# batra-mlp-lab/visdial

Hardware: AMD Instinct MI355X
Metric: QA-rounds/sec training mn-att-ques-im-hist+disc (batch 20x10x100) (higher is better)
Workload: dtype f32 operands and results; the option recurrence multiplies the EXACT 3-way bf16 split of both operands (9 bf16 MFMA products per fp32 product, f32 accumulate: fp32-grade, errors at the f32 MFMA's own level) -- its two step kernels and its weight-gradient contraction; f32 MFMA (v_mfma_f32_32x32x2_f32

## Files before the change

### visdial_amd/csrc/common.h

```cpp
#pragma once
#include <hip/hip_runtime.h>
#include <stdint.h>
#include <stdio.h>
#include <string.h>

#define VD_OK 0
#define VD_ERR_ARG -1
#define VD_ERR_HIP -2
#define VD_ERR_STATE -3
#define VD_FLAG_BF16 1
#define VD_FLAG_SPLIT9 2
#define VD_FLAG_SPLIT6 4
#define VD_FLAG_SPLIT3 8
#define VD_FLAG_SPLIT (VD_FLAG_SPLIT9 | VD_FLAG_SPLIT6 | VD_FLAG_SPLIT3)
#define VD_FLAG_LIVE_PREFIX 16
#define VD_FLAG_STATE_ONLY 32
#define VD_FLAG_TREE 64
#define VD_LIVE_PREFIX_ROWS 128

void vd_set_error(const char* fmt, ...);

#define VD_CHECK_ARG(cond, ...)                                   \
  do {                                                            \
    if (!(cond)) {                                                \
      vd_set_error(__VA_ARGS__);                                  \
      return VD_ERR_ARG;                                          \
    }                                                             \
  } while (0)

#define VD_HIP(expr)                                                          \
  do {                                                                        \
    hipError_t e__ = (expr);                                                  \
    if (e__ != hipSuccess) {                                                  \
      vd_set_error("%s:%d: %s -> %s", __FILE__, __LINE__, #expr,              \
                   hipGetErrorString(e__));                                   \
      return VD_ERR_HIP;                                                      \
    }                                                                         \
  } while (0)

#define VD_LAUNCH_CHECK() VD_HIP(hipGetLastError())

static inline int vd_cdiv(long a, long b) { return (int)((a + b - 1) / b); }
static inline unsigned grid_for(long n) { return (unsigned)std::max<long>(1, std::min<long>((n + 255) / 256, 4096)); }

void vd_range_push(const char* name);
void vd_range_pop();
struct VdRange {
  explicit VdRange(const char* name) { vd_range_push(name); }
  ~VdRange() { vd_range_pop(); }
  VdRange(const VdRange&) = delete;
  VdRange& operator=(const VdRange&) = delete;
};

struct VdStreamScratch {
  float* wht = nullptr;
  size_t wht_bytes = 0;
  unsigned* sync = nullptr;
  size_t sync_bytes = 0;
};
int vd_stream_scratch(hipStream_t stream, size_t wht_bytes, size_t sync_bytes, VdStreamScratch* out);
int vd_num_cus();

struct VdZeroSet {
  float* buf[6];
  int ncols[6];
  int n;
  long quads_per_row;
};
int vd_zero_inactive_multi(const VdZeroSet& z, const int32_t* nact_dev, int T, int N, hipStream_t stream);

typedef unsigned short vd_bf16_bits;
int vd_lstm_forward_c16(const vd_bf16_bits* table16, int64_t tab_ld, const int32_t* tok_gather, const float* Wh, vd_bf16_bits* gates16,
                        vd_bf16_bits* h16, float* h_last, float* c, int T, int N, int H, hipStream_t stream);
int vd_lstm_backward_c16(const float* Wh, vd_bf16_bits* gates16, const float* c, const float* dh_last, float* dc_work, int T, int N, int H,
                         hipStream_t stream);
int vd_f32_to_bf16(const float* src, vd_bf16_bits* dst, int64_t n, hipStream_t stream);
int vd_gemm_tn_acc_bf16(const vd_bf16_bits* A16, const vd_bf16_bits* B16, float* C, int64_t ldc, int M, int N, int K, hipStream_t stream);
int vd_segment_rowsum_acc_bf16(const vd_bf16_bits* X16, int64_t ldx, const int32_t* tok, const int32_t* perm, int64_t n, int ncol,
                               float* out, int64_t ldo, hipStream_t stream);

int vd_bf16_shadow_get(int slot, const float* base, size_t floats, vd_bf16_bits** out);
const vd_bf16_bits* vd_bf16_shadow_find(const float* p, size_t floats);
void vd_bf16_shadow_invalidate(const float* p, size_t floats);

typedef float f32x16 __attribute__((ext_vector_type(16)));

__device__ __forceinline__ float vd_rcp(float x) { return __builtin_amdgcn_rcpf(x); }
__device__ __forceinline__ float vd_sigmoid(float x) { return vd_rcp(1.0f + __expf(-x)); }
__device__ __forceinline__ float vd_tanh(float x) {
  const float e = __expf(-2.0f * fabsf(x));
  const float t = (1.0f - e) * vd_rcp(1.0f + e);
  return copysignf(t, x);
}

typedef unsigned vd_u32x4 __attribute__((ext_vector_type(4)));
typedef unsigned vd_u32x2 __attribute__((ext_vector_type(2)));
__device__ __forceinline__ __amdgpu_buffer_rsrc_t vd_rsrc(const void* p) {
  return __builtin_amdgcn_make_buffer_rsrc(const_cast<void*>(p), 0, -1, 0x00020000);
}
__device__ __forceinline__ float4 vd_buf_ld4(__amdgpu_buffer_rsrc_t r, unsigned voff, unsigned soff) {
  const vd_u32x4 v = __builtin_amdgcn_raw_buffer_load_b128(r, voff, soff, 0);
  return make_float4(__uint_as_float(v.x), __uint_as_float(v.y), __uint_as_float(v.z), __uint_as_float(v.w));
}
__device__ __forceinline__ void vd_buf_st4(__amdgpu_buffer_rsrc_t r, unsigned voff, unsigned soff, const float4& v) {
  const vd_u32x4 t = {__float_as_uint(v.x), __float_as_uint(v.y), __float_as_uint(v.z), __float_as_uint(v.w)};
  __builtin_amdgcn_raw_buffer_store_b128(t, r, voff, soff, 0);
}
__device__ __forceinline__ void vd_buf_st4_bf16(__amdgpu_buffer_rsrc_t r, unsigned voff, unsigned soff, const float4& v) {
  typedef __bf16 bf4 __attribute__((ext_vector_type(4)));
  const bf4 t = {(__bf16)v.x, (__bf16)v.y, (__bf16)v.z, (__bf16)v.w};
  __builtin_amdgcn_raw_buffer_store_b64(__builtin_bit_cast(vd_u32x2, t), r, voff, soff, 0);
}

__device__ __forceinline__ float4 vd_bf16x4_unpack(const vd_u32x2 v) {
  return make_float4(__uint_as_float(v.x << 16), __uint_as_float(v.x & 0xffff0000u), __uint_as_float(v.y << 16),
                     __uint_as_float(v.y & 0xffff0000u));
}
__device__ __forceinline__ float4 vd_buf_ld4_bf16(__amdgpu_buffer_rsrc_t r, unsigned voff, unsigned soff) {
  return vd_bf16x4_unpack(__builtin_amdgcn_raw_buffer_load_b64(r, voff, soff, 0));
}

__device__ __forceinline__ void vd_st4_bf16(vd_bf16_bits* p, const float4& v) {
  typedef __bf16 bf4 __attribute__((ext_vector_type(4)));
  bf4 t = {(__bf16)v.x, (__bf16)v.y, (__bf16)v.z, (__bf16)v.w};
  *reinterpret_cast<bf4*>(p) = t;
}

__device__ __forceinline__ float wave_sum(float v) {
#pragma unroll
  for (int o = 32; o > 0; o >>= 1) v += __shfl_xor(v, o, 64);
  return v;
}
__device__ __forceinline__ float wave_max(float v) {
#pragma unroll
  for (int o = 32; o > 0; o >>= 1) v = fmaxf(v, __shfl_xor(v, o, 64));
  return v;
}

__device__ __forceinline__ float block_row_lse(const float* row, int V, float* red) {
  const int tid = threadIdx.x, lane = tid & 63, wave = tid >> 6;
  float mx = -INFINITY;
  for (int c = tid; c < V; c += 256) mx = fmaxf(mx, row[c]);
  mx = wave_max(mx);
  if (lane == 0) red[wave] = mx;
  __syncthreads();
  mx = fmaxf(fmaxf(red[0], red[1]), fmaxf(red[2], red[3]));
  float sum = 0.f;
  for (int c = tid; c < V; c += 256) sum += expf(row[c] - mx);
  sum = wave_sum(sum);
  if (lane == 0) red[4 + wave] = sum;
  __syncthreads();
  return mx + logf(red[4] + red[5] + red[6] + red[7]);
}
```

### visdial_amd/csrc/elementwise.hip

```cpp
#include <stdlib.h>

#include "common.h"

__device__ __forceinline__ uint32_t mix32(uint64_t x) {
  x ^= x >> 33;
  x *= 0xff51afd7ed558ccdULL;
  x ^= x >> 33;
  x *= 0xc4ceb9fe1a85ec53ULL;
  x ^= x >> 33;
  return (uint32_t)x;
}

__global__ void dropout_mask_kernel(uint8_t* __restrict__ mask, long n, uint64_t seed, float p) {
  const long i4 = ((long)blockIdx.x * blockDim.x + threadIdx.x) * 4;
  if (i4 >= n) return;
  const uint32_t thr = (uint32_t)(p * 16777216.0f);
  uint8_t m[4];
#pragma unroll
  for (int k = 0; k < 4; ++k) {
    const uint32_t h = mix32(seed * 0x9E3779B97F4A7C15ULL + (uint64_t)(i4 + k));
    m[k] = ((h >> 8) >= thr) ? 1 : 0;
  }
  if (i4 + 3 < n) {
    *reinterpret_cast<uint32_t*>(mask + i4) = m[0] | (m[1] << 8) | (m[2] << 16) | ((uint32_t)m[3] << 24);
  } else {
    for (int k = 0; k < 4 && i4 + k < n; ++k) mask[i4 + k] = m[k];
  }
}

__global__ void dropout_apply_kernel(const float* __restrict__ x, const uint8_t* __restrict__ mask,
                                     float* __restrict__ y, long n, float scale) {
  const long i = (long)blockIdx.x * blockDim.x + threadIdx.x;
  if (i < n) y[i] = mask[i] ? x[i] * scale : 0.f;
}

__global__ void tanh_bwd_kernel(const float* __restrict__ dy, const float* __restrict__ y,
                                float* __restrict__ dx, long n) {
  const long i = (long)blockIdx.x * blockDim.x + threadIdx.x;
  if (i < n) {
    const float t = y[i];
    dx[i] = dy[i] * (1.f - t * t);
  }
}

__global__ void axpby_kernel(const float* __restrict__ a, const float* __restrict__ b, float* __restrict__ c,
                             long n, float alpha, float beta) {
  const long i = (long)blockIdx.x * blockDim.x + threadIdx.x;
  if (i < n) c[i] = alpha * a[i] + (b ? beta * b[i] : 0.f);
}

__global__ void embed_gather_kernel(const float* __restrict__ emb, const int* __restrict__ tok,
                                    const uint8_t* __restrict__ mask, float* __restrict__ out, long rows, int E,
                                    float scale) {
  const int e4 = E >> 2;
  const long idx = (long)blockIdx.x * blockDim.x + threadIdx.x;
  if (idx >= rows * e4) return;
  const long r = idx / e4;
  const int q = (int)(idx - r * e4);
  float4 v = *reinterpret_cast<const float4*>(emb + (long)tok[r] * E + q * 4);
  if (mask) {
    const uint32_t m = *reinterpret_cast<const uint32_t*>(mask + r * E + q * 4);
    v.x = (m & 0xff) ? v.x * scale : 0.f;
    v.y = (m & 0xff00) ? v.y * scale : 0.f;
    v.z = (m & 0xff0000) ? v.z * scale : 0.f;
    v.w = (m & 0xff000000u) ? v.w * scale : 0.f;
  }
  *reinterpret_cast<float4*>(out + r * E + q * 4) = v;
}

__global__ void embed_scatter_kernel(float* __restrict__ demb, const int* __restrict__ tok,
                                     const uint8_t* __restrict__ mask, const float* __restrict__ dx, long rows,
                                     int E, float scale) {
  const long idx = (long)blockIdx.x * blockDim.x + threadIdx.x;
  if (idx >= rows * E) return;
  const long r = idx / E;
  const int e = (int)(idx - r * E);
  float v = dx[idx];
  if (mask) v = mask[idx] ? v * scale : 0.f;
  if (v != 0.f) unsafeAtomicAdd(demb + (long)tok[r] * E + e, v);
}

__global__ void mask_time_fwd_kernel(const float* __restrict__ feat, const int* __restrict__ tok,
                                     float* __restrict__ out, int T, int N, int D) {
  const long idx = (long)blockIdx.x * blockDim.x + threadIdx.x;
  const long total = (long)T * N * D;
  if (idx >= total) return;
  const long tn = idx / D;
  const int d = (int)(idx - tn * D);
  const int n = (int)(tn % N);
  out[idx] = tok[tn] != 0 ? feat[(long)n * D + d] : 0.f;
}
__global__ void mask_time_bwd_kernel(const float* __restrict__ dout, const int* __restrict__ tok,
                                     float* __restrict__ dfeat, int T, int N, int D) {
  const long idx = (long)blockIdx.x * blockDim.x + threadIdx.x;
  if (idx >= (long)N * D) return;
  const int n = (int)(idx / D);
  const int d = (int)(idx - (long)n * D);
  float s = 0.f;
  for (int t = 0; t < T; ++t)
    if (tok[(long)t * N + n] != 0) s += dout[((long)t * N + n) * D + d];
  dfeat[idx] = s;
}

__global__ void zero_inactive_rows_kernel(float* __restrict__ buf, long tstride, long ld, int ncols,
                                          const int* __restrict__ nact, int N) {
  const int t = blockIdx.y;
  const int first = nact[t];
  const long total = (long)(N - first) * (ncols >> 2);
  for (long idx = (long)blockIdx.x * blockDim.x + threadIdx.x; idx < total; idx += (long)gridDim.x * blockDim.x) {
    const long r = idx / (ncols >> 2);
    const int q = (int)(idx - r * (ncols >> 2));
    *reinterpret_cast<float4*>(buf + t * tstride + (first + r) * ld + q * 4) = make_float4(0.f, 0.f, 0.f, 0.f);
  }
}

__global__ void zero_inactive_multi_kernel(VdZeroSet z, const int* __restrict__ nact, int N) {
  const int t = blockIdx.y;
  const int first = nact[t];
  const long per_row = z.quads_per_row;
  const long total = (long)(N - first) * per_row;
  for (long idx = (long)blockIdx.x * blockDim.x + threadIdx.x; idx < total; idx += (long)gridDim.x * blockDim.x) {
    const long r = idx / per_row;
    int q = (int)(idx - r * per_row);
    int b = 0;
#pragma unroll
    for (int i = 0; i < 5; ++i)
      if (b == i && i + 1 < z.n && q >= (z.ncols[i] >> 2)) { q -= z.ncols[i] >> 2; b = i + 1; }
    *reinterpret_cast<float4*>(z.buf[b] + ((long)t * N + first + r) * z.ncols[b] + q * 4) = make_float4(0.f, 0.f, 0.f, 0.f);
  }
}

__device__ __forceinline__ int wave_agg_atomic_inc(int* base, int tok, bool active) {
  int result = 0;
  unsigned long long todo = __ballot(active);
  const int lane = threadIdx.x & 63;
  while (todo) {
    const int leader = __ffsll((long long)todo) - 1;
    const int ltok = __shfl(tok, leader, 64);
    const unsigned long long same = __ballot(active && tok == ltok) & todo;
    int basev = 0;
    if (lane == leader) basev = atomicAdd(base + ltok, __popcll(same));
    basev = __shfl(basev, leader, 64);
    if ((same >> lane) & 1ULL) result = basev + __popcll(same & ((1ULL << lane) - 1ULL));
    todo &= ~same;
  }
  return result;
}

__global__ void tok_count_kernel(const int* __restrict__ tok, long n, int* __restrict__ count) {
  const long i = (long)blockIdx.x * blockDim.x + threadIdx.x;
  const bool active = i < n;
  wave_agg_atomic_inc(count, active ? tok[i] : 0, active);
}

__global__ void tok_scan_kernel(const int* __restrict__ count, int V, int* __restrict__ offset,
                                int* __restrict__ cursor) {
  __shared__ int part[1024];
  const int tid = threadIdx.x, nt = blockDim.x;
  const int per = (V + nt - 1) / nt;
  const int b = tid * per, e = min(V, b + per);
  int s = 0;
  for (int i = b; i < e; ++i) s += count[i];
  part[tid] = s;
  __syncthreads();
  if (tid == 0) {
    int run = 0;
    for (int i = 0; i < nt; ++i) {
      const int t = part[i];
      part[i] = run;
      run += t;
    }
    offset[V] = run;
  }
  __syncthreads();
  int run = part[tid];
  for (int i = b; i < e; ++i) {
    offset[i] = run;
    cursor[i] = run;
    run += count[i];
  }
}

__global__ void tok_fill_kernel(const int* __restrict__ tok, long n, int* __restrict__ cursor,
                                int* __restrict__ perm) {
  const long i = (long)blockIdx.x * blockDim.x + threadIdx.x;
  const bool active = i < n;
  const int p = wave_agg_atomic_inc(cursor, active ? tok[i] : 0, active);
  if (active) perm[p] = (int)i;
}

template <int CHUNK, bool X16 = false>
__global__ void __launch_bounds__(256)
segment_rowsum_kernel(const float* __restrict__ X, long ldx, const int* __restrict__ tok,
                      const int* __restrict__ perm, long n, int ncol, float* __restrict__ out, long ldo) {
  __shared__ int srow[CHUNK], stok[CHUNK];
  const long p0 = (long)blockIdx.x * CHUNK;
  if (p0 >= n) return;
  const int cnt = (int)min((long)CHUNK, n - p0);
  if ((int)threadIdx.x < cnt) {
    const int r = perm[p0 + threadIdx.x];
    srow[threadIdx.x] = r;
    stok[threadIdx.x] = tok[r];
  }
  __syncthreads();
  if constexpr (X16) {
    const vd_bf16_bits* X16p = reinterpret_cast<const vd_bf16_bits*>(X);
    for (int c = threadIdx.x * 4; c < ncol; c += blockDim.x * 8) {
      const int c2 = c + blockDim.x * 4;
      const bool two = c2 < ncol;
      float4 acc0 = make_float4(0.f, 0.f, 0.f, 0.f), acc1 = acc0;
      auto flush = [&](int token) {
        float* o = out + (long)token * ldo + c;
        unsafeAtomicAdd(o, acc0.x); unsafeAtomicAdd(o + 1, acc0.y); unsafeAtomicAdd(o + 2, acc0.z); unsafeAtomicAdd(o + 3, acc0.w);
        if (two) {
          float* o2 = out + (long)token * ldo + c2;
          unsafeAtomicAdd(o2, acc1.x); unsafeAtomicAdd(o2 + 1, acc1.y); unsafeAtomicAdd(o2 + 2, acc1.z); unsafeAtomicAdd(o2 + 3, acc1.w);
        }
        acc0 = acc1 = make_float4(0.f, 0.f, 0.f, 0.f);
      };
      int cur = stok[0];
      int j = 0;
      while (j < cnt) {
        uint2 w0[4], w1[4];
        int t[4];
#pragma unroll
        for (int u = 0; u < 4; ++u) {
          const int jj = min(j + u, cnt - 1);
          t[u] = stok[jj];
          const vd_bf16_bits* row = X16p + (long)srow[jj] * ldx;
          w0[u] = *reinterpret_cast<const uint2*>(row + c);
          w1[u] = two ? *reinterpret_cast<const uint2*>(row + c2) : make_uint2(0u, 0u);
        }
#pragma unroll
        for (int u = 0; u < 4; ++u) {
          if (j + u >= cnt) break;
          if (t[u] != cur) {
            flush(cur);
            cur = t[u];
          }
          acc0.x += __uint_as_float(w0[u].x << 16); acc0.y += __uint_as_float(w0[u].x & 0xffff0000u);
          acc0.z += __uint_as_float(w0[u].y << 16); acc0.w += __uint_as_float(w0[u].y & 0xffff0000u);
          acc1.x += __uint_as_float(w1[u].x << 16); acc1.y += __uint_as_float(w1[u].x & 0xffff0000u);
          acc1.z += __uint_as_float(w1[u].y << 16); acc1.w += __uint_as_float(w1[u].y & 0xffff0000u);
        }
        j += 4;
      }
      flush(cur);
    }
    return;
  }
  for (int c = threadIdx.x * 4; c < ncol; c += blockDim.x * 4) {
    float4 acc = make_float4(0.f, 0.f, 0.f, 0.f);
    int cur = stok[0];
    int j = 0;
    while (j < cnt) {
      float4 v[4];
      int t[4];
#pragma unroll
      for (int u = 0; u < 4; ++u) {
        const int jj = min(j + u, cnt - 1);
        t[u] = stok[jj];
        v[u] = *reinterpret_cast<const float4*>(X + (long)srow[jj] * ldx + c);
      }
#pragma unroll
      for (int u = 0; u < 4; ++u) {
        if (j + u >= cnt) break;
        if (t[u] != cur) {
          float* o = out + (long)cur * ldo + c;
          unsafeAtomicAdd(o, acc.x);
          unsafeAtomicAdd(o + 1, acc.y);
          unsafeAtomicAdd(o + 2, acc.z);
          unsafeAtomicAdd(o + 3, acc.w);
          acc = make_float4(0.f, 0.f, 0.f, 0.f);
          cur = t[u];
        }
        acc.x += v[u].x;
        acc.y += v[u].y;
        acc.z += v[u].z;
        acc.w += v[u].w;
      }
      j += 4;
    }
    float* o = out + (long)cur * ldo + c;
    unsafeAtomicAdd(o, acc.x);
    unsafeAtomicAdd(o + 1, acc.y);
    unsafeAtomicAdd(o + 2, acc.z);
    unsafeAtomicAdd(o + 3, acc.w);
  }
}

__global__ void clamp_adam_kernel(float* __restrict__ w, float* __restrict__ g, float* __restrict__ m,
                                  float* __restrict__ v, long n, float gscale, float clip, float b1, float b2,
                                  float eps, float step) {
  const long i4 = ((long)blockIdx.x * blockDim.x + threadIdx.x) * 4;
  if (i4 + 3 < n) {
    float4 W = *reinterpret_cast<float4*>(w + i4), G = *reinterpret_cast<float4*>(g + i4);
    float4 Mv = *reinterpret_cast<float4*>(m + i4), Vv = *reinterpret_cast<float4*>(v + i4);
    float* Wp = &W.x;
    float* Gp = &G.x;
    float* Mp = &Mv.x;
    float* Vp = &Vv.x;
#pragma unroll
    for (int k = 0; k < 4; ++k) {
      float gg = Gp[k] * gscale;
      gg = fminf(fmaxf(gg, -clip), clip);
      Gp[k] = gg;
      Mp[k] = b1 * Mp[k] + (1.f - b1) * gg;
      Vp[k] = b2 * Vp[k] + (1.f - b2) * gg * gg;
      Wp[k] -= step * Mp[k] / (sqrtf(Vp[k]) + eps);
    }
    *reinterpret_cast<float4*>(w + i4) = W;
    *reinterpret_cast<float4*>(g + i4) = G;
    *reinterpret_cast<float4*>(m + i4) = Mv;
    *reinterpret_cast<float4*>(v + i4) = Vv;
  } else {
    for (long i = i4; i < n; ++i) {
      float gg = g[i] * gscale;
      gg = fminf(fmaxf(gg, -clip), clip);
      g[i] = gg;
      m[i] = b1 * m[i] + (1.f - b1) * gg;
      v[i] = b2 * v[i] + (1.f - b2) * gg * gg;
      w[i] -= step * m[i] / (sqrtf(v[i]) + eps);
    }
  }
}

static inline dim3 grid1d(long n, int block) { return dim3((unsigned)((n + block - 1) / block)); }

extern "C" {

int vd_dropout_mask(uint8_t* mask, int64_t n, uint64_t seed, float p, void* stream) {
  VD_CHECK_ARG(mask && n >= 0 && p >= 0.f && p < 1.f && ((uintptr_t)mask & 3) == 0, "vd_dropout_mask: bad args");
  if (n == 0) return VD_OK;
  hipLaunchKernelGGL(dropout_mask_kernel, grid1d((n + 3) / 4, 256), dim3(256), 0, (hipStream_t)stream, mask,
                     (long)n, seed, p);
  VD_LAUNCH_CHECK();
  return VD_OK;
}

int vd_dropout_apply(const float* x, const uint8_t* mask, float* y, int64_t n, float scale, void* stream) {
  VD_CHECK_ARG(x && mask && y && n >= 0, "vd_dropout_apply: bad args");
  if (n == 0) return VD_OK;
  hipLaunchKernelGGL(dropout_apply_kernel, grid1d(n, 256), dim3(256), 0, (hipStream_t)stream, x, mask, y,
                     (long)n, scale);
  VD_LAUNCH_CHECK();
  return VD_OK;
}

int vd_tanh_backward(const float* dy, const float* y, float* dx, int64_t n, void* stream) {
  VD_CHECK_ARG(dy && y && dx && n >= 0, "vd_tanh_backward: bad args");
  if (n == 0) return VD_OK;
  hipLaunchKernelGGL(tanh_bwd_kernel, grid1d(n, 256), dim3(256), 0, (hipStream_t)stream, dy, y, dx, (long)n);
  VD_LAUNCH_CHECK();
  return VD_OK;
}

int vd_axpby(const float* a, const float* b, float* c, int64_t n, float alpha, float beta, void* stream) {
  VD_CHECK_ARG(a && c && n >= 0, "vd_axpby: bad args");
  if (n == 0) return VD_OK;
  hipLaunchKernelGGL(axpby_kernel, grid1d(n, 256), dim3(256), 0, (hipStream_t)stream, a, b, c, (long)n, alpha,
                     beta);
  VD_LAUNCH_CHECK();
  return VD_OK;
}

int vd_mask_time_forward(const float* feat, const int32_t* tok, float* out, int T, int N, int D, void* stream) {
  VD_CHECK_ARG(feat && tok && out && T >= 0 && N >= 0 && D > 0, "vd_mask_time_forward: bad args");
  const long total = (long)T * N * D;
  if (total == 0) return VD_OK;
  hipLaunchKernelGGL(mask_time_fwd_kernel, grid1d(total, 256), dim3(256), 0, (hipStream_t)stream, feat, tok, out,
                     T, N, D);
  VD_LAUNCH_CHECK();
  return VD_OK;
}

int vd_mask_time_backward(const float* dout, const int32_t* tok, float* dfeat, int T, int N, int D,
                          void* stream) {
  VD_CHECK_ARG(dout && tok && dfeat && T >= 0 && N >= 0 && D > 0, "vd_mask_time_backward: bad args");
  if ((long)N * D == 0) return VD_OK;
  hipLaunchKernelGGL(mask_time_bwd_kernel, grid1d((long)N * D, 256), dim3(256), 0, (hipStream_t)stream, dout,
                     tok, dfeat, T, N, D);
  VD_LAUNCH_CHECK();
  return VD_OK;
}

int vd_zero_inactive_rows(float* buf, int64_t tstride, int64_t ld, int ncols, const int32_t* nact_dev, int T,
                          int N, void* stream) {
  VD_CHECK_ARG(buf && nact_dev && T >= 0 && N >= 0 && ncols % 4 == 0 && ld % 4 == 0, "vd_zero_inactive_rows: bad args");
  if (T == 0 || N == 0) return VD_OK;
  hipLaunchKernelGGL(zero_inactive_rows_kernel, dim3(64, T), dim3(256), 0, (hipStream_t)stream, buf, (long)tstride,
                     (long)ld, ncols, nact_dev, N);
  VD_LAUNCH_CHECK();
  return VD_OK;
}

int vd_embed_gather(const float* emb, const int32_t* tok, const uint8_t* mask, float* out, int64_t rows, int E,
                    float scale, void* stream);
}
int vd_zero_inactive_multi(const VdZeroSet& z, const int32_t* nact_dev, int T, int N, hipStream_t stream) {
  VD_CHECK_ARG(z.n >= 1 && z.n <= 6 && nact_dev && T >= 0 && N >= 0, "vd_zero_inactive_multi: bad args");
  if (T == 0 || N == 0) return VD_OK;
  VdZeroSet zz = z;
  zz.quads_per_row = 0;
  for (int i = 0; i < z.n; ++i) {
    VD_CHECK_ARG(z.buf[i] && z.ncols[i] % 4 == 0, "vd_zero_inactive_multi: buffer %d", i);
    zz.quads_per_row += z.ncols[i] >> 2;
  }
  hipLaunchKernelGGL(zero_inactive_multi_kernel, dim3(128, T), dim3(256), 0, stream, zz, nact_dev, N);
  VD_LAUNCH_CHECK();
  return VD_OK;
}
extern "C" {
int vd_embed_gather(const float* emb, const int32_t* tok, const uint8_t* mask, float* out, int64_t rows, int E,
                    float scale, void* stream) {
  VD_CHECK_ARG(emb && tok && out && rows >= 0 && E > 0 && E % 4 == 0, "vd_embed_gather: bad args (E=%d)", E);
  if (rows == 0) return VD_OK;
  hipLaunchKernelGGL(embed_gather_kernel, grid1d(rows * (E / 4), 256), dim3(256), 0, (hipStream_t)stream, emb,
                     tok, mask, out, (long)rows, E, scale);
  VD_LAUNCH_CHECK();
  return VD_OK;
}

int vd_embed_scatter_acc(float* demb, const int32_t* tok, const uint8_t* mask, const float* dx, int64_t rows,
                         int E, float scale, void* stream) {
  VD_CHECK_ARG(demb && tok && dx && rows >= 0 && E > 0, "vd_embed_scatter_acc: bad args");
  if (rows == 0) return VD_OK;
  hipLaunchKernelGGL(embed_scatter_kernel, grid1d(rows * E, 256), dim3(256), 0, (hipStream_t)stream, demb, tok,
                     mask, dx, (long)rows, E, scale);
  VD_LAUNCH_CHECK();
  return VD_OK;
}

int vd_token_sort(const int32_t* tok, int64_t n, int V, int32_t* offset, int32_t* work, int32_t* perm,
                  void* stream) {
  VD_CHECK_ARG(tok && offset && work && perm && n >= 0 && V > 0, "vd_token_sort: bad args");
  hipStream_t s = (hipStream_t)stream;
  int* count = work;
  int* cursor = work + V;
  VD_HIP(hipMemsetAsync(count, 0, sizeof(int) * V, s));
  if (n > 0) {
    hipLaunchKernelGGL(tok_count_kernel, grid1d(n, 256), dim3(256), 0, s, tok, (long)n, count);
    VD_LAUNCH_CHECK();
  }
  hipLaunchKernelGGL(tok_scan_kernel, dim3(1), dim3(1024), 0, s, count, V, offset, cursor);
  VD_LAUNCH_CHECK();
  if (n > 0) {
    hipLaunchKernelGGL(tok_fill_kernel, grid1d(n, 256), dim3(256), 0, s, tok, (long)n, cursor, perm);
    VD_LAUNCH_CHECK();
  }
  return VD_OK;
}

int vd_segment_rowsum_acc(const float* X, int64_t ldx, const int32_t* tok, const int32_t* perm, int64_t n,
                          int ncol, float* out, int64_t ldo, void* stream) {
  VD_CHECK_ARG(X && tok && perm && out && n >= 0 && ncol > 0 && ncol % 4 == 0 && ldx % 4 == 0 && ldo % 4 == 0,
               "vd_segment_rowsum_acc: bad args");
  if (n == 0) return VD_OK;
  hipLaunchKernelGGL(segment_rowsum_kernel<256>, grid1d(n, 256), dim3(256), 0, (hipStream_t)stream, X, (long)ldx, tok, perm, (long)n, ncol,
                     out, (long)ldo);
  VD_LAUNCH_CHECK();
  return VD_OK;
}

int vd_clamp_adam(float* w, float* g, float* m, float* v, int64_t n, float gscale, float clip, float beta1,
                  float beta2, float eps, float step, void* stream) {
  VD_CHECK_ARG(w && g && m && v && n >= 0, "vd_clamp_adam: bad args");
  VD_CHECK_ARG((((uintptr_t)w | (uintptr_t)g | (uintptr_t)m | (uintptr_t)v) & 15) == 0,
               "vd_clamp_adam: buffers must be 16-byte aligned");
  if (n == 0) return VD_OK;
  hipLaunchKernelGGL(clamp_adam_kernel, grid1d((n + 3) / 4, 256), dim3(256), 0, (hipStream_t)stream, w, g, m, v,
                     (long)n, gscale, clip, beta1, beta2, eps, step);
  VD_LAUNCH_CHECK();
  return VD_OK;
}

}

int vd_segment_rowsum_acc_bf16(const vd_bf16_bits* X16, int64_t ldx, const int32_t* tok, const int32_t* perm, int64_t n, int ncol,
                               float* out, int64_t ldo, hipStream_t stream) {
  VD_CHECK_ARG(X16 && tok && perm && out && n >= 0 && ncol % 4 == 0 && ldx % 4 == 0, "vd_segment_rowsum_acc_bf16: bad args");
  if (n == 0) return VD_OK;
  hipLaunchKernelGGL((segment_rowsum_kernel<256, true>), grid1d(n, 256), dim3(256), 0, stream, reinterpret_cast<const float*>(X16), (long)ldx,
                     tok, perm, (long)n, ncol, out, (long)ldo);
  VD_LAUNCH_CHECK();
  return VD_OK;
}
```

### visdial_amd/csrc/gemm_ops.hip

```cpp
#include "gemm_core.h"
#include "split_core.h"

using CfgBigDB = GemmCfg<4, 1, 4, 32>;
using CfgBig = GemmCfg<4, 1, 4, 16, 0, 3>;
using CfgSmall = GemmCfg<1, 4, 1, 32, 0, 3>;

static inline bool use_small(int M, int N) {
  return (long)vd_cdiv(M, CfgBig::BM) * vd_cdiv(N, CfgBig::BN) < 48;
}

static int check_align(const void* p, long ld, const char* what) {
  if (((uintptr_t)p & 15) != 0 || (ld & 3) != 0) {
    vd_set_error("%s: pointer must be 16-byte aligned and leading dimension a multiple of 4 (ld=%ld)", what, ld);
    return VD_ERR_ARG;
  }
  return VD_OK;
}

__global__ void colsum_kernel(const float* __restrict__ X, long ld, int M, int N, int rows_per_block,
                              float* __restrict__ out) {
  const int col = blockIdx.x * blockDim.x + threadIdx.x;
  if (col >= N) return;
  const int r0 = blockIdx.y * rows_per_block;
  const int r1 = min(M, r0 + rows_per_block);
// ... 82 lines not shown
#pragma unroll
    for (int r = 0; r < 16; ++r) acc[j][r] = 0.f;

  const int key = (lane & 7) >> 1, col = (lane >> 3) * 16 + (lane & 1) * 8;
  unsigned voffa[2], voffb[2];
#pragma unroll
  for (int i = 0; i < 2; ++i) {
    const int krow = (i * 4 + wm) * 4 + key;
    voffa[i] = (unsigned)(((long)krow * M + m0 + col) * 2);
    voffb[i] = (unsigned)(((long)krow * N + n0 + col) * 2);
  }
  const unsigned lds0 = (unsigned)(uintptr_t)lds;
  auto issue = [&](int kt, int buf) {
    const float* ak = reinterpret_cast<const float*>(A + (long)(ks + kt * 32) * M);
    const float* bk = reinterpret_cast<const float*>(B + (long)(ks + kt * 32) * N);
#pragma unroll
    for (int i = 0; i < 2; ++i) glds16(voffb[i], bk, lds0 + buf * 2 * TILE + TILE + (i * 4 + wm) * 1024);
#pragma unroll
    for (int i = 0; i < 2; ++i) glds16(voffa[i], ak, lds0 + buf * 2 * TILE + (i * 4 + wm) * 1024);
  };
  const int g = lane >> 4, li = lane & 15;
  const int frag = ((g >> 1) * 2) * 1024 + (g & 1) * 128 + li * 8;

  if (nk > 0) {
    issue(0, 0);
    if (nk > 1) issue(1, 1);
    int buf = 0;
    for (int kt = 0; kt < nk; ++kt) {
      if (kt + 1 < nk) asm volatile("s_waitcnt vmcnt(4)" ::: "memory");
      else asm volatile("s_waitcnt vmcnt(0)" ::: "memory");
      asm volatile("s_barrier" ::: "memory");
      if (kt + 2 < nk) issue(kt + 2, buf == 0 ? 2 : buf - 1);
      const char* ta = lds + buf * 2 * TILE;
      const char* tb = ta + TILE;
#pragma unroll
      for (int st = 0; st < 2; ++st) {
        const vd_bf16x8 a8 = tr_read8(ta, frag + st * 4096 + wm * 256);
        vd_bf16x8 b8[4];
#pragma unroll
        for (int j = 0; j < 4; ++j) b8[j] = tr_read8(tb, frag + st * 4096 + j * 256);
#pragma unroll
        for (int j = 0; j < 4; ++j) acc[j] = __builtin_amdgcn_mfma_f32_32x32x16_bf16(a8, b8[j], acc[j], 0, 0, 0);
      }
      buf = buf == 2 ? 0 : buf + 1;
    }
  }
#pragma unroll
  for (int j = 0; j < 4; ++j) {
    const int c = n0 + j * 32 + (lane & 31);
#pragma unroll
    for (int r = 0; r < 16; ++r) {
      const int row = m0 + wm * 32 + mfma_row(r, lane);
      unsafeAtomicAdd(C + (long)row * ldc + c, acc[j][r]);
    }
  }
}

template <int NBUF>
__global__ void __launch_bounds__(512)
gemm_bf16_tn_tr256_kernel(const vd_bf16_bits* __restrict__ A, const vd_bf16_bits* __restrict__ B, float* __restrict__ C, long ldc,
                          int M, int N, int K, int kchunk, int tiles_m, int tiles_n) {
  extern __shared__ __attribute__((aligned(16))) float smem[];
  constexpr int TILE = 16384;
  char* const lds = reinterpret_cast<char*>(smem);
  const int wg = xcd_remap(blockIdx.x, gridDim.x);
  const int tile_n = wg % tiles_n, tile_m = (wg / tiles_n) % tiles_m, split = wg / (tiles_n * tiles_m);
  const int ks = split * kchunk, ke = min(K, ks + kchunk);
  const int nk = ke > ks ? (ke - ks) / 32 : 0;
  const int lane = threadIdx.x & 63;
  const int w = __builtin_amdgcn_readfirstlane((int)threadIdx.x >> 6);
  const int wm = w & 3, wn = w >> 2;
  const int m0 = tile_m * 256, n0 = tile_n * 256;

  f32x16 acc[2][4];
#pragma unroll
  for (int i = 0; i < 2; ++i)
#pragma unroll
    for (int j = 0; j < 4; ++j)
#pragma unroll
      for (int r = 0; r < 16; ++r) acc[i][j][r] = 0.f;

  unsigned voffa[2], voffb[2];
#pragma unroll
  for (int i = 0; i < 2; ++i) {
    const int krow = (i * 8 + w) * 2 + (lane >> 5);
    const int cb = ((lane & 31) * 16) ^ ((krow & 3) << 6);
    voffa[i] = (unsigned)(((long)krow * M + m0) * 2 + cb);
    voffb[i] = (unsigned)(((long)krow * N + n0) * 2 + cb);
  }
  const unsigned lds0 = (unsigned)(uintptr_t)lds;
  auto issue = [&](int kt, int buf) {
    const float* ak = reinterpret_cast<const float*>(A + (long)(ks + kt * 32) * M);
    const float* bk = reinterpret_cast<const float*>(B + (long)(ks + kt * 32) * N);
#pragma unroll
    for (int i = 0; i < 2; ++i) glds16(voffb[i], bk, lds0 + buf * 2 * TILE + TILE + (i * 8 + w) * 1024);
#pragma unroll
    for (int i = 0; i < 2; ++i) glds16(voffa[i], ak, lds0 + buf * 2 * TILE + (i * 8 + w) * 1024);
  };
  const int g = lane >> 4, li = lane & 15;
  const int frag = (g >> 1) * 4096 + (li >> 2) * 512 + (g & 1) * 32 + (li & 3) * 8;
  int xa[2], xb[4];
#pragma unroll
  for (int i = 0; i < 2; ++i) xa[i] = frag + (((wm * 2 + i) ^ (li >> 2)) << 6);
#pragma unroll
  for (int j = 0; j < 4; ++j) xb[j] = frag + (((wn * 4 + j) ^ (li >> 2)) << 6);
  auto rd8 = [&](const char* base, int off) {
    typedef __attribute__((address_space(3))) vd_s16x4* lds_p;
    union {
      vd_s16x4 h[2];
      vd_bf16x8 v;
    } u;
    u.h[0] = __builtin_amdgcn_ds_read_tr16_b64_v4i16((lds_p)(base + off));
    u.h[1] = __builtin_amdgcn_ds_read_tr16_b64_v4i16((lds_p)(base + off + 2048));
    return u.v;
  };

  struct Frags {
    vd_bf16x8 a[2], b[4];
  };
  auto read_step = [&](Frags& f, int buf, int st) {
    const char* ta = lds + buf * 2 * TILE;
    const char* tb = ta + TILE;
#pragma unroll
    for (int i = 0; i < 2; ++i) f.a[i] = rd8(ta, xa[i] + st * 8192);
#pragma unroll
    for (int j = 0; j < 4; ++j) f.b[j] = rd8(tb, xb[j] + st * 8192);
  };
  auto mfma_step = [&](const Frags& f) {
#pragma unroll
    for (int i = 0; i < 2; ++i)
#pragma unroll
      for (int j = 0; j < 4; ++j) acc[i][j] = __builtin_amdgcn_mfma_f32_32x32x16_bf16(f.a[i], f.b[j], acc[i][j], 0, 0, 0);
  };
  auto wait_tiles_in_flight = [&](int later) {
    if (later >= 3) asm volatile("s_waitcnt vmcnt(12)" ::: "memory");
    else if (later == 2) asm volatile("s_waitcnt vmcnt(8)" ::: "memory");
    else if (later == 1) asm volatile("s_waitcnt vmcnt(4)" ::: "memory");
    else asm volatile("s_waitcnt vmcnt(0)" ::: "memory");
  };
  if (nk > 0) {
#pragma unroll
    for (int i = 0; i < NBUF - 1; ++i)
      if (i < nk) issue(i, i);
    wait_tiles_in_flight(min(NBUF - 2, nk - 1));
    asm volatile("s_barrier" ::: "memory");
    Frags f0, f1;
    read_step(f0, 0, 0);
    int buf = 0;
    for (int kt = 0; kt < nk; ++kt) {
      const int nbuf = buf == NBUF - 1 ? 0 : buf + 1;
      read_step(f1, buf, 1);
      mfma_step(f0);
      if (kt + 1 < nk) {
        wait_tiles_in_flight(min(NBUF - 3, nk - 2 - kt));
        asm volatile("s_barrier" ::: "memory");
        if (kt + NBUF - 1 < nk) issue(kt + NBUF - 1, buf == 0 ? NBUF - 1 : buf - 1);
        read_step(f0, nbuf, 0);
      }
      mfma_step(f1);
      buf = nbuf;
    }
  }
#pragma unroll
  for (int i = 0; i < 2; ++i)
#pragma unroll
    for (int j = 0; j < 4; ++j) {
      const int c = n0 + wn * 128 + j * 32 + (lane & 31);
#pragma unroll
      for (int r = 0; r < 16; ++r) {
        const int row = m0 + wm * 64 + i * 32 + mfma_row(r, lane);
        unsafeAtomicAdd(C + (long)row * ldc + c, acc[i][j][r]);
      }
    }
}

static int launch_gemm_bf16_tn_tr256(const vd_bf16_bits* A, const vd_bf16_bits* B, float* C, long ldc, int M, int N, int K,
                                     hipStream_t stream) {
  const int tiles_m = M / 256, tiles_n = N / 256;
  long splits = vd_cdiv(256, (long)tiles_m * tiles_n);
  int kchunk = vd_cdiv(vd_cdiv(K, splits), 32) * 32;
  if (kchunk < 32) kchunk = 32;
  splits = vd_cdiv(K, kchunk);
  static bool attr_set = false;
#ifndef VD_TR256_NBUF
#define VD_TR256_NBUF 3
#endif
  constexpr int NBUF = VD_TR256_NBUF;
  const int lds = NBUF * 2 * 16384;
  if (!attr_set) {
    VD_HIP(hipFuncSetAttribute(reinterpret_cast<const void*>(gemm_bf16_tn_tr256_kernel<NBUF>),
                               hipFuncAttributeMaxDynamicSharedMemorySize, lds));
    attr_set = true;
  }
  hipLaunchKernelGGL(gemm_bf16_tn_tr256_kernel<NBUF>, dim3((unsigned)(tiles_m * tiles_n * splits)), dim3(512), lds, stream, A, B, C,
                     ldc, M, N, K, kchunk, tiles_m, tiles_n);
  VD_LAUNCH_CHECK();
  return VD_OK;
}

static int launch_gemm_bf16_tn_tr(const vd_bf16_bits* A, const vd_bf16_bits* B, float* C, long ldc, int M, int N, int K,
                                  hipStream_t stream) {
  const int tiles_m = M / 128, tiles_n = N / 128;
  long splits = vd_cdiv(768, (long)tiles_m * tiles_n);
  int kchunk = vd_cdiv(vd_cdiv(K, splits), 32) * 32;
  if (kchunk < 32) kchunk = 32;
  splits = vd_cdiv(K, kchunk);
  static bool attr_set = false;
  const int lds = 3 * 2 * 8192;
  if (!attr_set) {
    VD_HIP(hipFuncSetAttribute(reinterpret_cast<const void*>(gemm_bf16_tn_tr_kernel),
                               hipFuncAttributeMaxDynamicSharedMemorySize, lds));
    attr_set = true;
  }
  hipLaunchKernelGGL(gemm_bf16_tn_tr_kernel, dim3((unsigned)(tiles_m * tiles_n * splits)), dim3(256), lds, stream, A, B, C,
                     ldc, M, N, K, kchunk, tiles_m, tiles_n);
  VD_LAUNCH_CHECK();
  return VD_OK;
}

extern "C" {

int vd_gemm_nt(const float* A, int64_t lda, const float* W, int64_t ldw, const float* bias, float* C,
               int64_t ldc, int M, int N, int K, int act, int accumulate, void* stream) {
  VD_CHECK_ARG(A && W && C && M >= 0 && N >= 0 && K >= 0 && K % 4 == 0, "vd_gemm_nt: bad args M=%d N=%d K=%d", M,
               N, K);
  if (int rc = check_align(A, lda, "vd_gemm_nt A")) return rc;
  if (int rc = check_align(W, ldw, "vd_gemm_nt W")) return rc;
  SrcRow a{A, lda}, b{W, ldw};
  hipStream_t s = (hipStream_t)stream;
  if (use_small(M, N)) {
    EpiStore<1> e{C, ldc, bias, act, accumulate};
    return launch_gemm<CfgSmall>(M, N, K, 1, a, b, e, s);
  }
  EpiStore<4> e{C, ldc, bias, act, accumulate};
  if (M >= 1024 && K >= 64 && K % 16 == 0 && (long)M * lda * 4 < (1L << 32) && (long)N * ldw * 4 < (1L << 32)) {
    int splits = 1;
    const long tiles = (long)vd_cdiv(M, 128) * vd_cdiv(N, 128);
    if (accumulate == 2 && !bias && act == VD_ACT_NONE && tiles < 512 && K >= 1024) {
      splits = (int)vd_cdiv(768, tiles);
      if (splits > K / 512) splits = K / 512;
    }
    return launch_gemm_glds<GemmCfg<4, 1, 4, 16, 0, 4, 41984>, false>(M, N, K, splits, A, lda, W, ldw, e, s, -1, splits > 1);
  }
  return launch_gemm<CfgBig>(M, N, K, 1, a, b, e, s);
}

int vd_gemm_nn(const float* A, int64_t lda, const float* B, int64_t ldb, const float* bias, float* C,
               int64_t ldc, int M, int N, int K, int accumulate, void* stream) {
  VD_CHECK_ARG(A && B && C && M >= 0 && N >= 0 && K >= 0 && (K % 4 == 0 || lda >= (K + 3) / 4 * 4) && N % 4 == 0,
               "vd_gemm_nn: bad args M=%d N=%d K=%d", M, N, K);
  if (int rc = check_align(A, lda, "vd_gemm_nn A")) return rc;
  if (int rc = check_align(B, ldb, "vd_gemm_nn B")) return rc;
  SrcRow a{A, lda};
  SrcK b{B, ldb};
  hipStream_t s = (hipStream_t)stream;
  if (use_small(M, N)) {
    EpiStore<1> e{C, ldc, bias, VD_ACT_NONE, accumulate};
    return launch_gemm<CfgSmall>(M, N, K, 1, a, b, e, s);
  }
  EpiStore<4> e{C, ldc, bias, VD_ACT_NONE, accumulate};
  return launch_gemm<CfgBig>(M, N, K, 1, a, b, e, s);
}

}

template <int NT>
struct EpiStoreLive : EpiStore<NT> {
  const int* tok_mask;
  static constexpr bool HAS_DEAD = true;
  __device__ __forceinline__ bool dead(int row_base, int ) const { return tok_mask[row_base] == 0; }
};
static_assert(CfgSmall::BM == VD_LSTM_FWD_TILE_SMALL && CfgBig::BM == VD_LSTM_FWD_TILE_BIG, "the projection's row tiles are the step kernels'");

int vd_gemm_nn_live_p(const float* A, int64_t lda, const float* B, int64_t ldb, const float* bias, float* C, int64_t ldc, int M, int N, int K,
                      const int32_t* tok_mask, int row_tile, hipStream_t s) {
  VD_CHECK_ARG(A && B && C && tok_mask && M >= 0 && N >= 0 && K >= 0 && (K % 4 == 0 || lda >= (K + 3) / 4 * 4) && N % 4 == 0 &&
                   (row_tile == CfgSmall::BM || row_tile == CfgBig::BM),
               "vd_gemm_nn (live rows): bad args M=%d N=%d K=%d row tile %d", M, N, K, row_tile);
  if (int rc = check_align(A, lda, "vd_gemm_nn (live rows) A")) return rc;
  if (int rc = check_align(B, ldb, "vd_gemm_nn (live rows) B")) return rc;
  SrcRow a{A, lda};
  SrcK b{B, ldb};
  if (row_tile == CfgSmall::BM) {
    EpiStoreLive<1> e{{C, ldc, bias, VD_ACT_NONE, 0}, tok_mask};
    return launch_gemm<CfgSmall>(M, N, K, 1, a, b, e, s);
  }
  EpiStoreLive<4> e{{C, ldc, bias, VD_ACT_NONE, 0}, tok_mask};
  return launch_gemm<CfgBig>(M, N, K, 1, a, b, e, s);
}

extern "C" {

int vd_gemm_tn_acc(const float* A, int64_t lda, const float* B, int64_t ldb, float* C, int64_t ldc, int M,
                   int N, int K, int flags, void* stream) {
  VD_CHECK_ARG(A && B && C && M >= 0 && N >= 0 && K >= 0 && (M % 4 == 0 || lda >= (M + 3) / 4 * 4) &&
                   (N % 4 == 0 || ldb >= (N + 3) / 4 * 4),
               "vd_gemm_tn_acc: bad args M=%d N=%d K=%d", M, N, K);
  if (int rc = check_align(A, lda, "vd_gemm_tn_acc A")) return rc;
  if (int rc = check_align(B, ldb, "vd_gemm_tn_acc B")) return rc;
  if (K == 0) return VD_OK;
  SrcK a{A, lda}, b{B, ldb};
  EpiAtomic<4> e{C, ldc};
  const long tiles = (long)vd_cdiv(M, CfgBig::BM) * vd_cdiv(N, CfgBig::BN);
  if ((flags & VD_FLAG_SPLIT9) && !(flags & VD_FLAG_BF16) && vd_tn_split_tiles(M, N) && K >= 8192 &&
      16L * lda * 4 < (1L << 31) && 16L * ldb * 4 < (1L << 31)) {
    const int K1 = K & ~15;
    if (int rc = launch_gemm_split_tn<9>(M, N, K1, A, lda, B, ldb, C, ldc, (hipStream_t)stream)) return rc;
    if (K1 == K) return VD_OK;
    SrcK a2{A + (long)K1 * lda, lda}, b2{B + (long)K1 * ldb, ldb};
    return launch_gemm<GemmCfg<4, 1, 4, 16, 0, 4, 41984>>(M, N, K - K1, 1, a2, b2, e, (hipStream_t)stream);
  }
  const bool kmaj = !(flags & VD_FLAG_BF16) && vd_tn_kmajor_fits(M, N, K);
  if (kmaj && K % 16 != 0) {
    const int K1 = K & ~15;
    if (int rc = vd_gemm_tn_acc(A, lda, B, ldb, C, ldc, M, N, K1, flags, stream)) return rc;
    SrcK a2{A + (long)K1 * lda, lda}, b2{B + (long)K1 * ldb, ldb};
    return launch_gemm<GemmCfg<4, 1, 4, 16, 0, 4, 41984>>(M, N, K - K1, 1, a2, b2, e, (hipStream_t)stream);
  }
  long splits = vd_cdiv(768, tiles);
  const long max_splits = vd_cdiv(K, 1024);
  if (splits > max_splits) splits = max_splits;
  if (splits < 1) splits = 1;
  if (flags & VD_FLAG_BF16) {
    if (M % 128 == 0 && N % 128 == 0 && K >= 32 && lda == M && ldb == N && (long)32 * N * 2 + 256 < (1L << 31)) {
      const vd_bf16_bits* a16 = vd_bf16_shadow_find(A, (size_t)K * M);
      const vd_bf16_bits* b16 = vd_bf16_shadow_find(B, (size_t)K * N);
      if (a16 && b16) {
        const int K1 = K & ~31;
        if (int rc = launch_gemm_bf16_tn_tr(a16, b16, C, ldc, M, N, K1, (hipStream_t)stream)) return rc;
        if (K1 == K) return VD_OK;
        SrcK a2{A + (long)K1 * lda, lda}, b2{B + (long)K1 * ldb, ldb};
        return launch_gemm<GemmCfg<4, 1, 4, 32, 0, 3, 0, 1>>(M, N, K - K1, 1, a2, b2, e, (hipStream_t)stream);
      }
    }
    if (vd_tn_split_tiles(M, N) && K >= 1024 && lda % 4 == 0 && ldb % 4 == 0 && 16L * lda * 4 < (1L << 31) &&
        16L * ldb * 4 < (1L << 31)) {
      const int K1 = K & ~15;
      if (int rc = launch_gemm_split_tn<1>(M, N, K1, A, lda, B, ldb, C, ldc, (hipStream_t)stream)) return rc;
      if (K1 == K) return VD_OK;
      SrcK a2{A + (long)K1 * lda, lda}, b2{B + (long)K1 * ldb, ldb};
      return launch_gemm<GemmCfg<4, 1, 4, 32, 0, 3, 0, 1>>(M, N, K - K1, 1, a2, b2, e, (hipStream_t)stream);
    }
    return launch_gemm<GemmCfg<4, 1, 4, 32, 0, 3, 0, 1>>(M, N, K, (int)splits, a, b, e, (hipStream_t)stream);
  }
  if (kmaj)
    return launch_gemm_glds<GemmCfg<4, 1, 4, 16, 0, 4, 41984>, true>(M, N, K, (int)splits, A, lda, B, ldb, e, (hipStream_t)stream, 0);
  return launch_gemm<GemmCfg<4, 1, 4, 16, 0, 4, 41984>>(M, N, K, (int)splits, a, b, e, (hipStream_t)stream);
}

int vd_gemm_tn_rows_acc(const float* A, int64_t lda, const int32_t* a_rows, const float* B, int64_t ldb,
                        const int32_t* b_rows, float* C, int64_t ldc, int M, int N, int K, void* stream) {
  VD_CHECK_ARG(A && B && C && a_rows && b_rows && M >= 0 && N >= 0 && K >= 0 && (M % 4 == 0 || lda >= (M + 3) / 4 * 4) &&
                   (N % 4 == 0 || ldb >= (N + 3) / 4 * 4),
               "vd_gemm_tn_rows_acc: bad args M=%d N=%d K=%d", M, N, K);
  if (int rc = check_align(A, lda, "vd_gemm_tn_rows_acc A")) return rc;
  if (int rc = check_align(B, ldb, "vd_gemm_tn_rows_acc B")) return rc;
  if (K == 0) return VD_OK;
  SrcKRows a{A, lda, a_rows}, b{B, ldb, b_rows};
  EpiAtomic<4> e{C, ldc};
  using Cfg = GemmCfg<4, 1, 4, 16, 0, 4, 41984>;
  const long tiles = (long)vd_cdiv(M, Cfg::BM) * vd_cdiv(N, Cfg::BN);
  long splits = vd_cdiv(768, tiles);
  const long max_splits = vd_cdiv(K, 1024);
  if (splits > max_splits) splits = max_splits;
  if (splits < 1) splits = 1;
  return launch_gemm<Cfg>(M, N, K, (int)splits, a, b, e, (hipStream_t)stream);
}

int vd_colsum_acc(const float* X, int64_t ld, int M, int N, float* out, void* stream) {
  VD_CHECK_ARG(X && out && M >= 0 && N >= 0, "vd_colsum_acc: bad args");
  if (M == 0 || N == 0) return VD_OK;
  if (N % 4 == 0 && ld % 4 == 0 && ((uintptr_t)X & 15) == 0 && M >= 64) {
    const int cb4 = vd_cdiv(N, 256);
    int rb4 = vd_cdiv(2048, cb4);
    int rpb = vd_cdiv(vd_cdiv(M, rb4), 4) * 4;
    if (rpb < 32) rpb = 32;
    rb4 = vd_cdiv(M, rpb);
    hipLaunchKernelGGL(colsum4_kernel, dim3(cb4, rb4), dim3(256), 0, (hipStream_t)stream, X, ld, M, N, rpb, out);
    VD_LAUNCH_CHECK();
    return VD_OK;
  }
  const int cb = vd_cdiv(N, 256);
  int rb = vd_cdiv(1024, cb);
  int rows_per_block = vd_cdiv(M, rb);
  if (rows_per_block < 16) rows_per_block = 16;
  rb = vd_cdiv(M, rows_per_block);
  hipLaunchKernelGGL(colsum_kernel, dim3(cb, rb), dim3(256), 0, (hipStream_t)stream, X, ld, M, N,
                     rows_per_block, out);
  VD_LAUNCH_CHECK();
  return VD_OK;
}

}

__global__ void __launch_bounds__(256) bf16_tn_tail_kernel(const vd_bf16_bits* __restrict__ A, const vd_bf16_bits* __restrict__ B, float* __restrict__ C,
                                                           long ldc, int M, int N, int K) {
  const long i = (long)blockIdx.x * 256 + threadIdx.x;
  if (i >= (long)M * N) return;
  const int m = (int)(i / N), n = (int)(i % N);
  float acc = 0.f;
  for (int k = 0; k < K; ++k)
    acc += __uint_as_float((unsigned)A[(long)k * M + m] << 16) * __uint_as_float((unsigned)B[(long)k * N + n] << 16);
  unsafeAtomicAdd(C + (long)m * ldc + n, acc);
}
int vd_gemm_tn_acc_bf16(const vd_bf16_bits* A16, const vd_bf16_bits* B16, float* C, int64_t ldc, int M, int N, int K, hipStream_t stream) {
  VD_CHECK_ARG(A16 && B16 && C && M % 128 == 0 && N % 128 == 0 && K >= 0, "vd_gemm_tn_acc_bf16: M, N must be multiples of 128");
  const int K1 = K & ~31;
  if (K1 > 0) {
    const bool big = M % 256 == 0 && N % 256 == 0 && K1 >= 8192;
    if (int rc = big ? launch_gemm_bf16_tn_tr256(A16, B16, C, ldc, M, N, K1, stream) : launch_gemm_bf16_tn_tr(A16, B16, C, ldc, M, N, K1, stream)) return rc;
  }
  if (K1 < K) {
    hipLaunchKernelGGL(bf16_tn_tail_kernel, dim3((unsigned)(((long)M * N + 255) / 256)), dim3(256), 0, stream, A16 + (long)K1 * M, B16 + (long)K1 * N,
                       C, (long)ldc, M, N, K - K1);
    VD_LAUNCH_CHECK();
  }
  return VD_OK;
}
```

### visdial_amd/csrc/paths.h

```cpp
#pragma once
#include "common.h"

static inline int vd_precision_flags(int lstmBf16) {
  switch (lstmBf16) {
    case 0: return 0;
    case 1: return VD_FLAG_BF16;
    case 3: return VD_FLAG_SPLIT3;
    case 6: return VD_FLAG_SPLIT6;
    case 9: return VD_FLAG_SPLIT9;
    default: return -1;
  }
}
static inline int vd_split_nprod(int flags) {
  return (flags & VD_FLAG_SPLIT9) ? 9 : (flags & VD_FLAG_SPLIT6) ? 6 : (flags & VD_FLAG_SPLIT3) ? 3 : 0;
}

constexpr long VD_THROUGHPUT_ROWS = 2048;
constexpr int VD_LSTM_FWD_TILE_BIG = 128, VD_LSTM_FWD_TILE_SMALL = 32;
static inline int vd_lstm_fwd_row_tile(long N) { return N >= VD_THROUGHPUT_ROWS ? VD_LSTM_FWD_TILE_BIG : VD_LSTM_FWD_TILE_SMALL; }
static inline bool vd_lstm_glds_fwd_fits(long N, int H) { return N >= VD_THROUGHPUT_ROWS && H % 32 == 0 && N * H * 4 < (1L << 32); }
static inline bool vd_lstm_glds_bwd_fits(long N, int H) { return N >= VD_THROUGHPUT_ROWS && H % 32 == 0 && N * 4 * H * 4 < (1L << 32); }
static inline bool vd_lstm_bf16_fits(long N, int H) { return N >= VD_THROUGHPUT_ROWS && H % 32 == 0; }
static inline bool vd_lstm_c16_fits(long N, int H) { return N >= VD_THROUGHPUT_ROWS && H % 128 == 0; }

static inline bool vd_tn_kmajor_fits(long M, long N, long K) { return M % 128 == 0 && N % 128 == 0 && K >= 1024; }
constexpr int VD_SPLIT_TN_BM = 256, VD_SPLIT_TN_BN = 128;
static inline bool vd_tn_split_tiles(long M, long N) { return M % VD_SPLIT_TN_BM == 0 && N % VD_SPLIT_TN_BN == 0; }

static inline bool vd_img_split_ok(long rows, int H, int Kc) {
  return rows >= 128 && H % 16 == 0 && Kc % 16 == 0 && rows * (H > Kc ? H : Kc) * 4 < (1L << 32);
}

static inline bool vd_lhood_fused_fits(long rows, long ldh, long V, long ldw, int H) {
  return H >= 64 && H % 16 == 0 && V >= 128 && ldh % 4 == 0 && ldw % 4 == 0 && rows * ldh * 4 < (1L << 32) && V * ldw * 4 < (1L << 32);
}
static inline bool vd_lhood_prefix_fits(int T, long rows) { return T >= 1 && T < 256 && rows >= 1; }
```

### visdial_amd/csrc/rt_core.h

```cpp
#pragma once
#include <math.h>
#include <stdarg.h>
#include <stdlib.h>
#include <string.h>

#include <algorithm>
#include <map>
#include <memory>
#include <numeric>
#include <random>
#include <string>
#include <vector>

#include "../../include/visdial_hip.h"
#include "common.h"
#include "paths.h"

int vd_lstm2_forward_p(const vd_lstm2_fwd_t* st, int nstacks, int H, int flags, hipStream_t stream);
int vd_lstm2_backward_p(const vd_lstm2_bwd_t* st, int nstacks, int H, int flags, hipStream_t stream);

int vd_img_drop_gather(const float* pre, const uint8_t* mask1, float* xdrop, int N, int R, int S2, int H, float scale, hipStream_t stream);
int vd_img_common_forward_p(const float* pre, const uint8_t* mask1, const float* xdrop, const float* Wc, const float* bc, const float* qc,
                            const uint8_t* mask2, float* iqc, int N, int R, int S2, int H, int Kc, float scale, int flags, hipStream_t stream);
int vd_img_tr_backward_p(const float* dz, const float* Wc, const float* p, const float* datt, const uint8_t* mask1, float* dpre, int N, int R,
                         int S2, int H, int Kc, float scale, int flags, hipStream_t stream);
int vd_img_common_wgrad_p(const float* dz, const float* pre, const uint8_t* mask1, const float* xdrop, float* dWc, int N, int R, int S2, int H,
                          int Kc, float scale, int flags, hipStream_t stream);

int vd_gemm_nn_live_p(const float* A, int64_t lda, const float* B, int64_t ldb, const float* bias, float* C, int64_t ldc, int M, int N, int K,
                      const int32_t* tok_mask, int row_tile, hipStream_t stream);
int vd_lhood_order_p(const int32_t* tok_in, const int32_t* target, int T, int64_t rows, int C, int32_t* perm, int32_t* rep, int32_t* tok_in_s,
                     int32_t* target_s, int32_t* work, int32_t* info, hipStream_t stream);
int64_t vd_lhood_order_work_ints(int T, int64_t rows);
int vd_lhood_sum_p(const float* nll, const int32_t* act, int64_t n_act, int T, int64_t rows, int C, const int32_t* perm, float* out, int64_t ldo,
                   hipStream_t stream);

int vd_lhood_lse_p(const float* h, int64_t ldh, int64_t rows, const int32_t* act, int64_t n_act, const float* W, int64_t ldw, const float* bias,
                   int V, int H, float* lse, hipStream_t stream);
int vd_lhood_edge_sum_p(const float* h, int64_t ldh, const int32_t* node_row, const float* lse, const int32_t* enode, const int32_t* etgt, int T,
                        int64_t rows, int C, const float* W, int64_t ldw, const float* bias, int H, float* out, int64_t ldo, hipStream_t stream);

#define VD_TRY(expr)                  \
  do {                                \
    const int rc__ = (expr);          \
    if (rc__ != VD_OK) return rc__;   \
  } while (0)

namespace vdrt {

struct Tensor {
  std::string name;
  long off, rows, cols;
  int kind;
  long numel() const { return rows * cols; }
};

struct DevBuf {
  void* p = nullptr;
  size_t bytes = 0;
};

struct SeqTok {
  int T = 0, N = 0;
  bool present = false, sorted = false;
  int32_t* tok = nullptr;
  std::vector<int32_t> nact;
  int32_t *tok_sorted = nullptr, *fwd_idx = nullptr, *inv_idx = nullptr, *perm = nullptr, *inv = nullptr, *nact_dev = nullptr;
  int32_t *act = nullptr, *act1 = nullptr, *prev1 = nullptr;
  int n_act = 0, n_act1 = 0;
};

struct TreeChunk {
  int o0 = 0, C = 0, Tl = 0, Nw = 0;
  long n_nodes = 0;
  std::vector<int32_t> widths;
  int32_t* mask2 = nullptr;
  int32_t* node_row = nullptr;
  int32_t *enode = nullptr, *etgt = nullptr;
};

struct BatchSlot {
  int B = 0;
  bool tree_ok = false;
  std::vector<TreeChunk> tree;
  SeqTok q, h, opt, ain, aout, oin, oout;
  float* img = nullptr;
  int32_t* gt = nullptr;
  std::vector<int32_t> gt_host;
  bool has_gt = false;
  int32_t* opt_uid = nullptr;
  int opt_total = 0;
  int32_t *opt_sort_off = nullptr, *opt_sort_perm = nullptr;
  bool cached = false;
  uint64_t cache_stamp = 0;
  std::vector<int32_t> miss_keys, opt_host;
  hipEvent_t ready = nullptr;
  hipEvent_t done = nullptr;
  bool used = false;
  bool uploaded = false;
  std::map<std::string, DevBuf> bufs, pinned;
};

struct RowIndex {
  int T = 0;
  std::vector<int32_t> keys;
  std::vector<int32_t> table;
  int32_t size() const { return T ? (int32_t)(keys.size() / (size_t)T) : 0; }
  void reset(int T_) {
    T = T_;
    keys.clear();
    table.assign(1024, -1);
  }
  size_t home(const int32_t* row) const {
    uint64_t h = 1469598103934665603ull;
    for (int t = 0; t < T; ++t) h = (h ^ (uint32_t)row[t]) * 1099511628211ull;
    return (size_t)(h ^ (h >> 29)) & (table.size() - 1);
  }
  int32_t find(const int32_t* row) const {
    for (size_t pos = home(row);; pos = (pos + 1) & (table.size() - 1)) {
      const int32_t u = table[pos];
      if (u < 0) return -1;
      if (memcmp(keys.data() + (size_t)u * T, row, (size_t)T * sizeof(int32_t)) == 0) return u;
    }
  }
  int32_t add(const int32_t* row) {
    if ((size_t)(size() + 1) * 2 > table.size()) {
      table.assign(table.size() * 2, -1);
      for (int32_t u = 0; u < size(); ++u) place(keys.data() + (size_t)u * T, u);
    }
    const int32_t id = size();
    keys.insert(keys.end(), row, row + T);
    place(keys.data() + (size_t)id * T, id);
    return id;
  }
  void place(const int32_t* row, int32_t id) {
    size_t pos = home(row);
    while (table[pos] >= 0) pos = (pos + 1) & (table.size() - 1);
    table[pos] = id;
  }
};

struct OptionCache {
  long capacity = 0;
  RowIndex index;
  float* table = nullptr;
  long table_rows = 0;
  uint64_t stamp = 1;
  void flush() {
    index.reset(index.T);
    ++stamp;
  }
};
static constexpr long VD_OPTION_CACHE_DEFAULT_ROWS = 262144;
static constexpr long VD_OPTION_CACHE_FIRST_ROWS = 16384;

struct Encoder;
struct Decoder;

}

struct vd_model {
  vd_model_params p;
  int flags = 0;
  std::string enc_name, dec_name;
  std::vector<vdrt::Tensor> spec;
  std::map<std::string, int> index;
  long numel = 0;
  float *W = nullptr, *G = nullptr, *M = nullptr, *V = nullptr;
  std::map<std::string, vdrt::DevBuf> ws;
  std::map<std::string, vdrt::DevBuf> ext_masks;
  hipStream_t s_main = nullptr, s_enc = nullptr, s_img = nullptr, s_hist = nullptr, s_tab = nullptr, s_copy = nullptr;
  hipStream_t s_wg = nullptr;
  bool wg_active = false, wg_used = false;
  std::vector<hipEvent_t> ev_pool;
  size_t ev_next = 0;
  hipEvent_t ev_enc_grads = nullptr;
  hipEvent_t ev_updated = nullptr;
  bool updated_recorded = false;
  bool enc_grads_recorded = false;
  hipEvent_t ev_loss = nullptr, ev_prof[6] = {nullptr, nullptr, nullptr, nullptr, nullptr, nullptr};
  bool training = true, streams = true, prof_valid = false;
  long step = 0;
  int adam_t = 0;
  double lr = 1e-3;
  vdrt::BatchSlot slot[2];
  int cur = -1, uploaded = -1;
  float* loss_host = nullptr;
  long loss_cap = 0, loss_n = 0;
  bool loss_is_sum = false;
  std::unique_ptr<vdrt::Encoder> enc;
  std::unique_ptr<vdrt::Decoder> dec;
  float* scores = nullptr;
  float* gen_enc_out = nullptr;
  int gen_seq_len = 0;
  int N = 0, O = 0;
  long lhood_exec = -1, lhood_total = 0;
  bool use_im = false, use_hist = false, is_att = false, is_graph = false;
  vdrt::OptionCache ocache;
  bool lhood_tree = false;
  bool prof_hist = false;
  ~vd_model();
};

namespace vdrt {

inline int dev_get(std::map<std::string, DevBuf>& m, const std::string& key, size_t bytes, void** out) {
  DevBuf& b = m[key];
  if (b.bytes < bytes) {
    if (b.p) VD_HIP(hipFree(b.p));
    b.p = nullptr;
    b.bytes = 0;
    VD_HIP(hipMalloc(&b.p, bytes ? bytes : 16));
    b.bytes = bytes ? bytes : 16;
  }
  *out = b.p;
  return VD_OK;
}
inline int pin_get(std::map<std::string, DevBuf>& m, const std::string& key, size_t bytes, void** out) {
  DevBuf& b = m[key];
  if (b.bytes < bytes) {
    if (b.p) VD_HIP(hipHostFree(b.p));
    b.p = nullptr;
    b.bytes = 0;
    VD_HIP(hipHostMalloc(&b.p, bytes ? bytes : 16, hipHostMallocDefault));
    b.bytes = bytes ? bytes : 16;
  }
  *out = b.p;
  return VD_OK;
}

template <class T>
int ws_get(vd_model* m, const std::string& key, size_t count, T** out) {
  void* p = nullptr;
  VD_TRY(dev_get(m->ws, key, count * sizeof(T), &p));
  *out = static_cast<T*>(p);
  return VD_OK;
}

inline void add_lstm(vd_model* m, const std::string& name, long D, long H) {
  m->spec.push_back(Tensor{name + ".W", 0, D + H, 4 * H, 1});
  m->spec.push_back(Tensor{name + ".b", 0, 1, 4 * H, 2});
}
inline void add_linear(vd_model* m, const std::string& name, long in, long out) {
  m->spec.push_back(Tensor{name + ".W", 0, out, in, 3});
  m->spec.push_back(Tensor{name + ".b", 0, 1, out, 4});
}
inline std::string hop_sfx(int i) { return i == 0 ? std::string() : std::to_string(i + 1); }

inline float* Wp(vd_model* m, const std::string& n) { return m->W + m->spec[m->index.at(n)].off; }
inline float* Gp(vd_model* m, const std::string& n) { return m->G + m->spec[m->index.at(n)].off; }

inline int fork_stream(vd_model* m, hipStream_t from, hipStream_t side) {
  if (side == from) return VD_OK;
  hipEvent_t e = m->ev_pool[m->ev_next++ % m->ev_pool.size()];
  VD_HIP(hipEventRecord(e, from));
  VD_HIP(hipStreamWaitEvent(side, e, 0));
  return VD_OK;
}
inline int join_stream(vd_model* m, hipStream_t side, hipStream_t to) { return fork_stream(m, side, to); }
inline hipStream_t side_stream(vd_model* m, hipStream_t wanted, hipStream_t cur) { return m->streams ? wanted : cur; }
inline int wg_fork(vd_model* m, hipStream_t cur, hipStream_t* out) {
  *out = cur;
  if (!m->wg_active || !m->s_wg) return VD_OK;
  VD_TRY(fork_stream(m, cur, m->s_wg));
  m->wg_used = true;
  *out = m->s_wg;
  return VD_OK;
}

inline int drop_mask(vd_model* m, const std::string& site, size_t numel, float p, hipStream_t s, uint8_t** out) {
  *out = nullptr;
  if (!m->training || p <= 0.f) return VD_OK;
  auto it = m->ext_masks.find(site);
  if (it != m->ext_masks.end()) {
    VD_CHECK_ARG(it->second.bytes >= numel, "dropout mask '%s' holds %zu bytes, the batch needs %zu", site.c_str(),
                 it->second.bytes, numel);
    *out = static_cast<uint8_t*>(it->second.p);
    return VD_OK;
  }
  if (!m->ext_masks.empty()) {
    vd_set_error("external dropout masks are set but none for site '%s'", site.c_str());
    return VD_ERR_STATE;
  }
  uint8_t* buf = nullptr;
  VD_TRY(ws_get(m, "dropmask." + site, numel + 4, &buf));
  uint32_t h = 2166136261u;
  for (const char c : site) h = (h ^ (uint8_t)c) * 16777619u;
  const uint64_t seed = ((uint64_t)((m->p.seed * 1000003ull + (uint64_t)m->step) & 0xffffffffull) << 32) | h;
  VD_TRY(vd_dropout_mask(buf, (int64_t)numel, seed, p, s));
  *out = buf;
  return VD_OK;
}
inline int dropout_fwd(vd_model* m, const std::string& key, const float* x, const uint8_t* mask, float scale, long n, hipStream_t s,
                       const float** y) {
  *y = x;
  if (!mask) return VD_OK;
  float* buf;
  VD_TRY(ws_get(m, key, (size_t)n, &buf));
  VD_TRY(vd_dropout_apply(x, mask, buf, n, scale, s));
  *y = buf;
  return VD_OK;
}

inline int index_array(vd_model* m, const std::string& key, const std::vector<int32_t>& host, int32_t** out) {
  DevBuf& b = m->ws[key];
  if (b.bytes != host.size() * sizeof(int32_t) || !b.p) {
    if (b.p) VD_HIP(hipFree(b.p));
    b.p = nullptr;
    VD_HIP(hipMalloc(&b.p, host.size() * sizeof(int32_t) + 16));
    b.bytes = host.size() * sizeof(int32_t);
    VD_HIP(hipMemcpy(b.p, host.data(), b.bytes, hipMemcpyHostToDevice));
  }
  *out = static_cast<int32_t*>(b.p);
  return VD_OK;
}
inline int round_index(vd_model* m, int N, int R, int32_t** out) {
  std::vector<int32_t> h(N);
  for (int n = 0; n < N; ++n) h[n] = n / R;
  return index_array(m, "idx.rep." + std::to_string(N) + "." + std::to_string(R), h, out);
}

struct Linear {
  std::string name;
  long in = 0, out = 0;
  const float* x = nullptr;
  float* y = nullptr;
  long M = 0;
  bool tanh_ = false;
  void init(const std::string& n, long i, long o) { name = n; in = i; out = o; }
  int forward(vd_model* m, hipStream_t s, const float* x_, long M_, bool tanh, float** y_out) {
    x = x_; M = M_; tanh_ = tanh;
    VD_TRY(ws_get(m, name + ".y", (size_t)M * out, &y));
    VD_TRY(vd_gemm_nt(x, in, Wp(m, name + ".W"), in, Wp(m, name + ".b"), y, out, (int)M, (int)out, (int)in,
                      tanh ? VD_ACT_TANH : VD_ACT_NONE, 0, s));
    if (y_out) *y_out = y;
    return VD_OK;
  }
  int backward(vd_model* m, hipStream_t s, const float* dy, bool need_dx, float** dx_out) {
    const float* d = dy;
    if (tanh_) {
      float* dpre;
      VD_TRY(ws_get(m, name + ".dpre", (size_t)M * out, &dpre));
      VD_TRY(vd_tanh_backward(dy, y, dpre, M * out, s));
      d = dpre;
    }
    VD_TRY(vd_gemm_tn_acc(d, out, x, in, Gp(m, name + ".W"), in, (int)out, (int)in, (int)M, 0, s));
    VD_TRY(vd_colsum_acc(d, out, (int)M, (int)out, Gp(m, name + ".b"), s));
    if (dx_out) *dx_out = nullptr;
    if (need_dx) {
      float* dx;
      VD_TRY(ws_get(m, name + ".dx", (size_t)M * in, &dx));
      VD_TRY(vd_gemm_nn(d, out, Wp(m, name + ".W"), in, nullptr, dx, in, (int)M, (int)in, (int)out, 0, s));
      if (dx_out) *dx_out = dx;
    }
    return VD_OK;
  }
};

struct CatLinear {
  std::string name;
  std::vector<long> dims;
  long D = 0, H = 0, N = 0;
  Linear lin;
  const uint8_t* mask = nullptr;
  float scale = 1.f;
  void init(const std::string& n, const std::vector<long>& d, long H_) {
    name = n; dims = d; H = H_; D = 0;
    for (long v : d) D += v;
    lin.init(n, D, H_);
  }
  int forward(vd_model* m, hipStream_t s, const std::vector<const float*>& parts, long N_, const uint8_t* mask_, float scale_,
              float** y) {
    N = N_; mask = mask_; scale = scale_;
    float* cat;
    VD_TRY(ws_get(m, name + ".cat", (size_t)N * D, &cat));
    long off = 0;
    for (size_t i = 0; i < dims.size(); ++i) {
      VD_TRY(vd_copy_2d(cat + off, D, parts[i], dims[i], N, dims[i], s));
      off += dims[i];
    }
    const float* catd;
    VD_TRY(dropout_fwd(m, name + ".in", cat, mask, scale, N * D, s, &catd));
    return lin.forward(m, s, catd, N, true, y);
  }
  int backward(vd_model* m, hipStream_t s, const float* dy, const std::vector<bool>& need, std::vector<float*>* out) {
    float* dcatd;
    VD_TRY(lin.backward(m, s, dy, true, &dcatd));
    const float* dcat;
    VD_TRY(dropout_fwd(m, name + ".din", dcatd, mask, scale, N * D, s, &dcat));
    out->assign(dims.size(), nullptr);
    long off = 0;
    for (size_t i = 0; i < dims.size(); ++i) {
      if (need.empty() || need[i]) {
        float* g;
        VD_TRY(ws_get(m, name + ".dpart" + std::to_string(i), (size_t)N * dims[i], &g));
// ... 188 lines not shown
```

### visdial_amd/csrc/rt_decoders.h

```cpp
#pragma once
#include "rt_encoders.h"

namespace vdrt {

int option_cache_resolve(vd_model* m, BatchSlot& sl, const int32_t* options, long NO, int To, hipStream_t s);

struct Decoder {
  virtual ~Decoder() {}
  virtual void declare(vd_model* m) = 0;
  virtual int forward_backward(vd_model* m, BatchSlot& b, bool only_forward) = 0;
  virtual int retrieve(vd_model* m, BatchSlot& b) = 0;
  virtual int retrieve_lhood(vd_model*, BatchSlot&) {
    vd_set_error("vd_model_retrieve_lhood: the live-row log-likelihood head scores candidates of decoder 'gen'; this model's decoder is 'disc'");
    return VD_ERR_ARG;
  }
  virtual int gen_begin(vd_model*, const int32_t*, int) { return no_gen(); }
  virtual int gen_step(vd_model*, const int32_t*, float*) { return no_gen(); }
  virtual int gen_select(vd_model*, const int32_t*, int) { return no_gen(); }
  virtual int gen_beam_search(vd_model*, int, int, int, int, int32_t*, double*) { return no_gen(); }
  virtual int gen_sample(vd_model*, int, int, int, double, const double*, int32_t*, double*) { return no_gen(); }
  static int no_gen() {
    vd_set_error("sampling / beam search only for the generative decoder (model.lua:436-438)");
    return VD_ERR_STATE;
  }
};

inline int stage_loss(vd_model* m, const float* loss_rows, long n, bool is_sum, hipStream_t s) {
  if (m->loss_cap < n) {
    if (m->loss_host) VD_HIP(hipHostFree(m->loss_host));
    m->loss_host = nullptr;
    VD_HIP(hipHostMalloc((void**)&m->loss_host, (size_t)n * sizeof(float), hipHostMallocDefault));
    m->loss_cap = n;
  }
  m->loss_n = n;
  m->loss_is_sum = is_sum;
  VD_HIP(hipMemcpyAsync(m->loss_host, loss_rows, (size_t)n * sizeof(float), hipMemcpyDeviceToHost, s));
  VD_HIP(hipEventRecord(m->ev_loss, s));
  return VD_OK;
}

#ifdef VD_PROBE_PHASES
inline hipEvent_t* probe_events() {
  static hipEvent_t e[6];
  static bool made = false;
  if (!made) { for (auto& x : e) (void)hipEventCreate(&x); made = true; }
  return e;
}
#define VD_PROBE_REC(i, stream) (void)hipEventRecord(probe_events()[i], stream)
#else
#define VD_PROBE_REC(i, stream)
#endif
struct Disc : Decoder {
  void declare(vd_model* m) override { add_lstm(m, "opt", m->p.embedSize, m->p.rnnHiddenSize); }
  int forward_backward(vd_model* m, BatchSlot& b, bool only_forward) override {
    VD_CHECK_ARG(b.opt.present, "decoder 'disc' needs batch.options");
    VD_CHECK_ARG(only_forward || b.has_gt, "training decoder 'disc' needs batch.answer_ind");
    if (b.cached) return forward_cached(m, b, only_forward);
    const int N = b.q.N, O = m->p.numOptions, NOfull = N * O, NO = b.opt.N, To = b.opt.T;
    const bool dedup = b.opt_uid != nullptr;
    VD_CHECK_ARG(dedup ? NO <= NOfull : NO == NOfull, "decoder 'disc': %d option rows for %d x %d candidates", NO, N, O);
    const long H = m->p.rnnHiddenSize, E = m->p.embedSize, V = m->p.vocabSize;
    hipStream_t s = m->s_main;
    hipStream_t se = side_stream(m, m->s_enc, s);
    hipStream_t st = side_stream(m, m->s_tab, s);
    float *table, *gates, *h, *c, *scores, *loss_rows;
    VD_TRY(ws_get(m, "opt.table", (size_t)(V + 1) * 4 * H, &table));
    VD_TRY(ws_get(m, "opt.gates", (size_t)To * NO * 4 * H, &gates));
    VD_TRY(ws_get(m, "opt.h", (size_t)To * NO * H, &h));
    VD_TRY(ws_get(m, "opt.c", (size_t)To * NO * H, &c));
    VD_TRY(ws_get(m, "opt.scores", (size_t)N * O, &scores));
    VD_TRY(ws_get(m, "crit.loss_rows", (size_t)N, &loss_rows));
    float* Wopt = Wp(m, "opt.W");
    const int flags = m->flags;
    VD_TRY(fork_stream(m, s, se));
    float* enc_out = nullptr;
    VD_TRY(vd_gemm_nn(Wp(m, "embed"), E, Wopt, 4 * H, Wp(m, "opt.b"), table, 4 * H, (int)V + 1, (int)(4 * H), (int)E, 0, s));
    const bool c16 = (flags & VD_FLAG_BF16) && vd_lstm_c16_fits(NO, (int)H);
    vd_bf16_bits *gates16 = reinterpret_cast<vd_bf16_bits*>(gates), *h16 = reinterpret_cast<vd_bf16_bits*>(h), *table16 = nullptr;
    float* h_last = nullptr;
    if (c16) {
      float* t16;
      VD_TRY(ws_get(m, "opt.table16", (size_t)(V + 1) * 2 * H, &t16));
      VD_TRY(ws_get(m, "opt.h_last", (size_t)NO * H, &h_last));
      table16 = reinterpret_cast<vd_bf16_bits*>(t16);
      VD_TRY(vd_f32_to_bf16(table, table16, (V + 1) * 4 * H, s));
    }
    VD_HIP(hipEventRecord(m->ev_prof[0], s));
    {
      VdRange r("disc: option LSTM forward");
      if (c16) VD_TRY(vd_lstm_forward_c16(table16, 4 * H, b.opt.tok, Wopt + E * 4 * H, gates16, h16, h_last, c, To, NO, (int)H, s));
      else VD_TRY(vd_lstm_forward(table, 0, 4 * H, b.opt.tok, nullptr, Wopt + E * 4 * H, nullptr, nullptr, gates, h, c, To, NO, (int)H, flags, s));
    }
    VD_HIP(hipEventRecord(m->ev_prof[1], s));
    {
      VdRange r("encoder forward");
      VD_TRY(m->enc->forward(m, se, b, &enc_out));
      VD_PROBE_REC(0, se);
    }
    VD_TRY(join_stream(m, se, s));
    const float* optH = c16 ? h_last : h + (long)(To - 1) * NO * H;
    float *d_optH = nullptr, *d_enc = nullptr, *d_optH_full = nullptr;
    if (dedup) {
      float* full;
      VD_TRY(ws_get(m, "opt.h_full", (size_t)NOfull * H, &full));
      VD_TRY(vd_embed_gather(optH, b.opt_uid, nullptr, full, NOfull, (int)H, 1.f, s));
      optH = full;
    }
    if (!only_forward) {
      VD_TRY(ws_get(m, "crit.d_optH", (size_t)NO * H, &d_optH));
      VD_TRY(ws_get(m, "crit.d_enc", (size_t)N * H, &d_enc));
      if (dedup) VD_TRY(ws_get(m, "crit.d_optH_full", (size_t)NOfull * H, &d_optH_full));
    }
    VD_TRY(vd_score_ce(optH, enc_out, b.gt, scores, loss_rows, dedup ? d_optH_full : d_optH, d_enc, N, O, (int)H, 1.0f / N, s));
    if (dedup && !only_forward) {
      VD_TRY(vd_memset(d_optH, 0, (long)NO * H * 4, s));
      VD_TRY(vd_embed_scatter_acc(d_optH, b.opt_uid, nullptr, d_optH_full, NOfull, (int)H, 1.f, s));
    }
    VD_TRY(stage_loss(m, loss_rows, N, false, s));
    m->scores = scores;
    m->prof_valid = !only_forward;
    if (only_forward) return VD_OK;
    VD_TRY(fork_stream(m, s, se));
    float *dc, *dtab;
    int32_t* perm = b.opt_sort_perm;
    VD_TRY(ws_get(m, "opt.dc", (size_t)NO * H, &dc));
    VD_TRY(ws_get(m, "opt.dtable", (size_t)(V + 1) * 4 * H, &dtab));
    VD_CHECK_ARG(perm, "decoder 'disc': the batch slot carries no option-token sort");
    VD_TRY(fork_stream(m, s, st));
    VD_TRY(vd_memset(dtab, 0, (V + 1) * 4 * H * 4, st));
    VD_HIP(hipEventRecord(m->ev_prof[2], s));
    m->wg_active = m->streams && m->s_wg && (flags & VD_FLAG_BF16) != 0;
    m->wg_used = false;
    auto enc_bwd = [&]() -> int {
      VdRange r("encoder backward");
      VD_TRY(m->enc->backward(m, se, b, d_enc));
      VD_PROBE_REC(1, se);
      if (m->wg_used) VD_PROBE_REC(2, m->s_wg);
      if (m->wg_used) {
        VD_TRY(fork_stream(m, se, m->s_wg));
        VD_HIP(hipEventRecord(m->ev_enc_grads, m->s_wg));
      } else {
        VD_HIP(hipEventRecord(m->ev_enc_grads, se));
      }
      m->enc_grads_recorded = true;
      return VD_OK;
    };
    {
      VdRange r("disc: option LSTM backward");
      if (c16) VD_TRY(vd_lstm_backward_c16(Wopt + E * 4 * H, gates16, c, d_optH, dc, To, NO, (int)H, s));
      else VD_TRY(vd_lstm_backward(Wopt + E * 4 * H, gates, c, nullptr, nullptr, d_optH, nullptr, dc, nullptr, nullptr, nullptr, To, NO, (int)H, flags, s));
    }
    VD_HIP(hipEventRecord(m->ev_prof[3], s));
    VD_TRY(enc_bwd());
    VdRange rwg("disc: table gradient + dWh");
    VD_TRY(fork_stream(m, s, st));
    if (c16) VD_TRY(vd_segment_rowsum_acc_bf16(gates16, 4 * H, b.opt.tok, perm, (long)To * NO, (int)(4 * H), dtab, 4 * H, st));
    else VD_TRY(vd_segment_rowsum_acc(gates, 4 * H, b.opt.tok, perm, (long)To * NO, (int)(4 * H), dtab, 4 * H, st));
    VD_TRY(vd_colsum_acc(dtab, 4 * H, (int)V + 1, (int)(4 * H), Gp(m, "opt.b"), st));
    VD_TRY(vd_gemm_tn_acc(Wp(m, "embed"), E, dtab, 4 * H, Gp(m, "opt.W"), 4 * H, (int)E, (int)(4 * H), (int)V + 1, 0, st));
    VD_HIP(hipEventRecord(m->ev_prof[4], s));
    if (To > 1 && c16)
      VD_TRY(vd_gemm_tn_acc_bf16(h16, gates16 + (long)NO * 4 * H, Gp(m, "opt.W") + E * 4 * H, 4 * H, (int)H, (int)(4 * H), (To - 1) * NO, s));
    else if (To > 1)
      VD_TRY(vd_gemm_tn_acc(h, H, gates + (long)NO * 4 * H, 4 * H, Gp(m, "opt.W") + E * 4 * H, 4 * H, (int)H, (int)(4 * H), (To - 1) * NO,
                            flags & (VD_FLAG_BF16 | VD_FLAG_SPLIT9), s));
    VD_HIP(hipEventRecord(m->ev_prof[5], s));
    VD_TRY(vd_gemm_nt(dtab, 4 * H, Wopt, 4 * H, nullptr, Gp(m, "embed"), E, (int)V + 1, (int)E, (int)(4 * H), VD_ACT_NONE, 2, st));
    VD_PROBE_REC(3, st);
    VD_TRY(join_stream(m, se, s));
    if (m->wg_used) VD_TRY(join_stream(m, m->s_wg, s));
    m->wg_active = m->wg_used = false;
    VD_TRY(join_stream(m, st, s));
    VD_PROBE_REC(4, s);
    return VD_OK;
  }
  int retrieve(vd_model* m, BatchSlot& b) override { return forward_backward(m, b, true); }

  int forward_cached(vd_model* m, BatchSlot& b, bool only_forward) {
    if (!only_forward || m->training) {
      vd_set_error("decoder 'disc': this batch was uploaded for cached evaluation (VD_OPTION_CACHE with training off) and carries only the "
                   "candidate rows the cache did not hold; upload it again after vd_model_set_training(1) for a training step");
      return VD_ERR_STATE;
    }
    OptionCache& oc = m->ocache;
    const int N = b.q.N, O = m->p.numOptions, NOfull = N * O, To = b.opt.T;
    const long H = m->p.rnnHiddenSize, E = m->p.embedSize, V = m->p.vocabSize;
    hipStream_t s = m->s_main;
    hipStream_t se = side_stream(m, m->s_enc, s);
    if (b.cache_stamp != oc.stamp) {
      VD_HIP(hipEventSynchronize(b.ready));
      VD_TRY(option_cache_resolve(m, b, b.opt_host.data(), NOfull, To, s));
      VD_HIP(hipStreamSynchronize(s));
    }
    const int U = b.opt.N;
    const long count = oc.index.size();
    VD_CHECK_ARG(b.opt_total == NOfull && (long)b.miss_keys.size() == (long)U * To && count <= oc.capacity,
                 "decoder 'disc': inconsistent cached batch (%d candidates, %d misses)", b.opt_total, U);
    if (oc.table_rows < count + U) {
      const long want = std::min(std::max(2 * oc.table_rows, VD_OPTION_CACHE_FIRST_ROWS), oc.capacity);
      const long rows = std::max(want, count + U);
      float* nt = nullptr;
      VD_HIP(hipMalloc((void**)&nt, (size_t)rows * H * sizeof(float)));
      if (oc.table) {
        if (count > 0) VD_HIP(hipMemcpyAsync(nt, oc.table, (size_t)count * H * sizeof(float), hipMemcpyDeviceToDevice, s));
        VD_HIP(hipStreamSynchronize(s));
        VD_HIP(hipFree(oc.table));
      }
      oc.table = nt;
      oc.table_rows = rows;
    }
    float *scores, *loss_rows, *full;
    VD_TRY(ws_get(m, "opt.scores", (size_t)N * O, &scores));
    VD_TRY(ws_get(m, "crit.loss_rows", (size_t)N, &loss_rows));
    VD_TRY(ws_get(m, "opt.h_full", (size_t)NOfull * H, &full));
    VD_TRY(fork_stream(m, s, se));
    if (U > 0) {
      VdRange r("disc: option LSTM forward (state only, cache misses)");
      float *table, *h, *c;
      VD_TRY(ws_get(m, "opt.table", (size_t)(V + 1) * 4 * H, &table));
      VD_TRY(ws_get(m, "opt.h2", (size_t)2 * U * H, &h));
      VD_TRY(ws_get(m, "opt.c2", (size_t)2 * U * H, &c));
      float* Wopt = Wp(m, "opt.W");
      VD_TRY(vd_gemm_nn(Wp(m, "embed"), E, Wopt, 4 * H, Wp(m, "opt.b"), table, 4 * H, (int)V + 1, (int)(4 * H), (int)E, 0, s));
      VD_TRY(vd_lstm_forward(table, 0, 4 * H, b.opt.tok, nullptr, Wopt + E * 4 * H, nullptr, nullptr, nullptr, h, c, To, U, (int)H,
                             m->flags | VD_FLAG_STATE_ONLY, s));
      VD_HIP(hipMemcpyAsync(oc.table + count * H, h + (long)((To - 1) & 1) * U * H, (size_t)U * H * sizeof(float), hipMemcpyDeviceToDevice, s));
      const long fit = std::min<long>(U, oc.capacity - count);
      for (long i = 0; i < fit; ++i) oc.index.add(b.miss_keys.data() + (size_t)i * To);
    }
    ++oc.stamp;
    float* enc_out = nullptr;
    {
      VdRange r("encoder forward");
      VD_TRY(m->enc->forward(m, se, b, &enc_out));
    }
    VD_TRY(join_stream(m, se, s));
    VD_TRY(vd_embed_gather(oc.table, b.opt_uid, nullptr, full, NOfull, (int)H, 1.f, s));
    VD_TRY(vd_score_ce(full, enc_out, b.gt, scores, loss_rows, nullptr, nullptr, N, O, (int)H, 1.0f / N, s));
    VD_TRY(stage_loss(m, loss_rows, N, false, s));
    m->scores = scores;
    m->prof_valid = false;
    return VD_OK;
  }
};

struct Gen;
int Gen_begin(Gen* g, vd_model* m, const int32_t* rounds, int n);
int Gen_step(Gen* g, vd_model* m, const int32_t* tokens, float* host_logp);
int Gen_select(Gen* g, vd_model* m, const int32_t* src, int n_keep);
int Gen_beam_search(Gen* g, vd_model* m, int k, int L, int start, int end, int32_t* host_tokens, double* host_scores);
int Gen_sample(Gen* g, vd_model* m, int L, int start, int end, double T, const double* host_u, int32_t* host_tokens,
               double* host_loglik);

struct Gen : Decoder {
  int gen_begin(vd_model* m, const int32_t* r, int n) override { return Gen_begin(this, m, r, n); }
  int gen_step(vd_model* m, const int32_t* t, float* lp) override { return Gen_step(this, m, t, lp); }
  int gen_select(vd_model* m, const int32_t* src, int k) override { return Gen_select(this, m, src, k); }
  int gen_beam_search(vd_model* m, int k, int L, int st, int en, int32_t* t, double* sc) override {
    return Gen_beam_search(this, m, k, L, st, en, t, sc);
  }
  int gen_sample(vd_model* m, int L, int st, int en, double T, const double* u, int32_t* t, double* ll) override {
    return Gen_sample(this, m, L, st, en, T, u, t, ll);
  }
  std::vector<SeqLSTM> rnn;
  long E = 0, H = 0, V = 0, Vp = 0;
  int gen_n = 0;
  void declare(vd_model* m) override {
    E = m->p.embedSize; H = m->p.rnnHiddenSize; V = m->p.vocabSize; Vp = (V + 3) / 4 * 4;
    rnn.resize(m->p.numLayers);
    for (int l = 0; l < m->p.numLayers; ++l) {
      add_lstm(m, "dec" + std::to_string(l + 1), l == 0 ? E : H, H);
      rnn[l].init("dec" + std::to_string(l + 1), l == 0 ? E : H, H);
    }
    add_linear(m, "vocab", H, V);
  }
  int forwardConnect(vd_model* m, hipStream_t s, const float* encOut, int seqLen, const int32_t* rep, long rows) {
    auto put = [&](const float* x, const std::string& key, const float** dst) -> int {
      if (!rep) {
        *dst = x;
        return VD_OK;
      }
      float* r;
      VD_TRY(ws_get(m, key, (size_t)rows * H, &r));
      VD_TRY(vd_embed_gather(x, rep, nullptr, r, rows, (int)H, 1.f, s));
      *dst = r;
      return VD_OK;
    };
    std::vector<SeqLSTM>* layers = m->enc->rnnLayers();
    if (layers) {
      for (size_t i = 0; i < layers->size(); ++i) {
        VD_TRY(put((*layers)[i].out_at(seqLen - 1), "ret.h0_" + std::to_string(i), &rnn[i].userPrevOutput));
        VD_TRY(put((*layers)[i].cell_at(seqLen - 1), "ret.c0_" + std::to_string(i), &rnn[i].userPrevCell));
      }
      return put(encOut, "ret.enc", &rnn[layers->size() - 1].userPrevOutput);
    }
    return put(encOut, "ret.enc", &rnn.back().userPrevOutput);
  }
  const float* backwardConnect(vd_model* m) {
    std::vector<SeqLSTM>* layers = m->enc->rnnLayers();
    if (layers) {
      const size_t n = rnn.size();
      for (size_t i = 0; i < n; ++i) {
        (*layers)[i].userNextGradCell = rnn[i].userGradPrevCell;
        if (i != n - 1) (*layers)[i].gradPrevOutput = rnn[i].userGradPrevOutput;
      }
      return rnn[layers->size() - 1].userGradPrevOutput;
    }
    return rnn.back().userGradPrevOutput;
  }
  int forward_backward(vd_model* m, BatchSlot& b, bool only_forward) override {
    VD_CHECK_ARG(b.ain.present && b.aout.present, "decoder 'gen' needs batch.answer_in / answer_out");
    hipStream_t s = m->s_main;
    const int N = b.q.N, Ta = b.ain.T;
    const long rows = (long)Ta * N;
    float* encOut;
    {
      VdRange r("encoder forward");
      VD_TRY(m->enc->forward(m, s, b, &encOut));
    }
    VdRange rdec("gen: decoder forward + criterion + backward");
    VD_TRY(forwardConnect(m, s, encOut, m->enc->seqLen(b), nullptr, N));
    float *x, *h, *logits, *loss_rows;
    VD_TRY(ws_get(m, "dec.x", (size_t)rows * E, &x));
    VD_TRY(ws_get(m, "dec.logits", (size_t)rows * Vp, &logits));
    VD_TRY(ws_get(m, "dec.loss_rows", (size_t)rows, &loss_rows));
    VD_TRY(vd_embed_gather(Wp(m, "embed"), b.ain.tok, nullptr, x, rows, (int)E, 1.f, s));
    VD_TRY(lstm_stack_forward(m, s, rnn, {x}, Ta, N, b.ain.tok, &h));
    m->prof_valid = false;
    m->prof_hist = false;
    VD_HIP(hipEventRecord(m->ev_prof[4], s));
    VD_TRY(vd_gemm_nt(h, H, Wp(m, "vocab.W"), H, Wp(m, "vocab.b"), logits, Vp, (int)rows, (int)V, (int)H, VD_ACT_NONE, 0, s));
    VD_TRY(vd_logsoftmax_nll(logits, Vp, rows, (int)V, b.ain.tok, b.aout.tok, loss_rows, only_forward ? 0 : 1, s));
    VD_TRY(stage_loss(m, loss_rows, rows, true, s));
    if (only_forward) return VD_OK;
    float* dh;
    VD_TRY(ws_get(m, "dec.dh", (size_t)rows * H, &dh));
    VD_TRY(vd_gemm_tn_acc(logits, Vp, h, H, Gp(m, "vocab.W"), H, (int)V, (int)H, (int)rows, 0, s));
    VD_TRY(vd_colsum_acc(logits, Vp, (int)rows, (int)V, Gp(m, "vocab.b"), s));
    VD_TRY(vd_gemm_nn(logits, Vp, Wp(m, "vocab.W"), H, nullptr, dh, H, (int)rows, (int)H, (int)V, 0, s));
    VD_HIP(hipEventRecord(m->ev_prof[5], s));
    std::vector<float*> dx;
    VD_TRY(lstm_stack_backward(m, s, rnn, nullptr, dh, &dx));
    VD_TRY(vd_embed_scatter_acc(Gp(m, "embed"), b.ain.tok, nullptr, dx[0], rows, (int)E, 1.f, s));
    const float* gradDecOut = backwardConnect(m);
    VD_CHECK_ARG(gradDecOut, "backwardConnect produced no gradient");
    {
      VdRange r("encoder backward");
      VD_TRY(m->enc->backward(m, s, b, gradDecOut));
    }
    VD_HIP(hipEventRecord(m->ev_enc_grads, s));
    m->enc_grads_recorded = true;
    m->prof_valid = m->prof_hist;
    return VD_OK;
  }
  int retrieve(vd_model* m, BatchSlot& b) override { return retrieve_head(m, b, false); }
  int retrieve_lhood(vd_model* m, BatchSlot& b) override {
    if (m->lhood_tree && b.tree_ok) return retrieve_tree(m, b);
    return retrieve_head(m, b, true);
  }
  int retrieve_tree(vd_model* m, BatchSlot& b) {
    VD_CHECK_ARG(b.oin.present && b.oout.present, "retrieval with decoder 'gen' needs batch.option_in / option_out");
    hipStream_t s = m->s_main;
    const int N = b.q.N, O = m->p.numOptions, T = b.oin.T;
    float* encOut;
    VD_TRY(m->enc->forward(m, s, b, &encOut));
    const int seqLen = m->enc->seqLen(b);
    float *lhood, *table;
    VD_TRY(ws_get(m, "ret.lhood", (size_t)N * O, &lhood));
    VD_TRY(ws_get(m, "ret.table", (size_t)(V + 1) * 4 * H, &table));
    VD_TRY(vd_gemm_nn(Wp(m, "embed"), E, rnn[0].Wx(m), 4 * H, Wp(m, rnn[0].name + ".b"), table, 4 * H, (int)V + 1, (int)(4 * H), (int)E, 0, s));
    m->lhood_exec = 0;
    m->lhood_total = (long)T * N * O;
    for (const TreeChunk& tc : b.tree) {
      const long rows = (long)N * tc.C;
      const long tile = vd_lstm_fwd_row_tile(tc.Nw);
      for (int t = 0; t < tc.Tl; ++t) m->lhood_exec += std::min<long>(tc.Nw, (tc.widths[t] + tile - 1) / tile * tile);
      float *h = nullptr, *lse;
      VD_TRY(ws_get(m, "ret.lse", (size_t)std::max<long>(1, tc.n_nodes), &lse));
      if (tc.Tl > 0) {
        VD_TRY(forwardConnect(m, s, encOut, seqLen, nullptr, N));
        VD_TRY(rnn[0].forward_tree(m, s, table, nullptr, tc.Tl, tc.Nw, N, tc.mask2, &h));
        for (size_t l = 1; l < rnn.size(); ++l) VD_TRY(rnn[l].forward_tree(m, s, nullptr, h, tc.Tl, tc.Nw, N, tc.mask2, &h));
        VD_TRY(vd_lhood_lse_p(h, H, (long)tc.Tl * tc.Nw, tc.node_row, tc.n_nodes, Wp(m, "vocab.W"), H, Wp(m, "vocab.b"), (int)V, (int)H, lse, s));
      }
      VD_TRY(vd_lhood_edge_sum_p(h, H, tc.node_row, lse, tc.enode, tc.etgt, tc.Tl, rows, tc.C, Wp(m, "vocab.W"), H, Wp(m, "vocab.b"), (int)H,
                                 lhood + tc.o0, O, s));
    }
    m->scores = lhood;
    m->prof_valid = false;
    return VD_OK;
  }
  int retrieve_head(vd_model* m, BatchSlot& b, bool live) {
    VD_CHECK_ARG(b.oin.present && b.oout.present, "retrieval with decoder 'gen' needs batch.option_in / option_out");
    hipStream_t s = m->s_main;
    const int N = b.q.N, O = m->p.numOptions, T = b.oin.T;
    float* encOut;
    VD_TRY(m->enc->forward(m, s, b, &encOut));
    const int seqLen = m->enc->seqLen(b);
    float* lhood;
    VD_TRY(ws_get(m, "ret.lhood", (size_t)N * O, &lhood));
    const long per_opt = (long)T * N * (live ? E + 6 * H * (long)rnn.size() : Vp);
    const int oc = (int)std::max<long>(1, std::min<long>(O, (1L << 30) / std::max<long>(1, per_opt)));
    const bool ordered = live && vd_lhood_prefix_fits(T, (long)N * std::min(O, oc));
    float* table = nullptr;
    if (ordered) {
      VD_TRY(ws_get(m, "ret.table", (size_t)(V + 1) * 4 * H, &table));
      VD_TRY(vd_gemm_nn(Wp(m, "embed"), E, rnn[0].Wx(m), 4 * H, Wp(m, rnn[0].name + ".b"), table, 4 * H, (int)V + 1, (int)(4 * H), (int)E, 0, s));
    }
    if (live) {
      m->lhood_exec = 0;
      m->lhood_total = (long)T * N * O;
    }
    for (int o0 = 0; o0 < O; o0 += oc) {
      const int C = std::min(O, o0 + oc) - o0;
      const long rows = (long)N * C;
      int32_t *cin, *cout, *idx;
      VD_TRY(ws_get(m, "ret.cin", (size_t)T * rows, &cin));
      VD_TRY(ws_get(m, "ret.cout", (size_t)T * rows, &cout));
      VD_TRY(vd_copy_2d((float*)cin, C, (const float*)(b.oin.tok + o0), O, (long)T * N, C, s));
      VD_TRY(vd_copy_2d((float*)cout, C, (const float*)(b.oout.tok + o0), O, (long)T * N, C, s));
      float *x, *h, *logits, *nll, *acc;
      VD_TRY(ws_get(m, "ret.nll", (size_t)T * rows, &nll));
      if (ordered) {
        int32_t *perm, *cin_s, *cout_s, *owork, *info, *act, *work, n_act = 0;
        void* info_host;
        VD_TRY(ws_get(m, "ret.perm", (size_t)rows, &perm));
        VD_TRY(ws_get(m, "ret.rep", (size_t)rows, &idx));
        VD_TRY(ws_get(m, "ret.cin_s", (size_t)T * rows, &cin_s));
        VD_TRY(ws_get(m, "ret.cout_s", (size_t)T * rows, &cout_s));
        VD_TRY(ws_get(m, "ret.order_work", (size_t)vd_lhood_order_work_ints(T, rows), &owork));
        VD_TRY(ws_get(m, "ret.order_info", (size_t)T + 1, &info));
        VD_TRY(pin_get(b.pinned, "ret.order_info", ((size_t)T + 1) * sizeof(int32_t), &info_host));
        VD_TRY(ws_get(m, "ret.act", (size_t)T * rows, &act));
        VD_TRY(ws_get(m, "ret.act_work", (size_t)(T * rows + 1023) / 1024 + 1, &work));
        VD_TRY(vd_lhood_order_p(cin, cout, T, rows, C, perm, idx, cin_s, cout_s, owork, info, s));
        VD_HIP(hipMemcpyAsync(info_host, info, ((size_t)T + 1) * sizeof(int32_t), hipMemcpyDeviceToHost, s));
        VD_TRY(vd_lhood_live_rows(cin_s, cout_s, T * rows, act, work, &n_act, s));
        const int32_t* hinfo = static_cast<const int32_t*>(info_host);
        const int flags = hinfo[0] ? 0 : VD_FLAG_LIVE_PREFIX;
        int Tl = T;
        long ran = (long)T * rows;
        if (flags) {
          const long tile = vd_lstm_fwd_row_tile(rows);
          Tl = 1;
          ran = 0;
          for (int t = 0; t < T; ++t) {
            if (hinfo[1 + t] > 0) Tl = t + 1;
            ran += std::min<long>(rows, (hinfo[1 + t] + tile - 1) / tile * tile);
          }
        }
        m->lhood_exec += ran;
        VD_TRY(forwardConnect(m, s, encOut, seqLen, idx, rows));
        VD_TRY(rnn[0].forward_ordered(m, s, table, nullptr, Tl, (int)rows, cin_s, flags, &h));
        for (size_t l = 1; l < rnn.size(); ++l) VD_TRY(rnn[l].forward_ordered(m, s, nullptr, h, Tl, (int)rows, cin_s, flags, &h));
        VD_TRY(vd_lhood_nll(h, H, Tl * rows, act, n_act, cout_s,
                             Wp(m, "vocab.W"), H, Wp(m, "vocab.b"), (int)V, (int)H, nll, s));
        VD_TRY(vd_lhood_sum_p(nll, act, n_act, T, rows, C, perm, lhood + o0, O, s));
        continue;
      }
      std::vector<int32_t> hidx(rows);
      for (long r = 0; r < rows; ++r) hidx[r] = (int32_t)(r / C);
      VD_TRY(index_array(m, "idx.ret." + std::to_string(rows) + "." + std::to_string(C), hidx, &idx));
      VD_TRY(forwardConnect(m, s, encOut, seqLen, idx, rows));
      VD_TRY(ws_get(m, "ret.x", (size_t)T * rows * E, &x));
      VD_TRY(vd_embed_gather(Wp(m, "embed"), cin, nullptr, x, T * rows, (int)E, 1.f, s));
      VD_TRY(lstm_stack_forward(m, s, rnn, {x}, T, (int)rows, cin, &h));
// ... 246 lines not shown
```

### visdial_amd/csrc/runtime.hip

```cpp
#include "rt_decoders.h"

using namespace vdrt;

vd_model::~vd_model() {}

namespace {

int upload_tokens(BatchSlot& sl, SeqTok& ss, const std::string& tag, const int32_t* rows_major, int N, int T, bool sorted, hipStream_t s) {
  ss.T = T;
  ss.N = N;
  ss.present = true;
  ss.sorted = sorted;
  const size_t TN = (size_t)T * N;
  const size_t total = sorted ? 7 * TN + 2 * (size_t)N + T : TN;
  int32_t* stage = nullptr;
  VD_TRY(pin_get(sl.pinned, tag + ".stage", total * sizeof(int32_t), (void**)&stage));
  int32_t* tok = stage;
  std::vector<int> len(sorted ? N : 0);
  for (int n = 0; n < N; ++n) {
    int first = T;
    for (int t = 0; t < T; ++t) {
      const int32_t v = rows_major[(size_t)n * T + t];
      tok[(size_t)t * N + n] = v;
      if (v != 0 && first == T) first = t;
    }
    if (sorted) len[n] = T - first;
  }
  if (sorted) {
    int32_t* tok_sorted = stage + TN;
    int32_t* fwd_idx = stage + 2 * TN;
    int32_t* inv_idx = stage + 3 * TN;
    int32_t* perm = stage + 4 * TN;
    int32_t* inv = perm + N;
    int32_t* nact = inv + N;
    std::vector<int> order(N);
    std::iota(order.begin(), order.end(), 0);
    std::stable_sort(order.begin(), order.end(), [&](int a, int b) { return len[a] > len[b]; });
    for (int i = 0; i < N; ++i) {
      perm[i] = order[i];
      inv[order[i]] = i;
    }
    ss.nact.assign(T, 0);
    for (int t = 0; t < T; ++t) {
      int c = 0;
      for (int n = 0; n < N; ++n) c += len[n] >= T - t;
      ss.nact[t] = c;
      nact[t] = c;
      for (int i = 0; i < N; ++i) {
        tok_sorted[(size_t)t * N + i] = tok[(size_t)t * N + perm[i]];
        fwd_idx[(size_t)t * N + i] = t * N + perm[i];
        inv_idx[(size_t)t * N + i] = t * N + inv[i];
      }
    }
    int32_t* act = nact + T;
    int na = 0;
    for (int t = 0; t < T; ++t)
      for (int i = 0; i < ss.nact[t]; ++i) act[na++] = t * N + i;
    const int n0 = T > 0 ? ss.nact[0] : 0;
    int32_t* prev1 = act + TN;
    for (int k = n0; k < na; ++k) prev1[k - n0] = act[k] - N;
    ss.n_act = na;
    ss.n_act1 = na - n0;
  }
  int32_t* dev = nullptr;
  VD_TRY(dev_get(sl.bufs, tag + ".dev", total * sizeof(int32_t), (void**)&dev));
  VD_HIP(hipMemcpyAsync(dev, stage, total * sizeof(int32_t), hipMemcpyHostToDevice, s));
  ss.tok = dev;
  if (sorted) {
    ss.tok_sorted = dev + TN;
    ss.fwd_idx = dev + 2 * TN;
    ss.inv_idx = dev + 3 * TN;
    ss.perm = dev + 4 * TN;
    ss.inv = ss.perm + N;
    ss.nact_dev = ss.inv + N;
    ss.act = ss.nact_dev + T;
    ss.act1 = ss.act + (T > 0 ? ss.nact[0] : 0);
    ss.prev1 = ss.act + TN;
  }
  return VD_OK;
}

bool has(const std::string& s, const char* sub) { return s.find(sub) != std::string::npos; }

}

int vdrt::option_cache_resolve(vd_model* m, BatchSlot& sl, const int32_t* options, long NO, int To, hipStream_t s) {
  OptionCache& oc = m->ocache;
  if (oc.index.T != To) {
    oc.index.reset(To);
    ++oc.stamp;
  }
  const int32_t count = oc.index.size();
  RowIndex miss;
  miss.reset(To);
  int32_t* up = nullptr;
  VD_TRY(pin_get(sl.pinned, "opt.uid.stage", (size_t)NO * sizeof(int32_t), (void**)&up));
  for (long r = 0; r < NO; ++r) {
    const int32_t* row = options + (size_t)r * To;
    int32_t u = oc.index.find(row);
    if (u < 0) {
      int32_t l = miss.find(row);
      if (l < 0) l = miss.add(row);
      u = count + l;
    }
    up[r] = u;
  }
  const int U = miss.size();
  sl.miss_keys.swap(miss.keys);
  sl.cached = true;
  sl.cache_stamp = oc.stamp;
  sl.opt_total = (int)NO;
  if (U > 0) {
    VD_TRY(upload_tokens(sl, sl.opt, "opt", sl.miss_keys.data(), U, To, false, s));
  } else {
    sl.opt.T = To;
    sl.opt.N = 0;
    sl.opt.present = true;
    sl.opt.sorted = false;
    sl.opt.tok = nullptr;
  }
  VD_TRY(dev_get(sl.bufs, "opt.uid", (size_t)NO * sizeof(int32_t), (void**)&sl.opt_uid));
  VD_HIP(hipMemcpyAsync(sl.opt_uid, up, (size_t)NO * sizeof(int32_t), hipMemcpyHostToDevice, s));
  sl.opt_sort_off = sl.opt_sort_perm = nullptr;
  return VD_OK;
}

struct TreeHost {
  int Tl = 0, Nw = 0;
  long n_nodes = 0;
  std::vector<int32_t> widths, enode, etgt;
  std::vector<std::vector<int32_t>> tok, par;
};

static void tree_build_range(const int32_t* oin, const int32_t* oout, int N, int O, int T, int o0, int C, TreeHost& th) {
  const long rows = (long)N * C;
  std::vector<int32_t> cur((size_t)rows);
  std::vector<uint8_t> alive((size_t)rows, 1);
  for (long r = 0; r < rows; ++r) cur[r] = (int32_t)(r / C);
  th = TreeHost();
  th.enode.assign((size_t)T * rows, 0);
  th.etgt.assign((size_t)T * rows, 0);
  std::vector<uint64_t> keys;
  std::vector<int32_t> vals;
  for (int t = 0; t < T; ++t) {
    long cnt = 0;
    for (long r = 0; r < rows; ++r) {
      if (alive[r] && oin[((size_t)(r / C) * O + o0 + r % C) * T + t] == 0) alive[r] = 0;
      cnt += alive[r];
    }
    if (cnt == 0) break;
    size_t cap = 16;
    while (cap < 2 * (size_t)cnt) cap <<= 1;
    keys.assign(cap, ~0ull);
    vals.assign(cap, -1);
    std::vector<int32_t> ltok, lpar;
    for (long r = 0; r < rows; ++r) {
      if (!alive[r]) continue;
      const size_t src = ((size_t)(r / C) * O + o0 + r % C) * T + t;
      const uint64_t key = ((uint64_t)(uint32_t)cur[r] << 32) | (uint32_t)oin[src];
      size_t pos = (size_t)((key * 0x9E3779B97F4A7C15ull) >> 20) & (cap - 1);
      while (keys[pos] != ~0ull && keys[pos] != key) pos = (pos + 1) & (cap - 1);
      if (keys[pos] == ~0ull) {
        keys[pos] = key;
        vals[pos] = (int32_t)ltok.size();
        ltok.push_back(oin[src]);
        lpar.push_back(cur[r]);
      }
      cur[r] = vals[pos];
      if (oout[src] != 0) {
        th.enode[(size_t)t * rows + r] = (int32_t)(th.n_nodes + cur[r]);
        th.etgt[(size_t)t * rows + r] = oout[src];
      }
    }
    th.widths.push_back((int32_t)ltok.size());
    th.n_nodes += (long)ltok.size();
    th.Nw = std::max<int>(th.Nw, (int)ltok.size());
    th.tok.push_back(std::move(ltok));
    th.par.push_back(std::move(lpar));
    th.Tl = t + 1;
  }
}

static bool tree_chunk_fits(const TreeHost& th, long H, long layers) {
  const long slots = (long)th.Tl * th.Nw;
  return slots * (2 * H * layers + 4 * H * (layers - 1)) <= (1L << 30) && slots * H * 4 < (1L << 32) && (long)th.Nw * 4 * H * 4 < (1L << 32) &&
         slots < (1L << 31);
}

static int tree_chunks(vd_model* m, BatchSlot& sl, const int32_t* oin, const int32_t* oout, int N, int O, int T, int o0, int C, hipStream_t s) {
  TreeHost th;
  tree_build_range(oin, oout, N, O, T, o0, C, th);
  if (!tree_chunk_fits(th, m->p.rnnHiddenSize, m->p.numLayers) && C > 1) {
    VD_TRY(tree_chunks(m, sl, oin, oout, N, O, T, o0, C / 2, s));
    return tree_chunks(m, sl, oin, oout, N, O, T, o0 + C / 2, C - C / 2, s);
  }
  TreeChunk tc;
  tc.o0 = o0; tc.C = C; tc.Tl = th.Tl; tc.Nw = th.Nw; tc.n_nodes = th.n_nodes; tc.widths = th.widths;
  const size_t slots = (size_t)th.Tl * th.Nw, edges = (size_t)T * N * C;
  const size_t total = 2 * slots + (size_t)th.n_nodes + 2 * edges;
  const std::string tag = "tree." + std::to_string(sl.tree.size());
  int32_t *stage = nullptr, *dev = nullptr;
  VD_TRY(pin_get(sl.pinned, tag + ".stage", total * sizeof(int32_t), (void**)&stage));
  VD_TRY(dev_get(sl.bufs, tag, total * sizeof(int32_t), (void**)&dev));
  memset(stage, 0, 2 * slots * sizeof(int32_t));
  int32_t* nr = stage + 2 * slots;
  for (int t = 0; t < th.Tl; ++t) {
    const size_t w = th.tok[t].size();
    memcpy(stage + (size_t)t * th.Nw, th.tok[t].data(), w * sizeof(int32_t));
    memcpy(stage + slots + (size_t)t * th.Nw, th.par[t].data(), w * sizeof(int32_t));
    for (size_t n = 0; n < w; ++n) *nr++ = (int32_t)((size_t)t * th.Nw + n);
  }
  memcpy(nr, th.enode.data(), edges * sizeof(int32_t));
  memcpy(nr + edges, th.etgt.data(), edges * sizeof(int32_t));
  if (total) VD_HIP(hipMemcpyAsync(dev, stage, total * sizeof(int32_t), hipMemcpyHostToDevice, s));
  tc.mask2 = dev;
  tc.node_row = dev + 2 * slots;
  tc.enode = tc.node_row + th.n_nodes;
  tc.etgt = tc.enode + edges;
  sl.tree.push_back(std::move(tc));
  return VD_OK;
}

static int build_lhood_tree(vd_model* m, BatchSlot& sl, const int32_t* oin, const int32_t* oout, int N, int O, int T, hipStream_t s) {
  sl.tree.clear();
  sl.tree_ok = false;
  const long V = m->p.vocabSize;
  for (size_t r = 0; r < (size_t)N * O; ++r) {
    bool run = true;
    for (int t = 0; t < T; ++t) {
      const int32_t a = oin[r * T + t], b = oout[r * T + t];
      if (a < 0 || a > V || b < 0 || b > V || (a != 0 && !run)) return VD_OK;
      run = run && a != 0;
    }
  }
  VD_TRY(tree_chunks(m, sl, oin, oout, N, O, T, 0, O, s));
  sl.tree_ok = true;
  return VD_OK;
}

extern "C" {

int vd_model_create(const vd_model_params* p, const char* encoder, const char* decoder, vd_model** out) {
  VD_CHECK_ARG(p && encoder && decoder && out, "vd_model_create: null argument");
  std::unique_ptr<Encoder> enc = make_encoder(encoder);
  std::unique_ptr<Decoder> dec = make_decoder(decoder);
  if (!enc || !dec) {
    vd_set_error("vd_model_create: unknown plug-in pair '%s' + '%s' (encoders: lf-ques, lf-ques-im, lf-ques-hist, lf-ques-im-hist, "
                 "lf-att-ques-im-hist, hre-ques-hist, hre-ques-im-hist, hrea-ques-im-hist, mn-ques-hist, mn-ques-im-hist, "
                 "mn-att-ques-im-hist; decoders: disc, gen)", encoder, decoder);
    return VD_ERR_ARG;
  }
  const std::string en(encoder);
  const bool use_im = has(en, "im"), is_att = has(en, "att") && !has(en, "hrea");
  VD_CHECK_ARG(p->rnnHiddenSize > 0 && p->rnnHiddenSize % 32 == 0 && p->embedSize > 0 && p->embedSize % 4 == 0 && p->vocabSize > 0 &&
                   p->maxQuesCount > 0 && p->numOptions > 0,
               "vd_model_create: rnnHiddenSize must be a positive multiple of 32, embedSize of 4; vocabSize, maxQuesCount, numOptions > 0");
  VD_CHECK_ARG(((long)p->vocabSize + 1) * 4 * p->rnnHiddenSize * 4 < (1L << 32),
               "vd_model_create: (vocabSize + 1) x 4 x rnnHiddenSize floats exceed 4 GB");
  VD_CHECK_ARG(!use_im || (p->imgFeatureSize > 0 && p->imgFeatureSize % 4 == 0), "vd_model_create: imgFeatureSize must be a positive multiple of 4");
  VD_CHECK_ARG(!is_att || (p->commonEmbeddingSize > 0 && p->commonEmbeddingSize % 4 == 0 && p->imgSpatialSize > 0),
               "vd_model_create: commonEmbeddingSize must be a positive multiple of 4 and imgSpatialSize > 0 for attention encoders");
  VD_CHECK_ARG(!(has(en, "hre") && use_im) || (p->imgEmbedSize > 0 && p->imgEmbedSize % 4 == 0),
               "vd_model_create: imgEmbedSize must be a positive multiple of 4 for hre*-ques-im-hist");
  VD_CHECK_ARG(p->dropout >= 0.f && p->dropout < 1.f, "vd_model_create: dropout must lie in [0, 1)");
  const int flags = vd_precision_flags(p->lstmBf16);
  VD_CHECK_ARG(flags >= 0, "vd_model_create: lstmBf16 must be 0, 1, 3, 6 or 9 (got %d)", p->lstmBf16);
  long cache_rows = 0;
  if (const char* e = getenv("VD_OPTION_CACHE")) {
    const long v = atol(e);
    cache_rows = v <= 0 ? 0 : v == 1 ? VD_OPTION_CACHE_DEFAULT_ROWS : v;
  }
  VD_CHECK_ARG(!cache_rows || std::string(decoder) == "disc",
               "vd_model_create: VD_OPTION_CACHE caches the candidate encodings of decoder 'disc'; this model's decoder is '%s'", decoder);
  VD_CHECK_ARG(!cache_rows || p->lstmBf16 != 1,
               "vd_model_create: VD_OPTION_CACHE needs the state-only option recurrence, which the compact bf16 recurrence (lstmBf16 = 1) "
               "does not have");
  VD_CHECK_ARG(cache_rows < (1L << 30), "vd_model_create: VD_OPTION_CACHE = %ld rows is out of range", cache_rows);
  bool lhood_tree = false;
  if (const char* e = getenv("VD_LHOOD_TREE")) lhood_tree = atol(e) > 0;
  VD_CHECK_ARG(!lhood_tree || std::string(decoder) == "gen",
               "vd_model_create: VD_LHOOD_TREE scores the candidates of decoder 'gen' over a prefix tree; this model's decoder is '%s'", decoder);
  VD_CHECK_ARG(!lhood_tree || p->lstmBf16 != 1,
               "vd_model_create: VD_LHOOD_TREE runs the exact fp32 tree recurrence (VD_FLAG_TREE), which the compact bf16 recurrence "
               "(lstmBf16 = 1) does not have");
  vd_model* m = new vd_model();
  m->p = *p;
  m->flags = flags;
  m->ocache.capacity = cache_rows;
  m->lhood_tree = lhood_tree;
  if (m->p.numAttentionLayers < 1 || has(en, "lf-att")) m->p.numAttentionLayers = 1;
  if (m->p.numLayers < 1) m->p.numLayers = 2;
  m->enc_name = encoder;
  m->dec_name = decoder;
  m->use_im = use_im;
  m->use_hist = has(en, "hist");
  m->is_att = is_att;
  m->is_graph = en.rfind("mn", 0) == 0 || en.rfind("lf-att", 0) == 0;
  m->lr = p->learningRate;
  m->streams = p->useStreams != 0;
  m->enc = std::move(enc);
  m->dec = std::move(dec);
  m->spec.push_back(Tensor{"embed", 0, p->vocabSize + 1, p->embedSize, 0});
  m->enc->declare(m);
  m->dec->declare(m);
  long off = 0;
  for (size_t i = 0; i < m->spec.size(); ++i) {
    m->spec[i].off = off;
    m->index[m->spec[i].name] = (int)i;
    off += (m->spec[i].numel() + 3) / 4 * 4;
  }
  m->numel = off;
  auto fail = [&](int rc) {
    vd_model_destroy(m);
    return rc;
  };
  for (float** v : {&m->W, &m->G, &m->M, &m->V}) {
    if (hipMalloc((void**)v, off * sizeof(float)) != hipSuccess) {
      vd_set_error("vd_model_create: hipMalloc of %ld floats failed", off);
      return fail(VD_ERR_HIP);
    }
    (void)hipMemset(*v, 0, off * sizeof(float));
  }
  int least = 0, greatest = 0;
  (void)hipDeviceGetStreamPriorityRange(&least, &greatest);
  if (hipStreamCreateWithPriority(&m->s_main, hipStreamNonBlocking, least) != hipSuccess) return fail(VD_ERR_HIP);
  for (hipStream_t* s : {&m->s_enc, &m->s_img, &m->s_copy})
    if (hipStreamCreateWithPriority(s, hipStreamNonBlocking, greatest) != hipSuccess) return fail(VD_ERR_HIP);
  const int tab_prio = greatest;
  if (hipStreamCreateWithPriority(&m->s_tab, hipStreamNonBlocking, tab_prio) != hipSuccess) return fail(VD_ERR_HIP);
  if (least - greatest >= 2 &&
      hipStreamCreateWithPriority(&m->s_wg, hipStreamNonBlocking, (least + greatest) / 2) != hipSuccess)
    return fail(VD_ERR_HIP);
  m->s_hist = m->s_img;
  m->ev_pool.resize(64);
  for (auto& e : m->ev_pool)
    if (hipEventCreateWithFlags(&e, hipEventDisableTiming) != hipSuccess) return fail(VD_ERR_HIP);
  if (hipEventCreateWithFlags(&m->ev_loss, hipEventDisableTiming) != hipSuccess) return fail(VD_ERR_HIP);
  if (hipEventCreateWithFlags(&m->ev_enc_grads, hipEventDisableTiming) != hipSuccess) return fail(VD_ERR_HIP);
  if (hipEventCreateWithFlags(&m->ev_updated, hipEventDisableTiming) != hipSuccess) return fail(VD_ERR_HIP);
  for (auto& e : m->ev_prof)
    if (hipEventCreate(&e) != hipSuccess) return fail(VD_ERR_HIP);
  for (auto& sl : m->slot)
    if (hipEventCreateWithFlags(&sl.ready, hipEventDisableTiming) != hipSuccess ||
        hipEventCreateWithFlags(&sl.done, hipEventDisableTiming) != hipSuccess)
      return fail(VD_ERR_HIP);
  *out = m;
  return VD_OK;
}

void vd_model_destroy(vd_model* m) {
  if (!m) return;
  (void)hipDeviceSynchronize();
  for (float* v : {m->W, m->G, m->M, m->V})
    if (v) (void)hipFree(v);
  for (auto& kv : m->ws)
    if (kv.second.p) (void)hipFree(kv.second.p);
  for (auto& kv : m->ext_masks)
    if (kv.second.p) (void)hipFree(kv.second.p);
  if (m->ocache.table) (void)hipFree(m->ocache.table);
  for (auto& sl : m->slot) {
    for (auto& kv : sl.bufs)
      if (kv.second.p) (void)hipFree(kv.second.p);
    for (auto& kv : sl.pinned)
      if (kv.second.p) (void)hipHostFree(kv.second.p);
    if (sl.ready) (void)hipEventDestroy(sl.ready);
    if (sl.done) (void)hipEventDestroy(sl.done);
  }
  if (m->loss_host) (void)hipHostFree(m->loss_host);
  for (auto& e : m->ev_pool)
    if (e) (void)hipEventDestroy(e);
  if (m->ev_loss) (void)hipEventDestroy(m->ev_loss);
  if (m->ev_enc_grads) (void)hipEventDestroy(m->ev_enc_grads);
  if (m->ev_updated) (void)hipEventDestroy(m->ev_updated);
  for (auto& e : m->ev_prof)
    if (e) (void)hipEventDestroy(e);
  for (hipStream_t s : {m->s_main, m->s_enc, m->s_img, m->s_tab, m->s_copy, m->s_wg})
    if (s) {
      (void)hipStreamDestroy(s);
    }
  delete m;
}

int64_t vd_model_num_tensors(const vd_model* m) { return m ? (int64_t)m->spec.size() : 0; }
int64_t vd_model_flat_size(const vd_model* m) { return m ? m->numel : 0; }

int vd_model_tensor_info(const vd_model* m, int64_t i, char* name64, int64_t* offset, int64_t* rows, int64_t* cols) {
  VD_CHECK_ARG(m && i >= 0 && i < (int64_t)m->spec.size(), "vd_model_tensor_info: bad index");
  const Tensor& t = m->spec[i];
  if (name64) {
    strncpy(name64, t.name.c_str(), 63);
    name64[63] = 0;
  }
  if (offset) *offset = t.off;
  if (rows) *rows = t.rows;
  if (cols) *cols = t.cols;
  return VD_OK;
}

int vd_model_flat_pointers(vd_model* m, float** W, float** dW, float** adam_m, float** adam_v) {
  VD_CHECK_ARG(m, "vd_model_flat_pointers: null model");
  m->ocache.flush();
  if (W) *W = m->W;
  if (dW) *dW = m->G;
  if (adam_m) *adam_m = m->M;
  if (adam_v) *adam_v = m->V;
  return VD_OK;
}

void* vd_model_stream(vd_model* m) { return m ? (void*)m->s_main : nullptr; }

int vd_model_encoder_range(const vd_model* m, int64_t* lo, int64_t* hi) {
  VD_CHECK_ARG(m && lo && hi, "vd_model_encoder_range: null");
  const char* first_dec = m->dec_name == "disc" ? "opt.W" : "dec1.W";
  *lo = m->spec[1].off;
  *hi = m->spec[m->index.at(first_dec)].off;
  return VD_OK;
}
int vd_model_wait_encoder_grads(vd_model* m, void* stream) {
  VD_CHECK_ARG(m && m->enc_grads_recorded, "vd_model_wait_encoder_grads: no backward pass has been enqueued");
  VD_HIP(hipStreamWaitEvent((hipStream_t)stream, m->ev_enc_grads, 0));
  return VD_OK;
}

int vd_model_init_params(vd_model* m, uint64_t seed) {
  VD_CHECK_ARG(m, "vd_model_init_params: null model");
  std::mt19937_64 rng(seed);
  std::vector<float> host((size_t)m->numel, 0.f);
  const long H = m->p.rnnHiddenSize;
  for (const Tensor& t : m->spec) {
    float* w = host.data() + t.off;
    const long n = t.numel();
    if (t.kind == 0) {
      std::normal_distribution<float> nd(0.f, 1.f);
      for (long i = t.cols; i < n; ++i) w[i] = nd(rng);
    } else if (t.kind == 1) {
      std::normal_distribution<float> nd(0.f, 1.f / sqrtf((float)t.rows));
      for (long i = 0; i < n; ++i) w[i] = nd(rng);
    } else if (t.kind == 2) {
      for (long i = H; i < 2 * H; ++i) w[i] = 1.f;
    } else {
      const long in = t.kind == 3 ? t.cols : m->spec[m->index.at(t.name.substr(0, t.name.size() - 2) + ".W")].cols;
      const float s = 1.f / sqrtf((float)in);
      std::uniform_real_distribution<float> ud(-s, s);
      for (long i = 0; i < n; ++i) w[i] = ud(rng);
    }
  }
  VD_HIP(hipMemcpy(m->W, host.data(), host.size() * sizeof(float), hipMemcpyHostToDevice));
  m->ocache.flush();
  return VD_OK;
}

int vd_model_set_tensor(vd_model* m, const char* name, const float* host, int64_t n) {
  VD_CHECK_ARG(m && name && host && m->index.count(name), "vd_model_set_tensor: unknown tensor '%s'", name ? name : "(null)");
  const Tensor& t = m->spec[m->index.at(name)];
  VD_CHECK_ARG(n == t.numel(), "vd_model_set_tensor: '%s' holds %ld values, got %ld", name, t.numel(), (long)n);
  VD_HIP(hipStreamSynchronize(m->s_main));
  VD_HIP(hipMemcpy(m->W + t.off, host, n * sizeof(float), hipMemcpyHostToDevice));
  m->ocache.flush();
  return VD_OK;
}

int vd_model_get_tensor(vd_model* m, const char* name, int which, float* host, int64_t n) {
  VD_CHECK_ARG(m && name && host && m->index.count(name), "vd_model_get_tensor: unknown tensor '%s'", name ? name : "(null)");
  const Tensor& t = m->spec[m->index.at(name)];
  VD_CHECK_ARG(n == t.numel() && which >= 0 && which <= 3, "vd_model_get_tensor: bad size / selector");
  VD_HIP(hipStreamSynchronize(m->s_main));
  float* base[4] = {m->W, m->G, m->M, m->V};
  VD_HIP(hipMemcpy(host, base[which] + t.off, n * sizeof(float), hipMemcpyDeviceToHost));
  return VD_OK;
}

int vd_model_set_training(vd_model* m, int on) {
  VD_CHECK_ARG(m, "vd_model_set_training: null model");
  m->training = on != 0;
  if (on) m->ocache.flush();
  return VD_OK;
}

int vd_model_set_dropout_mask(vd_model* m, const char* site, const uint8_t* host, int64_t n) {
  VD_CHECK_ARG(m, "vd_model_set_dropout_mask: null model");
  VD_HIP(hipStreamSynchronize(m->s_main));
  if (!host) {
    for (auto& kv : m->ext_masks)
      if (kv.second.p) VD_HIP(hipFree(kv.second.p));
    m->ext_masks.clear();
    return VD_OK;
  }
  VD_CHECK_ARG(site && n > 0, "vd_model_set_dropout_mask: bad arguments");
  void* p = nullptr;
  VD_TRY(dev_get(m->ext_masks, site, (size_t)n, &p));
  VD_HIP(hipMemcpy(p, host, (size_t)n, hipMemcpyHostToDevice));
  return VD_OK;
}

int vd_model_upload_batch(vd_model* m, const vd_batch* hb) {
  VD_CHECK_ARG(m && hb && hb->ques_fwd && hb->B > 0 && hb->Tq > 0, "vd_model_upload_batch: missing ques_fwd / B / Tq");
  VD_CHECK_ARG(!m->use_hist || (hb->hist && hb->Th > 0), "vd_model_upload_batch: encoder '%s' needs hist", m->enc_name.c_str());
  VD_CHECK_ARG(!m->use_im || hb->img_feat, "vd_model_upload_batch: encoder '%s' needs img_feat", m->enc_name.c_str());
  const bool disc = m->dec_name == "disc";
  VD_CHECK_ARG(!disc || (hb->options && hb->To > 0), "vd_model_upload_batch: decoder 'disc' needs options");
  VdRange r("vd_model_upload_batch");
  BatchSlot& sl = m->slot[m->cur < 0 ? 0 : (m->cur ^ 1)];
  hipStream_t s = m->s_copy;
  if (sl.used) VD_HIP(hipStreamWaitEvent(s, sl.done, 0));
  if (sl.uploaded) VD_HIP(hipEventSynchronize(sl.ready));
  sl.uploaded = true;
  sl.B = hb->B;
  const int R = m->p.maxQuesCount, N = hb->B * R, O = m->p.numOptions;
  const long NO = (long)N * O;
  for (SeqTok* t : {&sl.q, &sl.h, &sl.opt, &sl.ain, &sl.aout, &sl.oin, &sl.oout}) t->present = false;
  VD_TRY(upload_tokens(sl, sl.q, "q", hb->ques_fwd, N, hb->Tq, m->is_graph, s));
  const bool hist_wave = !m->is_graph && m->p.numLayers == 2;
  if (m->use_hist) VD_TRY(upload_tokens(sl, sl.h, "h", hb->hist, N, hb->Th, m->is_graph || hist_wave, s));
  if (m->use_im) {
    const size_t img_n = (size_t)hb->B * (m->is_att ? (size_t)m->p.imgSpatialSize * m->p.imgSpatialSize : 1) * m->p.imgFeatureSize;
    float* ip = nullptr;
    VD_TRY(pin_get(sl.pinned, "img.stage", img_n * sizeof(float), (void**)&ip));
    memcpy(ip, hb->img_feat, img_n * sizeof(float));
    VD_TRY(dev_get(sl.bufs, "img", img_n * sizeof(float), (void**)&sl.img));
    VD_HIP(hipMemcpyAsync(sl.img, ip, img_n * sizeof(float), hipMemcpyHostToDevice, s));
  }
  if (disc) {
    sl.opt_uid = nullptr;
    sl.opt_total = (int)NO;
    sl.cached = false;
    const int To = hb->To;
    bool dedup = false;
    if (m->ocache.capacity > 0 && !m->training) {
      sl.opt_host.assign(hb->options, hb->options + (size_t)NO * To);
      VD_TRY(option_cache_resolve(m, sl, sl.opt_host.data(), NO, To, s));
    } else if (NO > 1) {
      std::vector<int32_t> uid((size_t)NO), uniq;
      uniq.reserve((size_t)NO * To);
      const size_t cap = (size_t)1 << (64 - __builtin_clzll((unsigned long long)(2 * NO)));
      std::vector<int32_t> table(cap, -1);
      int U = 0;
      for (long r = 0; r < NO; ++r) {
        const int32_t* row = hb->options + (size_t)r * To;
        uint64_t h = 1469598103934665603ull;
        for (int t = 0; t < To; ++t) h = (h ^ (uint32_t)row[t]) * 1099511628211ull;
        size_t pos = (size_t)(h ^ (h >> 29)) & (cap - 1);
        for (;;) {
          const int32_t u = table[pos];
          if (u < 0) {
            table[pos] = U;
            uid[r] = U++;
            uniq.insert(uniq.end(), row, row + To);
            break;
          }
          if (memcmp(uniq.data() + (size_t)u * To, row, (size_t)To * sizeof(int32_t)) == 0) {
            uid[r] = u;
            break;
          }
          pos = (pos + 1) & (cap - 1);
        }
      }
      if ((double)U <= 0.95 * (double)NO) {
        dedup = true;
        VD_TRY(upload_tokens(sl, sl.opt, "opt", uniq.data(), U, To, false, s));
        int32_t* up = nullptr;
        VD_TRY(pin_get(sl.pinned, "opt.uid.stage", (size_t)NO * sizeof(int32_t), (void**)&up));
        memcpy(up, uid.data(), (size_t)NO * sizeof(int32_t));
        VD_TRY(dev_get(sl.bufs, "opt.uid", (size_t)NO * sizeof(int32_t), (void**)&sl.opt_uid));
        VD_HIP(hipMemcpyAsync(sl.opt_uid, up, (size_t)NO * sizeof(int32_t), hipMemcpyHostToDevice, s));
      }
    }
    if (!dedup && !sl.cached) VD_TRY(upload_tokens(sl, sl.opt, "opt", hb->options, (int)NO, hb->To, false, s));
    sl.opt_sort_off = sl.opt_sort_perm = nullptr;
    if (!sl.cached) {
      const long V1 = (long)m->p.vocabSize + 1, n = (long)sl.opt.T * sl.opt.N;
      int32_t* work;
      VD_TRY(dev_get(sl.bufs, "opt.sort_off", (size_t)(V1 + 1) * sizeof(int32_t), (void**)&sl.opt_sort_off));
      VD_TRY(dev_get(sl.bufs, "opt.sort_work", (size_t)2 * V1 * sizeof(int32_t), (void**)&work));
      VD_TRY(dev_get(sl.bufs, "opt.sort_perm", (size_t)n * sizeof(int32_t), (void**)&sl.opt_sort_perm));
      VD_TRY(vd_token_sort(sl.opt.tok, n, (int)V1, sl.opt_sort_off, work, sl.opt_sort_perm, s));
    }
  }
  if (!disc && hb->answer_in && hb->answer_out) {
    VD_TRY(upload_tokens(sl, sl.ain, "ain", hb->answer_in, N, hb->Ta, false, s));
    VD_TRY(upload_tokens(sl, sl.aout, "aout", hb->answer_out, N, hb->Ta, false, s));
  }
  sl.tree_ok = false;
  if (!disc && hb->option_in && hb->option_out) {
    VD_TRY(upload_tokens(sl, sl.oin, "oin", hb->option_in, (int)NO, hb->To, false, s));
    VD_TRY(upload_tokens(sl, sl.oout, "oout", hb->option_out, (int)NO, hb->To, false, s));
    if (m->lhood_tree) VD_TRY(build_lhood_tree(m, sl, hb->option_in, hb->option_out, N, O, hb->To, s));
  }
  sl.has_gt = hb->answer_ind != nullptr;
  sl.gt_host.assign(N, 0);
  int32_t* gp = nullptr;
  VD_TRY(pin_get(sl.pinned, "gt.stage", (size_t)N * sizeof(int32_t), (void**)&gp));
  for (int n = 0; n < N; ++n) {
    const int g = hb->answer_ind ? hb->answer_ind[n] - 1 : 0;
    VD_CHECK_ARG(!hb->answer_ind || (g >= 0 && g < O), "vd_model_upload_batch: answer_ind[%d] = %d out of 1..%d", n, g + 1, O);
    sl.gt_host[n] = g;
    gp[n] = g;
  }
  VD_TRY(dev_get(sl.bufs, "gt", (size_t)N * sizeof(int32_t), (void**)&sl.gt));
  VD_HIP(hipMemcpyAsync(sl.gt, gp, (size_t)N * sizeof(int32_t), hipMemcpyHostToDevice, s));
  VD_HIP(hipEventRecord(sl.ready, s));
  m->uploaded = (int)(&sl - m->slot);
  m->lhood_exec = -1;
  return VD_OK;
}

static int begin_step(vd_model* m, bool zero_grads, BatchSlot** out) {
  VD_CHECK_ARG(m && m->uploaded >= 0, "no batch uploaded");
  m->cur = m->uploaded;
  m->enc_grads_recorded = false;
  m->lhood_exec = -1;
  BatchSlot& b = m->slot[m->cur];
  m->N = b.q.N;
  m->O = m->p.numOptions;
  hipStream_t s = m->s_main;
  VD_HIP(hipStreamWaitEvent(s, b.ready, 0));
  if (zero_grads) VD_TRY(vd_memset(m->G, 0, m->numel * 4, s));
  VD_TRY(vd_memset(Wp(m, "embed"), 0, (long)m->p.embedSize * 4, s));
  b.used = true;
  *out = &b;
  return VD_OK;
}

int vd_model_forward_backward(vd_model* m, int only_forward) {
  VdRange r(only_forward ? "vd_model_forward" : "vd_model_forward_backward");
  BatchSlot* b = nullptr;
  VD_TRY(begin_step(m, !only_forward, &b));
  if (!only_forward) m->ocache.flush();
  const int rc = m->dec->forward_backward(m, *b, only_forward != 0);
  VD_HIP(hipEventRecord(b->done, m->s_main));
  return rc;
}

int vd_model_retrieve(vd_model* m) {
  VdRange r("vd_model_retrieve");
  BatchSlot* b = nullptr;
  VD_TRY(begin_step(m, false, &b));
  const int rc = m->dec->retrieve(m, *b);
  VD_HIP(hipEventRecord(b->done, m->s_main));
  return rc;
}

int vd_model_retrieve_lhood(vd_model* m) {
  VdRange r("vd_model_retrieve_lhood");
  BatchSlot* b = nullptr;
  VD_TRY(begin_step(m, false, &b));
  const int rc = m->dec->retrieve_lhood(m, *b);
  VD_HIP(hipEventRecord(b->done, m->s_main));
  return rc;
}

int vd_model_encode(vd_model* m) {
  BatchSlot* b = nullptr;
  VD_TRY(begin_step(m, false, &b));
  m->gen_enc_out = nullptr;
  float* out = nullptr;
  const int rc = m->enc->forward(m, m->s_main, *b, &out);
  VD_HIP(hipEventRecord(b->done, m->s_main));
  if (rc == VD_OK) {
    m->gen_enc_out = out;
    m->gen_seq_len = m->enc->seqLen(*b);
  }
  return rc;
}
int vd_model_decode_begin(vd_model* m, const int32_t* rounds, int n) {
  VD_CHECK_ARG(m, "vd_model_decode_begin: null model");
  return m->dec->gen_begin(m, rounds, n);
}
int vd_model_decode_step(vd_model* m, const int32_t* tokens, float* host_logprobs) {
  VD_CHECK_ARG(m, "vd_model_decode_step: null model");
  return m->dec->gen_step(m, tokens, host_logprobs);
}
int vd_model_decode_select(vd_model* m, const int32_t* src, int n_keep) {
  VD_CHECK_ARG(m, "vd_model_decode_select: null model");
  return m->dec->gen_select(m, src, n_keep);
}
int vd_model_beam_search(vd_model* m, int beam_size, int beam_len, int start_token, int end_token, int32_t* host_tokens,
                         double* host_scores) {
  VD_CHECK_ARG(m, "vd_model_beam_search: null model");
  VdRange r("vd_model_beam_search");
  return m->dec->gen_beam_search(m, beam_size, beam_len, start_token, end_token, host_tokens, host_scores);
}
int vd_model_sample(vd_model* m, int beam_len, int start_token, int end_token, double temperature, const double* host_uniforms,
                    int32_t* host_tokens, double* host_loglik) {
  VD_CHECK_ARG(m, "vd_model_sample: null model");
  VdRange r("vd_model_sample");
  return m->dec->gen_sample(m, beam_len, start_token, end_token, temperature, host_uniforms, host_tokens, host_loglik);
}

int vd_model_loss(vd_model* m, float* loss) {
  VD_CHECK_ARG(m && loss && m->cur >= 0 && m->loss_n > 0, "vd_model_loss: nothing to read");
  VD_HIP(hipEventSynchronize(m->ev_loss));
  double s = 0;
  for (long i = 0; i < m->loss_n; ++i) s += m->loss_host[i];
  *loss = (float)(m->loss_is_sum ? s : s / (double)m->loss_n);
  return VD_OK;
}

int vd_model_update(vd_model* m, float gscale) {
  VD_CHECK_ARG(m, "vd_model_update: null model");
  VdRange r("vd_model_update: clamp + adam");
  m->adam_t += 1;
  m->ocache.flush();
  const double t = m->adam_t;
  const float step = (float)(m->lr * sqrt(1.0 - pow(0.999, t)) / (1.0 - pow(0.9, t)));
  VD_TRY(vd_clamp_adam(m->W, m->G, m->M, m->V, m->numel, gscale, 5.0f, 0.9f, 0.999f, 1e-8f, step, m->s_main));
  VD_HIP(hipEventRecord(m->ev_updated, m->s_main));
  m->updated_recorded = true;
  if (m->lr > m->p.minLRate) m->lr *= m->p.lrDecayRate;
  m->step += 1;
  return VD_OK;
}

int vd_model_learning_rate(vd_model* m, double* lr, int set) {
  VD_CHECK_ARG(m && lr, "vd_model_learning_rate: null");
  if (set) m->lr = *lr;
  else *lr = m->lr;
  return VD_OK;
}

int vd_model_scores(vd_model* m, float* host, int64_t n) {
  VD_CHECK_ARG(m && host && m->cur >= 0 && m->scores && n == (int64_t)m->N * m->O, "vd_model_scores: no scores / bad size");
  VD_HIP(hipStreamSynchronize(m->s_main));
  VD_HIP(hipMemcpy(host, m->scores, n * sizeof(float), hipMemcpyDeviceToHost));
  return VD_OK;
}

int vd_model_ranks(vd_model* m, int use_gt, int32_t* ranks_out) {
  VD_CHECK_ARG(m && ranks_out && m->cur >= 0 && m->scores, "vd_model_ranks: nothing to rank");
  const int N = m->N, O = m->O;
  const BatchSlot& b = m->slot[m->cur];
  VD_CHECK_ARG(!use_gt || b.has_gt, "vd_model_ranks: the batch carries no answer_ind");
  int32_t* ranks;
  VD_TRY(ws_get(m, "opt.ranks", (size_t)N * O, &ranks));
  VD_TRY(vd_ranks(m->scores, ranks, N, O, m->s_main));
  std::vector<int32_t> host((size_t)N * O);
  VD_HIP(hipMemcpyAsync(host.data(), ranks, host.size() * sizeof(int32_t), hipMemcpyDeviceToHost, m->s_main));
  VD_HIP(hipStreamSynchronize(m->s_main));
  if (use_gt) {
    for (int n = 0; n < N; ++n) ranks_out[n] = host[(size_t)n * O + b.gt_host[n]];
  } else {
    memcpy(ranks_out, host.data(), host.size() * sizeof(int32_t));
  }
  return VD_OK;
}

int vd_model_family_ms(vd_model* m, float* ms3) {
  VD_CHECK_ARG(m && ms3, "vd_model_family_ms: null");
  ms3[0] = ms3[1] = ms3[2] = 0.f;
  if (!m->prof_valid) return VD_OK;
  VD_HIP(hipStreamSynchronize(m->s_main));
  VD_HIP(hipEventElapsedTime(&ms3[0], m->ev_prof[0], m->ev_prof[1]));
  VD_HIP(hipEventElapsedTime(&ms3[1], m->ev_prof[2], m->ev_prof[3]));
  VD_HIP(hipEventElapsedTime(&ms3[2], m->ev_prof[4], m->ev_prof[5]));
#ifdef VD_PROBE_PHASES
  { float t[12]; hipEvent_t* pe = vdrt::probe_events();
    for (int i = 1; i < 6; ++i) (void)hipEventElapsedTime(&t[i], m->ev_prof[0], m->ev_prof[i]);
    for (int i = 0; i < 5; ++i) (void)hipEventElapsedTime(&t[6 + i], m->ev_prof[0], pe[i]);
    fprintf(stderr, "PHASES (ms after option-fwd start) main: fwd end %.2f | bwd %.2f -> %.2f | dWh %.2f -> %.2f | all joined %.2f  ||  enc fwd end %.2f | enc bwd chain end %.2f | "
            "wg chain end %.2f | table chain end %.2f\n", t[1], t[2], t[3], t[4], t[5], t[10], t[6], t[7], t[8], t[9]); }
#endif
  return VD_OK;
}

int vd_model_option_rows(vd_model* m, int64_t* executed, int64_t* total) {
  VD_CHECK_ARG(m && executed && total && (m->cur >= 0 || m->uploaded >= 0), "vd_model_option_rows: no batch uploaded");
  if (m->lhood_exec >= 0) {
    *executed = m->lhood_exec;
    *total = m->lhood_total;
    return VD_OK;
  }
  const BatchSlot& b = m->slot[m->cur >= 0 ? m->cur : m->uploaded];
  *executed = b.opt.present ? b.opt.N : 0;
  *total = b.opt.present ? (b.opt_total ? b.opt_total : b.opt.N) : 0;
  return VD_OK;
}

int vd_model_synchronize(vd_model* m) {
  VD_CHECK_ARG(m, "vd_model_synchronize: null model");
  for (hipStream_t s : {m->s_copy, m->s_enc, m->s_img, m->s_tab, m->s_wg, m->s_main})
    if (s) VD_HIP(hipStreamSynchronize(s));
  return VD_OK;
}

}
```

### visdial_amd/csrc/split_core.h

```cpp
#pragma once
#include "gemm_core.h"
#include "paths.h"

typedef __bf16 vd_bf16x8 __attribute__((ext_vector_type(8)));
typedef float vd_f32x4 __attribute__((ext_vector_type(4)));

__device__ __forceinline__ void vd_split3(const float4& u, const float4& w, vd_bf16x8& hi, vd_bf16x8& mid, vd_bf16x8& lo) {
  const float v[8] = {u.x, u.y, u.z, u.w, w.x, w.y, w.z, w.w};
#pragma unroll
  for (int i = 0; i < 8; ++i) {
    const __bf16 h = (__bf16)v[i];
    const float r1 = v[i] - (float)h;
    const __bf16 m = (__bf16)r1;
    const float r2 = r1 - (float)m;
    hi[i] = h; mid[i] = m; lo[i] = (__bf16)r2;
  }
}

static __global__ void __launch_bounds__(256) f32_to_bf16x3_kernel(const float* __restrict__ src, vd_bf16_bits* __restrict__ dst, long n4, long plane) {
  const long i = (long)blockIdx.x * 256 + threadIdx.x;
  if (i >= n4) return;
  const float4 v = reinterpret_cast<const float4*>(src)[i];
  float4 r1, r2;
  typedef __bf16 bf4 __attribute__((ext_vector_type(4)));
  const bf4 h = {(__bf16)v.x, (__bf16)v.y, (__bf16)v.z, (__bf16)v.w};
  r1.x = v.x - (float)h[0]; r1.y = v.y - (float)h[1]; r1.z = v.z - (float)h[2]; r1.w = v.w - (float)h[3];
  const bf4 m = {(__bf16)r1.x, (__bf16)r1.y, (__bf16)r1.z, (__bf16)r1.w};
  r2.x = r1.x - (float)m[0]; r2.y = r1.y - (float)m[1]; r2.z = r1.z - (float)m[2]; r2.w = r1.w - (float)m[3];
  const bf4 l = {(__bf16)r2.x, (__bf16)r2.y, (__bf16)r2.z, (__bf16)r2.w};
  *reinterpret_cast<bf4*>(dst + i * 4) = h;
  *reinterpret_cast<bf4*>(dst + plane + i * 4) = m;
  *reinterpret_cast<bf4*>(dst + 2 * plane + i * 4) = l;
}
static int weights_to_bf16x3(const float* src, vd_bf16_bits* dst, long n, hipStream_t s) {
  hipLaunchKernelGGL(f32_to_bf16x3_kernel, dim3((unsigned)((n / 4 + 255) / 256)), dim3(256), 0, s, src, dst, n / 4, n);
  VD_LAUNCH_CHECK();
  return VD_OK;
}

struct SplitCfg {
  static constexpr int NT = 4, WM = 4, THREADS = 256;
  static constexpr int BM = 128, BN = 128;
  static constexpr int ATILE = BM * 64;
  static constexpr int BTILE = BN * 32;
  static constexpr int STAGE = ATILE + 3 * BTILE;
#ifndef VD_SPLIT_LDS
#define VD_SPLIT_LDS 41984
#endif
  static constexpr int LDS_BYTES = VD_SPLIT_LDS;
  static_assert(LDS_BYTES >= 2 * STAGE, "two stages of 20 KB");
};

#ifndef VD_SPLIT_CG
#define VD_SPLIT_CG 2
#endif
static_assert(VD_SPLIT_CG >= 1 && VD_SPLIT_CG <= 8 && 8 % VD_SPLIT_CG == 0, "the XCD grid is VD_SPLIT_CG x (8 / VD_SPLIT_CG)");
__device__ __forceinline__ bool split_tile_of(int bid, int nwg, int tiles_m, int tiles_n, int& tile_m, int& tile_n) {
  constexpr int CG = VD_SPLIT_CG, RG = 8 / CG;
  if ((tiles_n % CG) == 0 && tiles_n >= 8) {
    const int xcd = bid & 7, li = bid >> 3, cpg = tiles_n / CG, rpg = (tiles_m + RG - 1) / RG;
    tile_n = (xcd % CG) * cpg + li % cpg;
    tile_m = (xcd / CG) * rpg + li / cpg;
    return tile_m < tiles_m && li / cpg < rpg;
  }
  const int wg = xcd_remap(bid, nwg);
  tile_n = wg % tiles_n;
  tile_m = wg / tiles_n;
  return true;
}
static int split_grid(int tiles_m, int tiles_n) {
  constexpr int CG = VD_SPLIT_CG, RG = 8 / CG;
  if ((tiles_n % CG) == 0 && tiles_n >= 8) return 8 * ((tiles_m + RG - 1) / RG) * (tiles_n / CG);
  return tiles_m * tiles_n;
}

template <int NPROD, class Epi>
__global__ void __launch_bounds__(256, 3)
gemm_split_kernel(int M, int N, int K, int tiles_n, const float* A, long lda, const vd_bf16_bits* B, long ldb, long bplane, Epi epi) {
  using Cfg = SplitCfg;
  constexpr int NT = Cfg::NT;
  extern __shared__ __attribute__((aligned(16))) float smem[];
  int tile_m, tile_n;
  if (!split_tile_of((int)blockIdx.x, (int)gridDim.x, (M + Cfg::BM - 1) / Cfg::BM, tiles_n, tile_m, tile_n)) return;
  const int row_base = tile_m * Cfg::BM, col_base = tile_n * Cfg::BN;
  constexpr int NIA = 2;
  constexpr int NIB = 3;
  const int tid = (int)threadIdx.x, lane = tid & 63;
  const int wm = __builtin_amdgcn_readfirstlane(tid >> 6);
  const int nm = K / 16;
  const int wrow = row_base + wm * 32;

  f32x16 acc[NT];
#pragma unroll
  for (int j = 0; j < NT; ++j)
#pragma unroll
    for (int r = 0; r < 16; ++r) acc[j][r] = 0.f;

  typename EpiPreOf<Epi>::type pre;
  if constexpr (EpiPreOf<Epi>::value) epi.preload(pre, wrow, lane, M);

  unsigned voffa[NIA], voffb[NIB];
#pragma unroll
  for (int i = 0; i < NIA; ++i) {
    const int r = wm * 32 + i * 16 + (lane >> 2);
    const int c = (lane & 3) ^ ((r >> 2) & 3);
    voffa[i] = (unsigned)(((long)min(row_base + r, M - 1) * lda + c * 4) * 4);
  }
  {
    const int r = wm * 32 + (lane >> 1);
    const int c = (lane & 1) ^ ((r >> 4) & 1);
    const unsigned v = (unsigned)(((long)min(col_base + r, N - 1) * ldb + c * 8) * 2);
#pragma unroll
    for (int i = 0; i < NIB; ++i) voffb[i] = v;
  }
  const unsigned lds0 = (unsigned)(uintptr_t)smem;
  auto issue = [&](int m, int st) {
    const unsigned base = lds0 + st * Cfg::STAGE;
#pragma unroll
    for (int i = 0; i < NIB; ++i)
      glds16(voffb[i], reinterpret_cast<const float*>(B + (long)i * bplane + (long)m * 16), base + Cfg::ATILE + i * Cfg::BTILE + wm * 1024);
    const float* ak = A + (long)m * 16;
#pragma unroll
    for (int i = 0; i < NIA; ++i) glds16(voffa[i], ak, base + (wm * NIA + i) * 1024);
  };
  const int hi = lane >> 5, l31 = lane & 31;
  const int sw = (l31 >> 2) & 3;
  const int cb = (hi ^ ((l31 >> 4) & 1)) * 16;

  if (nm > 0) {
    issue(0, 0);
    int st = 0;
    for (int m = 0; m < nm; ++m) {
      if (m + 1 < nm) {
        issue(m + 1, st ^ 1);
        asm volatile("s_waitcnt vmcnt(5)" ::: "memory");
      } else {
        asm volatile("s_waitcnt vmcnt(0)" ::: "memory");
      }
      asm volatile("s_barrier" ::: "memory");
      const char* sbase = reinterpret_cast<const char*>(smem) + st * Cfg::STAGE;
      const float* sa = reinterpret_cast<const float*>(sbase) + (wm * 32 + l31) * 16;
      const float4 u = *reinterpret_cast<const float4*>(sa + (((hi * 2) ^ sw) * 4));
      const float4 w = *reinterpret_cast<const float4*>(sa + (((hi * 2 + 1) ^ sw) * 4));
      vd_bf16x8 ap[3];
      vd_split3(u, w, ap[0], ap[1], ap[2]);
#pragma unroll
      for (int p = 2; p >= 0; --p) {
        vd_bf16x8 bp[NT];
#pragma unroll
        for (int j = 0; j < NT; ++j) {
          const vd_f32x4 t = *reinterpret_cast<const vd_f32x4*>(sbase + Cfg::ATILE + p * Cfg::BTILE + (j * 32 + l31) * 32 + cb);
          bp[j] = __builtin_bit_cast(vd_bf16x8, t);
        }
#pragma unroll
        for (int i = 2; i >= 0; --i) {
          constexpr int LIM = NPROD >= 9 ? 4 : NPROD >= 6 ? 2 : NPROD >= 3 ? 1 : 0;
          if (i + p > LIM) continue;
#pragma unroll
          for (int j = 0; j < NT; ++j) acc[j] = __builtin_amdgcn_mfma_f32_32x32x16_bf16(ap[i], bp[j], acc[j], 0, 0, 0);
        }
      }
      asm volatile("s_waitcnt lgkmcnt(0)\n\ts_barrier" ::: "memory");
      st ^= 1;
    }
  }
  if constexpr (EpiPreOf<Epi>::value) epi(acc, wrow, col_base, lane, M, N, smem + wm * 1024, &pre);
  else epi(acc, wrow, col_base, lane, M, N, smem + wm * 1024);
}

template <int NPROD, class Epi>
static int launch_gemm_split(int M, int N, int K, const float* A, long lda, const vd_bf16_bits* B, long ldb, long bplane, const Epi& e,
                             hipStream_t stream) {
  if (M <= 0 || N <= 0) return VD_OK;
  using Cfg = SplitCfg;
  VD_CHECK_ARG(K % 16 == 0 && lda % 4 == 0 && ldb % 8 == 0 && (long)M * lda * 4 < (1L << 32) && (long)N * ldb * 2 < (1L << 32),
               "launch_gemm_split: unsupported shape M=%d N=%d K=%d", M, N, K);
  const int tiles_m = vd_cdiv(M, Cfg::BM), tiles_n = vd_cdiv(N, Cfg::BN);
  auto kern = gemm_split_kernel<NPROD, Epi>;
  static bool attr_set = false;
  if (!attr_set) {
    VD_HIP(hipFuncSetAttribute(reinterpret_cast<const void*>(kern), hipFuncAttributeMaxDynamicSharedMemorySize, 160 * 1024));
    attr_set = true;
  }
  hipLaunchKernelGGL(kern, dim3(split_grid(tiles_m, tiles_n)), dim3(256), Cfg::LDS_BYTES, stream, M, N, K, tiles_n, A, lda, B, ldb, bplane, e);
  VD_LAUNCH_CHECK();
  return VD_OK;
}

struct SplitTnCfg {
  static constexpr int BM = 256, BN = 128, THREADS = 256;
  static constexpr int ATILE = 16 * BM * 4;
  static constexpr int BTILE = 16 * BN * 4;
  static constexpr int STAGE = ATILE + BTILE;
  static constexpr int LDS_BYTES = 2 * STAGE;
};
static_assert(SplitTnCfg::BM == VD_SPLIT_TN_BM && SplitTnCfg::BN == VD_SPLIT_TN_BN, "paths.h vd_tn_split_tiles");

template <int NPROD>
__global__ void __launch_bounds__(256, 2)
gemm_split_tn_kernel(int M, int N, int kchunk, int K, int tiles, int tiles_n, int splits, const float* A, long lda, const float* B, long ldb,
                     float* C, long ldc) {
  using Cfg = SplitTnCfg;
  extern __shared__ __attribute__((aligned(16))) float smem[];
  int tile, split;
  if ((splits & 7) == 0) {
    const int xcd = (int)blockIdx.x & 7, li = (int)blockIdx.x >> 3;
    split = xcd * (splits >> 3) + li / tiles;
    tile = li % tiles;
  } else {
    split = (int)blockIdx.x / tiles;
    tile = (int)blockIdx.x % tiles;
  }
  const int m_base = (tile / tiles_n) * Cfg::BM, n_base = (tile % tiles_n) * Cfg::BN;
  const int ks = split * kchunk, ke = min(K, ks + kchunk);
  const int nm = ke > ks ? (ke - ks) / 16 : 0;
  const int tid = (int)threadIdx.x, lane = tid & 63;
  const int wm = __builtin_amdgcn_readfirstlane(tid >> 6);

  f32x16 acc[2][4];
#pragma unroll
  for (int mb = 0; mb < 2; ++mb)
#pragma unroll
    for (int j = 0; j < 4; ++j)
#pragma unroll
      for (int r = 0; r < 16; ++r) acc[mb][j][r] = 0.f;

  unsigned voffa[4], voffb[2];
#pragma unroll
  for (int i = 0; i < 4; ++i) voffa[i] = (unsigned)(((long)(wm * 4 + i) * lda + m_base + lane * 4) * 4);
#pragma unroll
  for (int i = 0; i < 2; ++i) voffb[i] = (unsigned)(((long)((wm * 2 + i) * 2 + (lane >> 5)) * ldb + n_base + (lane & 31) * 4) * 4);
  const unsigned lds0 = (unsigned)(uintptr_t)smem;
  auto issue = [&](int m, int st) {
    const unsigned base = lds0 + st * Cfg::STAGE;
    const float* ak = A + (long)(ks + m * 16) * lda;
    const float* bk = B + (long)(ks + m * 16) * ldb;
#pragma unroll
    for (int i = 0; i < 2; ++i) glds16(voffb[i], bk, base + Cfg::ATILE + (wm * 2 + i) * 1024);
#pragma unroll
    for (int i = 0; i < 4; ++i) glds16(voffa[i], ak, base + (wm * 4 + i) * 1024);
  };
  const int hi = lane >> 5, l31 = lane & 31;

  if (nm > 0) {
    issue(0, 0);
    int st = 0;
    for (int m = 0; m < nm; ++m) {
      if (m + 1 < nm) {
        issue(m + 1, st ^ 1);
        asm volatile("s_waitcnt vmcnt(6)" ::: "memory");
      } else {
        asm volatile("s_waitcnt vmcnt(0)" ::: "memory");
      }
      asm volatile("s_barrier" ::: "memory");
      const float* sA = reinterpret_cast<const float*>(reinterpret_cast<const char*>(smem) + st * Cfg::STAGE) + (hi * 8) * Cfg::BM + wm * 64 + l31;
      const float* sB = reinterpret_cast<const float*>(reinterpret_cast<const char*>(smem) + st * Cfg::STAGE + Cfg::ATILE) + (hi * 8) * Cfg::BN + l31;
      vd_bf16x8 ap[2][3], bp[2][3];
      auto load_b = [&](int j, vd_bf16x8 (&dst)[3]) {
        const float* p = sB + j * 32;
        const float4 u = make_float4(p[0], p[Cfg::BN], p[2 * Cfg::BN], p[3 * Cfg::BN]);
        const float4 w = make_float4(p[4 * Cfg::BN], p[5 * Cfg::BN], p[6 * Cfg::BN], p[7 * Cfg::BN]);
        vd_split3(u, w, dst[0], dst[1], dst[2]);
      };
#pragma unroll
      for (int mb = 0; mb < 2; ++mb) {
        const float* p = sA + mb * 32;
        const float4 u = make_float4(p[0], p[Cfg::BM], p[2 * Cfg::BM], p[3 * Cfg::BM]);
        const float4 w = make_float4(p[4 * Cfg::BM], p[5 * Cfg::BM], p[6 * Cfg::BM], p[7 * Cfg::BM]);
        vd_split3(u, w, ap[mb][0], ap[mb][1], ap[mb][2]);
      }
      load_b(0, bp[0]);
#pragma unroll
      for (int j = 0; j < 4; ++j) {
        __builtin_amdgcn_sched_barrier(0);
        if (j + 1 < 4) load_b(j + 1, bp[(j + 1) & 1]);
#pragma unroll
        for (int pb = 2; pb >= 0; --pb)
#pragma unroll
          for (int pa = 2; pa >= 0; --pa) {
            constexpr int LIM = NPROD >= 9 ? 4 : NPROD >= 6 ? 2 : NPROD >= 3 ? 1 : 0;
            if (pa + pb > LIM) continue;
#pragma unroll
            for (int mb = 0; mb < 2; ++mb) acc[mb][j] = __builtin_amdgcn_mfma_f32_32x32x16_bf16(ap[mb][pa], bp[j & 1][pb], acc[mb][j], 0, 0, 0);
          }
        if (j + 1 < 4) {
          __builtin_amdgcn_sched_group_barrier(0x100, 4, 0);
#pragma unroll
          for (int i = 0; i < 18; ++i) {
            __builtin_amdgcn_sched_group_barrier(0x008, 1, 0);
            __builtin_amdgcn_sched_group_barrier(0x002, 4, 0);
          }
        }
      }
      asm volatile("s_waitcnt lgkmcnt(0)\n\ts_barrier" ::: "memory");
      st ^= 1;
    }
  }
  if (nm == 0) return;
  const EpiAtomic<4> e{C, ldc};
#pragma unroll
  for (int mb = 0; mb < 2; ++mb) e(acc[mb], m_base + wm * 64 + mb * 32, n_base, lane, M, N);
}

template <int NPROD>
static int launch_gemm_split_tn(int M, int N, int K, const float* A, long lda, const float* B, long ldb, float* C, long ldc, hipStream_t stream) {
  using Cfg = SplitTnCfg;
  VD_CHECK_ARG(M % Cfg::BM == 0 && N % Cfg::BN == 0 && K % 16 == 0 && lda % 4 == 0 && ldb % 4 == 0 && 16L * lda * 4 < (1L << 31) && 16L * ldb * 4 < (1L << 31),
               "launch_gemm_split_tn: unsupported shape M=%d N=%d K=%d", M, N, K);
  if (K == 0) return VD_OK;
  const int tiles_n = N / Cfg::BN, tiles = (M / Cfg::BM) * tiles_n;
  int splits = vd_cdiv(2L * vd_num_cus(), tiles);
  splits = (splits + 7) & ~7;
  int kchunk = vd_cdiv(vd_cdiv(K, splits), 16) * 16;
  if (kchunk < 64) kchunk = 64;
  splits = vd_cdiv(K, kchunk);
  if (splits >= 8) splits = (splits + 7) & ~7;
  auto kern = gemm_split_tn_kernel<NPROD>;
  static bool attr_set = false;
  if (!attr_set) {
    VD_HIP(hipFuncSetAttribute(reinterpret_cast<const void*>(kern), hipFuncAttributeMaxDynamicSharedMemorySize, 160 * 1024));
    attr_set = true;
  }
  hipLaunchKernelGGL(kern, dim3(tiles * splits), dim3(256), Cfg::LDS_BYTES, stream, M, N, kchunk, K, tiles, tiles_n, splits, A, lda, B, ldb, C, ldc);
  VD_LAUNCH_CHECK();
  return VD_OK;
}
```

Before: 8184.

## Fold pad-token table gradient into split-9 dWh GEMM via indicator MFMA

Pad tokens (token 0) in option steps 1..To-1 are dropped from the token sort and the segmented table-gradient row sum. Their gate-gradient column sums are instead produced inside the exact split TN weight-gradient GEMM, using an extra indicator MFMA per tile in the m_base==0 tiles. A small kernel then applies that pad sum to the option bias and to embedding row 0. The aim is to shrink the irregular segmented row-sum over many pad rows, in exchange for extra MFMAs and atomics in the GEMM, a new kernel, and host bookkeeping of skipped counts.

```diff
diff --git a/visdial_amd/csrc/common.h b/visdial_amd/csrc/common.h
--- a/visdial_amd/csrc/common.h
+++ b/visdial_amd/csrc/common.h
@@ -79,6 +79,20 @@
 int vd_segment_rowsum_acc_bf16(const vd_bf16_bits* X16, int64_t ldx, const int32_t* tok, const int32_t* perm, int64_t n, int ncol,
                                float* out, int64_t ldo, hipStream_t stream);
 
+int vd_gemm_tn_acc_pad_p(const float* A, int64_t lda, const float* B, int64_t ldb, float* C, int64_t ldc, int M, int N, int K, int flags,
+                         const int32_t* tok, float* pad_sum, hipStream_t stream);
+int vd_pad_sum_apply_p(const float* pad_sum, int N, const float* Wx, int64_t ldw, int E, float* gb, float* demb0, hipStream_t stream);
+int vd_token_sort_skip_p(const int32_t* tok, int64_t n, int V, int64_t skip_lo, int64_t skip_hi, int32_t* offset, int32_t* work, int32_t* perm,
+                         hipStream_t stream);
+struct vd_model;
+extern "C" {
+int vdt_gemm_tn_acc_pad(const float* A, int64_t lda, const float* B, int64_t ldb, float* C, int64_t ldc, int M, int N, int K, int flags,
+                        const int32_t* tok, float* pad_sum, void* stream);
+int vdt_token_sort_skip(const int32_t* tok, int64_t n, int V, int64_t skip_lo, int64_t skip_hi, int32_t* offset, int32_t* work, int32_t* perm,
+                        void* stream);
+int vdt_model_rowsum_pairs(vd_model* m, int64_t* pairs, int64_t* covered, int64_t* total);
+}
+
 int vd_bf16_shadow_get(int slot, const float* base, size_t floats, vd_bf16_bits** out);
 const vd_bf16_bits* vd_bf16_shadow_find(const float* p, size_t floats);
 void vd_bf16_shadow_invalidate(const float* p, size_t floats);
diff --git a/visdial_amd/csrc/elementwise.hip b/visdial_amd/csrc/elementwise.hip
--- a/visdial_amd/csrc/elementwise.hip
+++ b/visdial_amd/csrc/elementwise.hip
@@ -147,10 +147,11 @@
   return result;
 }
 
-__global__ void tok_count_kernel(const int* __restrict__ tok, long n, int* __restrict__ count) {
+__global__ void tok_count_kernel(const int* __restrict__ tok, long n, int* __restrict__ count, long skip_lo, long skip_hi) {
   const long i = (long)blockIdx.x * blockDim.x + threadIdx.x;
-  const bool active = i < n;
-  wave_agg_atomic_inc(count, active ? tok[i] : 0, active);
+  const int t = i < n ? tok[i] : 0;
+  const bool active = i < n && !(t == 0 && i >= skip_lo && i < skip_hi);
+  wave_agg_atomic_inc(count, t, active);
 }
 
 __global__ void tok_scan_kernel(const int* __restrict__ count, int V, int* __restrict__ offset,
@@ -182,10 +183,11 @@
 }
 
 __global__ void tok_fill_kernel(const int* __restrict__ tok, long n, int* __restrict__ cursor,
-                                int* __restrict__ perm) {
+                                int* __restrict__ perm, long skip_lo, long skip_hi) {
   const long i = (long)blockIdx.x * blockDim.x + threadIdx.x;
-  const bool active = i < n;
-  const int p = wave_agg_atomic_inc(cursor, active ? tok[i] : 0, active);
+  const int t = i < n ? tok[i] : 0;
+  const bool active = i < n && !(t == 0 && i >= skip_lo && i < skip_hi);
+  const int p = wave_agg_atomic_inc(cursor, t, active);
   if (active) perm[p] = (int)i;
 }
 
@@ -433,22 +435,35 @@
 
 int vd_token_sort(const int32_t* tok, int64_t n, int V, int32_t* offset, int32_t* work, int32_t* perm,
                   void* stream) {
-  VD_CHECK_ARG(tok && offset && work && perm && n >= 0 && V > 0, "vd_token_sort: bad args");
-  hipStream_t s = (hipStream_t)stream;
+  return vd_token_sort_skip_p(tok, n, V, 0, 0, offset, work, perm, (hipStream_t)stream);
+}
+
+}
+
+int vd_token_sort_skip_p(const int32_t* tok, int64_t n, int V, int64_t skip_lo, int64_t skip_hi, int32_t* offset, int32_t* work, int32_t* perm,
+                         hipStream_t s) {
+  VD_CHECK_ARG(tok && offset && work && perm && n >= 0 && V > 0 && skip_lo <= skip_hi, "vd_token_sort: bad args");
   int* count = work;
   int* cursor = work + V;
   VD_HIP(hipMemsetAsync(count, 0, sizeof(int) * V, s));
   if (n > 0) {
-    hipLaunchKernelGGL(tok_count_kernel, grid1d(n, 256), dim3(256), 0, s, tok, (long)n, count);
+    hipLaunchKernelGGL(tok_count_kernel, grid1d(n, 256), dim3(256), 0, s, tok, (long)n, count, (long)skip_lo, (long)skip_hi);
     VD_LAUNCH_CHECK();
   }
   hipLaunchKernelGGL(tok_scan_kernel, dim3(1), dim3(1024), 0, s, count, V, offset, cursor);
   VD_LAUNCH_CHECK();
   if (n > 0) {
-    hipLaunchKernelGGL(tok_fill_kernel, grid1d(n, 256), dim3(256), 0, s, tok, (long)n, cursor, perm);
+    hipLaunchKernelGGL(tok_fill_kernel, grid1d(n, 256), dim3(256), 0, s, tok, (long)n, cursor, perm, (long)skip_lo, (long)skip_hi);
     VD_LAUNCH_CHECK();
   }
   return VD_OK;
+}
+
+extern "C" {
+
+int vdt_token_sort_skip(const int32_t* tok, int64_t n, int V, int64_t skip_lo, int64_t skip_hi, int32_t* offset, int32_t* work, int32_t* perm,
+                        void* stream) {
+  return vd_token_sort_skip_p(tok, n, V, skip_lo, skip_hi, offset, work, perm, (hipStream_t)stream);
 }
 
 int vd_segment_rowsum_acc(const float* X, int64_t ldx, const int32_t* tok, const int32_t* perm, int64_t n,
diff --git a/visdial_amd/csrc/gemm_ops.hip b/visdial_amd/csrc/gemm_ops.hip
--- a/visdial_amd/csrc/gemm_ops.hip
+++ b/visdial_amd/csrc/gemm_ops.hip
@@ -408,8 +408,7 @@
   SrcK a{A, lda}, b{B, ldb};
   EpiAtomic<4> e{C, ldc};
   const long tiles = (long)vd_cdiv(M, CfgBig::BM) * vd_cdiv(N, CfgBig::BN);
-  if ((flags & VD_FLAG_SPLIT9) && !(flags & VD_FLAG_BF16) && vd_tn_split_tiles(M, N) && K >= 8192 &&
-      16L * lda * 4 < (1L << 31) && 16L * ldb * 4 < (1L << 31)) {
+  if (vd_tn_split9_fits(flags, M, N, K) && 16L * lda * 4 < (1L << 31) && 16L * ldb * 4 < (1L << 31)) {
     const int K1 = K & ~15;
     if (int rc = launch_gemm_split_tn<9>(M, N, K1, A, lda, B, ldb, C, ldc, (hipStream_t)stream)) return rc;
     if (K1 == K) return VD_OK;
@@ -499,6 +498,51 @@
 
 }
 
+int vd_gemm_tn_acc_pad_p(const float* A, int64_t lda, const float* B, int64_t ldb, float* C, int64_t ldc, int M, int N, int K, int flags,
+                         const int32_t* tok, float* pad_sum, hipStream_t stream) {
+  VD_CHECK_ARG(A && B && C && tok && pad_sum && M >= 0 && N >= 0 && K >= 0, "vd_gemm_tn_acc (pad sum): bad args M=%d N=%d K=%d", M, N, K);
+  if (int rc = check_align(A, lda, "vd_gemm_tn_acc (pad sum) A")) return rc;
+  if (int rc = check_align(B, ldb, "vd_gemm_tn_acc (pad sum) B")) return rc;
+  const long K1 = vd_tn_split9_fits(flags, M, N, K) ? (K & ~15L) : 0;
+  VD_CHECK_ARG(K1 > 0 && 16L * lda * 4 < (1L << 31) && 16L * ldb * 4 < (1L << 31),
+               "vd_gemm_tn_acc (pad sum): M=%d N=%d K=%d flags=%d does not take the exact split with the pad sum", M, N, K, flags);
+  if (int rc = launch_gemm_split_tn<9, true>(M, N, (int)K1, A, lda, B, ldb, C, ldc, stream, tok, pad_sum)) return rc;
+  if (K1 == K) return VD_OK;
+  SrcK a2{A + K1 * lda, lda}, b2{B + K1 * ldb, ldb};
+  EpiAtomic<4> e{C, ldc};
+  return launch_gemm<GemmCfg<4, 1, 4, 16, 0, 4, 41984>>(M, N, K - (int)K1, 1, a2, b2, e, stream);
+}
+
+extern "C" int vdt_gemm_tn_acc_pad(const float* A, int64_t lda, const float* B, int64_t ldb, float* C, int64_t ldc, int M, int N, int K, int flags,
+                                   const int32_t* tok, float* pad_sum, void* stream) {
+  return vd_gemm_tn_acc_pad_p(A, lda, B, ldb, C, ldc, M, N, K, flags, tok, pad_sum, (hipStream_t)stream);
+}
+
+__global__ void __launch_bounds__(256) pad_sum_apply_kernel(const float* __restrict__ pad_sum, int N, const float* __restrict__ Wx, long ldw, int E,
+                                                            float* __restrict__ gb, float* __restrict__ demb0) {
+  const int tid = (int)threadIdx.x, lane = tid & 63;
+  const int gid = (int)blockIdx.x * 256 + tid;
+  if (gid < N) unsafeAtomicAdd(gb + gid, pad_sum[gid]);
+  const int e = (int)blockIdx.x * 4 + (tid >> 6);
+  if (e >= E) return;
+  const float* w = Wx + (long)e * ldw;
+  float s = 0.f;
+  for (int n = lane * 4; n < N; n += 256) {
+    const float4 a = *reinterpret_cast<const float4*>(pad_sum + n), b = *reinterpret_cast<const float4*>(w + n);
+    s += a.x * b.x + a.y * b.y + a.z * b.z + a.w * b.w;
+  }
+  s = wave_sum(s);
+  if (lane == 0) unsafeAtomicAdd(demb0 + e, s);
+}
+int vd_pad_sum_apply_p(const float* pad_sum, int N, const float* Wx, int64_t ldw, int E, float* gb, float* demb0, hipStream_t stream) {
+  VD_CHECK_ARG(pad_sum && Wx && gb && demb0 && N > 0 && N % 4 == 0 && ldw % 4 == 0 && E > 0 && (((uintptr_t)pad_sum | (uintptr_t)Wx) & 15) == 0,
+               "vd_pad_sum_apply: bad args N=%d E=%d", N, E);
+  const int blocks = std::max(vd_cdiv(E, 4), vd_cdiv(N, 256));
+  hipLaunchKernelGGL(pad_sum_apply_kernel, dim3(blocks), dim3(256), 0, stream, pad_sum, N, Wx, (long)ldw, E, gb, demb0);
+  VD_LAUNCH_CHECK();
+  return VD_OK;
+}
+
 __global__ void __launch_bounds__(256) bf16_tn_tail_kernel(const vd_bf16_bits* __restrict__ A, const vd_bf16_bits* __restrict__ B, float* __restrict__ C,
                                                            long ldc, int M, int N, int K) {
   const long i = (long)blockIdx.x * 256 + threadIdx.x;
diff --git a/visdial_amd/csrc/paths.h b/visdial_amd/csrc/paths.h
--- a/visdial_amd/csrc/paths.h
+++ b/visdial_amd/csrc/paths.h
@@ -1,4 +1,5 @@
 #pragma once
+#include <stdlib.h>
 #include "common.h"
 
 static inline int vd_precision_flags(int lstmBf16) {
@@ -26,6 +27,17 @@
 static inline bool vd_tn_kmajor_fits(long M, long N, long K) { return M % 128 == 0 && N % 128 == 0 && K >= 1024; }
 constexpr int VD_SPLIT_TN_BM = 256, VD_SPLIT_TN_BN = 128;
 static inline bool vd_tn_split_tiles(long M, long N) { return M % VD_SPLIT_TN_BM == 0 && N % VD_SPLIT_TN_BN == 0; }
+constexpr long VD_TN_SPLIT9_MIN_K = 8192;
+static inline bool vd_tn_split9_fits(int flags, long M, long N, long K) {
+  return (flags & VD_FLAG_SPLIT9) && !(flags & VD_FLAG_BF16) && vd_tn_split_tiles(M, N) && K >= VD_TN_SPLIT9_MIN_K;
+}
+static inline bool vd_tn_pad_sum_enabled() {
+  const char* e = getenv("VD_DWH_PAD_SUM");
+  return !e || atol(e) > 0;
+}
+static inline long vd_tn_pad_sum_rows(int flags, long M, long N, long K) {
+  return vd_tn_pad_sum_enabled() && vd_tn_split9_fits(flags, M, N, K) ? (K & ~15L) : 0;
+}
 
 static inline bool vd_img_split_ok(long rows, int H, int Kc) {
   return rows >= 128 && H % 16 == 0 && Kc % 16 == 0 && rows * (H > Kc ? H : Kc) * 4 < (1L << 32);
diff --git a/visdial_amd/csrc/rt_core.h b/visdial_amd/csrc/rt_core.h
--- a/visdial_amd/csrc/rt_core.h
+++ b/visdial_amd/csrc/rt_core.h
@@ -91,6 +91,7 @@
   int32_t* opt_uid = nullptr;
   int opt_total = 0;
   int32_t *opt_sort_off = nullptr, *opt_sort_perm = nullptr;
+  long opt_pad_rows = 0, opt_pad_covered = 0, opt_sort_n = 0;
   bool cached = false;
   uint64_t cache_stamp = 0;
   std::vector<int32_t> miss_keys, opt_host;
diff --git a/visdial_amd/csrc/rt_decoders.h b/visdial_amd/csrc/rt_decoders.h
--- a/visdial_amd/csrc/rt_decoders.h
+++ b/visdial_amd/csrc/rt_decoders.h
@@ -153,15 +153,25 @@
     VD_HIP(hipEventRecord(m->ev_prof[3], s));
     VD_TRY(enc_bwd());
     VdRange rwg("disc: table gradient + dWh");
+    const long pad_rows = c16 ? 0 : b.opt_pad_rows;
+    VD_CHECK_ARG(pad_rows == 0 || (To > 1 && pad_rows == (((long)(To - 1) * NO) & ~15L) && b.opt_sort_n + b.opt_pad_covered == (long)To * NO),
+                 "decoder 'disc': the batch slot's pad-sum plan does not match the step (%ld rows of %ld)", pad_rows, (long)(To - 1) * NO);
+    float* pad_sum = nullptr;
+    if (pad_rows > 0) VD_TRY(ws_get(m, "opt.pad_sum", (size_t)(4 * H), &pad_sum));
     VD_TRY(fork_stream(m, s, st));
     if (c16) VD_TRY(vd_segment_rowsum_acc_bf16(gates16, 4 * H, b.opt.tok, perm, (long)To * NO, (int)(4 * H), dtab, 4 * H, st));
-    else VD_TRY(vd_segment_rowsum_acc(gates, 4 * H, b.opt.tok, perm, (long)To * NO, (int)(4 * H), dtab, 4 * H, st));
+    else VD_TRY(vd_segment_rowsum_acc(gates, 4 * H, b.opt.tok, perm, pad_rows > 0 ? b.opt_sort_n : (long)To * NO, (int)(4 * H), dtab, 4 * H, st));
     VD_TRY(vd_colsum_acc(dtab, 4 * H, (int)V + 1, (int)(4 * H), Gp(m, "opt.b"), st));
     VD_TRY(vd_gemm_tn_acc(Wp(m, "embed"), E, dtab, 4 * H, Gp(m, "opt.W"), 4 * H, (int)E, (int)(4 * H), (int)V + 1, 0, st));
     VD_HIP(hipEventRecord(m->ev_prof[4], s));
     if (To > 1 && c16)
       VD_TRY(vd_gemm_tn_acc_bf16(h16, gates16 + (long)NO * 4 * H, Gp(m, "opt.W") + E * 4 * H, 4 * H, (int)H, (int)(4 * H), (To - 1) * NO, s));
-    else if (To > 1)
+    else if (pad_rows > 0) {
+      VD_TRY(vd_memset(pad_sum, 0, 4 * H * 4, s));
+      VD_TRY(vd_gemm_tn_acc_pad_p(h, H, gates + (long)NO * 4 * H, 4 * H, Gp(m, "opt.W") + E * 4 * H, 4 * H, (int)H, (int)(4 * H), (To - 1) * NO,
+                                  flags & (VD_FLAG_BF16 | VD_FLAG_SPLIT9), b.opt.tok + NO, pad_sum, s));
+      VD_TRY(vd_pad_sum_apply_p(pad_sum, (int)(4 * H), Wopt, 4 * H, (int)E, Gp(m, "opt.b"), Gp(m, "embed"), s));
+    } else if (To > 1)
       VD_TRY(vd_gemm_tn_acc(h, H, gates + (long)NO * 4 * H, 4 * H, Gp(m, "opt.W") + E * 4 * H, 4 * H, (int)H, (int)(4 * H), (To - 1) * NO,
                             flags & (VD_FLAG_BF16 | VD_FLAG_SPLIT9), s));
     VD_HIP(hipEventRecord(m->ev_prof[5], s));
diff --git a/visdial_amd/csrc/runtime.hip b/visdial_amd/csrc/runtime.hip
--- a/visdial_amd/csrc/runtime.hip
+++ b/visdial_amd/csrc/runtime.hip
@@ -6,7 +6,8 @@
 
 namespace {
 
-int upload_tokens(BatchSlot& sl, SeqTok& ss, const std::string& tag, const int32_t* rows_major, int N, int T, bool sorted, hipStream_t s) {
+int upload_tokens(BatchSlot& sl, SeqTok& ss, const std::string& tag, const int32_t* rows_major, int N, int T, bool sorted, hipStream_t s,
+                  long skip_lo = 0, long skip_hi = 0, long* n_skip = nullptr) {
   ss.T = T;
   ss.N = N;
   ss.present = true;
@@ -17,15 +18,18 @@
   VD_TRY(pin_get(sl.pinned, tag + ".stage", total * sizeof(int32_t), (void**)&stage));
   int32_t* tok = stage;
   std::vector<int> len(sorted ? N : 0);
+  long skipped = 0;
   for (int n = 0; n < N; ++n) {
     int first = T;
     for (int t = 0; t < T; ++t) {
       const int32_t v = rows_major[(size_t)n * T + t];
       tok[(size_t)t * N + n] = v;
       if (v != 0 && first == T) first = t;
+      else if (v == 0) skipped += (long)t * N + n >= skip_lo && (long)t * N + n < skip_hi;
     }
     if (sorted) len[n] = T - first;
   }
+  if (n_skip) *n_skip = skipped;
   if (sorted) {
     int32_t* tok_sorted = stage + TN;
     int32_t* fwd_idx = stage + 2 * TN;
@@ -122,6 +126,7 @@
   VD_TRY(dev_get(sl.bufs, "opt.uid", (size_t)NO * sizeof(int32_t), (void**)&sl.opt_uid));
   VD_HIP(hipMemcpyAsync(sl.opt_uid, up, (size_t)NO * sizeof(int32_t), hipMemcpyHostToDevice, s));
   sl.opt_sort_off = sl.opt_sort_perm = nullptr;
+  sl.opt_pad_rows = sl.opt_pad_covered = sl.opt_sort_n = 0;
   return VD_OK;
 }
 
@@ -526,6 +531,10 @@
     sl.cached = false;
     const int To = hb->To;
     bool dedup = false;
+    const long Hh = m->p.rnnHiddenSize;
+    long pad_covered = 0;
+    auto pad_rows_of = [&](long rows) { return To > 1 ? vd_tn_pad_sum_rows(m->flags, Hh, 4 * Hh, (long)(To - 1) * rows) : 0L; };
+    sl.opt_pad_rows = sl.opt_pad_covered = sl.opt_sort_n = 0;
     if (m->ocache.capacity > 0 && !m->training) {
       sl.opt_host.assign(hb->options, hb->options + (size_t)NO * To);
       VD_TRY(option_cache_resolve(m, sl, sl.opt_host.data(), NO, To, s));
@@ -557,7 +566,8 @@
       }
       if ((double)U <= 0.95 * (double)NO) {
         dedup = true;
-        VD_TRY(upload_tokens(sl, sl.opt, "opt", uniq.data(), U, To, false, s));
+        sl.opt_pad_rows = pad_rows_of(U);
+        VD_TRY(upload_tokens(sl, sl.opt, "opt", uniq.data(), U, To, false, s, U, U + sl.opt_pad_rows, &pad_covered));
         int32_t* up = nullptr;
         VD_TRY(pin_get(sl.pinned, "opt.uid.stage", (size_t)NO * sizeof(int32_t), (void**)&up));
         memcpy(up, uid.data(), (size_t)NO * sizeof(int32_t));
@@ -565,7 +575,10 @@
         VD_HIP(hipMemcpyAsync(sl.opt_uid, up, (size_t)NO * sizeof(int32_t), hipMemcpyHostToDevice, s));
       }
     }
-    if (!dedup && !sl.cached) VD_TRY(upload_tokens(sl, sl.opt, "opt", hb->options, (int)NO, hb->To, false, s));
+    if (!dedup && !sl.cached) {
+      sl.opt_pad_rows = pad_rows_of(NO);
+      VD_TRY(upload_tokens(sl, sl.opt, "opt", hb->options, (int)NO, hb->To, false, s, NO, NO + sl.opt_pad_rows, &pad_covered));
+    }
     sl.opt_sort_off = sl.opt_sort_perm = nullptr;
     if (!sl.cached) {
       const long V1 = (long)m->p.vocabSize + 1, n = (long)sl.opt.T * sl.opt.N;
@@ -573,7 +586,10 @@
       VD_TRY(dev_get(sl.bufs, "opt.sort_off", (size_t)(V1 + 1) * sizeof(int32_t), (void**)&sl.opt_sort_off));
       VD_TRY(dev_get(sl.bufs, "opt.sort_work", (size_t)2 * V1 * sizeof(int32_t), (void**)&work));
       VD_TRY(dev_get(sl.bufs, "opt.sort_perm", (size_t)n * sizeof(int32_t), (void**)&sl.opt_sort_perm));
-      VD_TRY(vd_token_sort(sl.opt.tok, n, (int)V1, sl.opt_sort_off, work, sl.opt_sort_perm, s));
+      const long lo = sl.opt.N, hi = lo + sl.opt_pad_rows;
+      VD_TRY(vd_token_sort_skip_p(sl.opt.tok, n, (int)V1, lo, hi, sl.opt_sort_off, work, sl.opt_sort_perm, s));
+      sl.opt_pad_covered = pad_covered;
+      sl.opt_sort_n = n - pad_covered;
     }
   }
   if (!disc && hb->answer_in && hb->answer_out) {
@@ -775,6 +791,16 @@
   return VD_OK;
 }
 
+int vdt_model_rowsum_pairs(vd_model* m, int64_t* pairs, int64_t* covered, int64_t* total) {
+  VD_CHECK_ARG(m && pairs && covered && total && (m->cur >= 0 || m->uploaded >= 0), "vdt_model_rowsum_pairs: no batch uploaded");
+  const BatchSlot& b = m->slot[m->cur >= 0 ? m->cur : m->uploaded];
+  const bool sorted = b.opt.present && b.opt_sort_perm;
+  *pairs = sorted ? b.opt_sort_n : 0;
+  *covered = sorted ? b.opt_pad_covered : 0;
+  *total = sorted ? (int64_t)b.opt.T * b.opt.N : 0;
+  return VD_OK;
+}
+
 int vd_model_synchronize(vd_model* m) {
   VD_CHECK_ARG(m, "vd_model_synchronize: null model");
   for (hipStream_t s : {m->s_copy, m->s_enc, m->s_img, m->s_tab, m->s_wg, m->s_main})
diff --git a/visdial_amd/csrc/split_core.h b/visdial_amd/csrc/split_core.h
--- a/visdial_amd/csrc/split_core.h
+++ b/visdial_amd/csrc/split_core.h
@@ -196,10 +196,114 @@
 };
 static_assert(SplitTnCfg::BM == VD_SPLIT_TN_BM && SplitTnCfg::BN == VD_SPLIT_TN_BN, "paths.h vd_tn_split_tiles");
 
-template <int NPROD>
+typedef int vd_i32x16 __attribute__((ext_vector_type(16)));
+__device__ __forceinline__ vd_i32x16 vd_sload16(const int* p) {
+  vd_i32x16 v;
+  asm volatile("s_load_dwordx16 %0, %1, 0x0" : "=s"(v) : "s"(p) : "memory");
+  return v;
+}
+
+template <int NPROD, int PJ>
+__device__ __forceinline__ void split_tn_loop(f32x16 (&acc)[2][4], f32x16& pacc, int nm, int ks, int m_base, int n_base, int wm, int lane,
+                                              const float* A, long lda, const float* B, long ldb, const int* tok, float* smem) {
+  using Cfg = SplitTnCfg;
+  unsigned voffa[4], voffb[2];
+#pragma unroll
+  for (int i = 0; i < 4; ++i) voffa[i] = (unsigned)(((long)(wm * 4 + i) * lda + m_base + lane * 4) * 4);
+#pragma unroll
+  for (int i = 0; i < 2; ++i) voffb[i] = (unsigned)(((long)((wm * 2 + i) * 2 + (lane >> 5)) * ldb + n_base + (lane & 31) * 4) * 4);
+  const unsigned lds0 = (unsigned)(uintptr_t)smem;
+  auto issue = [&](int m, int st) {
+    const unsigned base = lds0 + st * Cfg::STAGE;
+    const float* ak = A + (long)(ks + m * 16) * lda;
+    const float* bk = B + (long)(ks + m * 16) * ldb;
+#pragma unroll
+    for (int i = 0; i < 2; ++i) glds16(voffb[i], bk, base + Cfg::ATILE + (wm * 2 + i) * 1024);
+#pragma unroll
+    for (int i = 0; i < 4; ++i) glds16(voffa[i], ak, base + (wm * 4 + i) * 1024);
+  };
+  const int hi = lane >> 5, l31 = lane & 31;
+  const unsigned lane0 = lane == 0 ? ~0u : 0u, lane32 = lane == 32 ? ~0u : 0u;
+  vd_i32x16 tk = {};
+  if constexpr (PJ >= 0) {
+    tk = vd_sload16(tok + ks);
+    asm volatile("s_waitcnt lgkmcnt(0)" : "+s"(tk)::"memory");
+  }
+
+  issue(0, 0);
+  int st = 0;
+  for (int m = 0; m < nm; ++m) {
+    if (m + 1 < nm) {
+      issue(m + 1, st ^ 1);
+      asm volatile("s_waitcnt vmcnt(6)" ::: "memory");
+    } else {
+      asm volatile("s_waitcnt vmcnt(0)" ::: "memory");
+    }
+    asm volatile("s_barrier" ::: "memory");
+    vd_bf16x8 ind = {};
+    vd_i32x16 tkn = {};
+    if constexpr (PJ >= 0) {
+      unsigned w[8];
+#pragma unroll
+      for (int d = 0; d < 8; ++d) w[d] = (tk[2 * d] == 0 ? 0x3f80u : 0u) | (tk[2 * d + 1] == 0 ? 0x3f800000u : 0u);
+      vd_u32x4 v;
+#pragma unroll
+      for (int d = 0; d < 4; ++d) v[d] = (w[d] & lane0) | (w[4 + d] & lane32);
+      ind = __builtin_bit_cast(vd_bf16x8, v);
+      tkn = vd_sload16(tok + ks + min(m + 1, nm - 1) * 16);
+    }
+    const float* sA = reinterpret_cast<const float*>(reinterpret_cast<const char*>(smem) + st * Cfg::STAGE) + (hi * 8) * Cfg::BM + wm * 64 + l31;
+    const float* sB = reinterpret_cast<const float*>(reinterpret_cast<const char*>(smem) + st * Cfg::STAGE + Cfg::ATILE) + (hi * 8) * Cfg::BN + l31;
+    vd_bf16x8 ap[2][3], bp[2][3];
+    auto load_b = [&](int j, vd_bf16x8 (&dst)[3]) {
+      const float* p = sB + j * 32;
+      const float4 u = make_float4(p[0], p[Cfg::BN], p[2 * Cfg::BN], p[3 * Cfg::BN]);
+      const float4 w = make_float4(p[4 * Cfg::BN], p[5 * Cfg::BN], p[6 * Cfg::BN], p[7 * Cfg::BN]);
+      vd_split3(u, w, dst[0], dst[1], dst[2]);
+    };
+#pragma unroll
+    for (int mb = 0; mb < 2; ++mb) {
+      const float* p = sA + mb * 32;
+      const float4 u = make_float4(p[0], p[Cfg::BM], p[2 * Cfg::BM], p[3 * Cfg::BM]);
+      const float4 w = make_float4(p[4 * Cfg::BM], p[5 * Cfg::BM], p[6 * Cfg::BM], p[7 * Cfg::BM]);
+      vd_split3(u, w, ap[mb][0], ap[mb][1], ap[mb][2]);
+    }
+    load_b(0, bp[0]);
+#pragma unroll
+    for (int j = 0; j < 4; ++j) {
+      __builtin_amdgcn_sched_barrier(0);
+      if (j + 1 < 4) load_b(j + 1, bp[(j + 1) & 1]);
+#pragma unroll
+      for (int pb = 2; pb >= 0; --pb) {
+#pragma unroll
+        for (int pa = 2; pa >= 0; --pa) {
+          constexpr int LIM = NPROD >= 9 ? 4 : NPROD >= 6 ? 2 : NPROD >= 3 ? 1 : 0;
+          if (pa + pb > LIM) continue;
+#pragma unroll
+          for (int mb = 0; mb < 2; ++mb) acc[mb][j] = __builtin_amdgcn_mfma_f32_32x32x16_bf16(ap[mb][pa], bp[j & 1][pb], acc[mb][j], 0, 0, 0);
+        }
+        if (PJ == j) pacc = __builtin_amdgcn_mfma_f32_32x32x16_bf16(ind, bp[j & 1][pb], pacc, 0, 0, 0);
+      }
+      if (j + 1 < 4) {
+        __builtin_amdgcn_sched_group_barrier(0x100, 4, 0);
+#pragma unroll
+        for (int i = 0; i < 18 + (PJ == j ? 3 : 0); ++i) {
+          __builtin_amdgcn_sched_group_barrier(0x008, 1, 0);
+          __builtin_amdgcn_sched_group_barrier(0x002, 4, 0);
+        }
+      }
+    }
+    if constexpr (PJ >= 0) asm volatile("s_waitcnt lgkmcnt(0)\n\ts_barrier" : "+s"(tkn)::"memory");
+    else asm volatile("s_waitcnt lgkmcnt(0)\n\ts_barrier" ::: "memory");
+    tk = tkn;
+    st ^= 1;
+  }
+}
+
+template <int NPROD, bool PAD = false>
 __global__ void __launch_bounds__(256, 2)
 gemm_split_tn_kernel(int M, int N, int kchunk, int K, int tiles, int tiles_n, int splits, const float* A, long lda, const float* B, long ldb,
-                     float* C, long ldc) {
+                     float* C, long ldc, const int* tok, float* pad_sum) {
   using Cfg = SplitTnCfg;
   extern __shared__ __attribute__((aligned(16))) float smem[];
   int tile, split;
@@ -216,94 +320,37 @@
   const int nm = ke > ks ? (ke - ks) / 16 : 0;
   const int tid = (int)threadIdx.x, lane = tid & 63;
   const int wm = __builtin_amdgcn_readfirstlane(tid >> 6);
-
-  f32x16 acc[2][4];
+  if (nm == 0) return;
+
+  f32x16 acc[2][4], pacc;
 #pragma unroll
   for (int mb = 0; mb < 2; ++mb)
 #pragma unroll
     for (int j = 0; j < 4; ++j)
 #pragma unroll
       for (int r = 0; r < 16; ++r) acc[mb][j][r] = 0.f;
-
-  unsigned voffa[4], voffb[2];
-#pragma unroll
-  for (int i = 0; i < 4; ++i) voffa[i] = (unsigned)(((long)(wm * 4 + i) * lda + m_base + lane * 4) * 4);
-#pragma unroll
-  for (int i = 0; i < 2; ++i) voffb[i] = (unsigned)(((long)((wm * 2 + i) * 2 + (lane >> 5)) * ldb + n_base + (lane & 31) * 4) * 4);
-  const unsigned lds0 = (unsigned)(uintptr_t)smem;
-  auto issue = [&](int m, int st) {
-    const unsigned base = lds0 + st * Cfg::STAGE;
-    const float* ak = A + (long)(ks + m * 16) * lda;
-    const float* bk = B + (long)(ks + m * 16) * ldb;
-#pragma unroll
-    for (int i = 0; i < 2; ++i) glds16(voffb[i], bk, base + Cfg::ATILE + (wm * 2 + i) * 1024);
-#pragma unroll
-    for (int i = 0; i < 4; ++i) glds16(voffa[i], ak, base + (wm * 4 + i) * 1024);
-  };
-  const int hi = lane >> 5, l31 = lane & 31;
-
-  if (nm > 0) {
-    issue(0, 0);
-    int st = 0;
-    for (int m = 0; m < nm; ++m) {
-      if (m + 1 < nm) {
-        issue(m + 1, st ^ 1);
-        asm volatile("s_waitcnt vmcnt(6)" ::: "memory");
-      } else {
-        asm volatile("s_waitcnt vmcnt(0)" ::: "memory");
-      }
-      asm volatile("s_barrier" ::: "memory");
-      const float* sA = reinterpret_cast<const float*>(reinterpret_cast<const char*>(smem) + st * Cfg::STAGE) + (hi * 8) * Cfg::BM + wm * 64 + l31;
-      const float* sB = reinterpret_cast<const float*>(reinterpret_cast<const char*>(smem) + st * Cfg::STAGE + Cfg::ATILE) + (hi * 8) * Cfg::BN + l31;
-      vd_bf16x8 ap[2][3], bp[2][3];
-      auto load_b = [&](int j, vd_bf16x8 (&dst)[3]) {
-        const float* p = sB + j * 32;
-        const float4 u = make_float4(p[0], p[Cfg::BN], p[2 * Cfg::BN], p[3 * Cfg::BN]);
-        const float4 w = make_float4(p[4 * Cfg::BN], p[5 * Cfg::BN], p[6 * Cfg::BN], p[7 * Cfg::BN]);
-        vd_split3(u, w, dst[0], dst[1], dst[2]);
-      };
-#pragma unroll
-      for (int mb = 0; mb < 2; ++mb) {
-        const float* p = sA + mb * 32;
-        const float4 u = make_float4(p[0], p[Cfg::BM], p[2 * Cfg::BM], p[3 * Cfg::BM]);
-        const float4 w = make_float4(p[4 * Cfg::BM], p[5 * Cfg::BM], p[6 * Cfg::BM], p[7 * Cfg::BM]);
-        vd_split3(u, w, ap[mb][0], ap[mb][1], ap[mb][2]);
-      }
-      load_b(0, bp[0]);
-#pragma unroll
-      for (int j = 0; j < 4; ++j) {
-        __builtin_amdgcn_sched_barrier(0);
-        if (j + 1 < 4) load_b(j + 1, bp[(j + 1) & 1]);
-#pragma unroll
-        for (int pb = 2; pb >= 0; --pb)
-#pragma unroll
-          for (int pa = 2; pa >= 0; --pa) {
-            constexpr int LIM = NPROD >= 9 ? 4 : NPROD >= 6 ? 2 : NPROD >= 3 ? 1 : 0;
-            if (pa + pb > LIM) continue;
-#pragma unroll
-            for (int mb = 0; mb < 2; ++mb) acc[mb][j] = __builtin_amdgcn_mfma_f32_32x32x16_bf16(ap[mb][pa], bp[j & 1][pb], acc[mb][j], 0, 0, 0);
-          }
-        if (j + 1 < 4) {
-          __builtin_amdgcn_sched_group_barrier(0x100, 4, 0);
-#pragma unroll
-          for (int i = 0; i < 18; ++i) {
-            __builtin_amdgcn_sched_group_barrier(0x008, 1, 0);
-            __builtin_amdgcn_sched_group_barrier(0x002, 4, 0);
-          }
-        }
-      }
-      asm volatile("s_waitcnt lgkmcnt(0)\n\ts_barrier" ::: "memory");
-      st ^= 1;
-    }
-  }
-  if (nm == 0) return;
+#pragma unroll
+  for (int r = 0; r < 16; ++r) pacc[r] = 0.f;
+
+  bool padded = false;
+  if constexpr (PAD) padded = m_base == 0;
+  if (padded) {
+    if (wm == 0) split_tn_loop<NPROD, 0>(acc, pacc, nm, ks, m_base, n_base, wm, lane, A, lda, B, ldb, tok, smem);
+    else if (wm == 1) split_tn_loop<NPROD, 1>(acc, pacc, nm, ks, m_base, n_base, wm, lane, A, lda, B, ldb, tok, smem);
+    else if (wm == 2) split_tn_loop<NPROD, 2>(acc, pacc, nm, ks, m_base, n_base, wm, lane, A, lda, B, ldb, tok, smem);
+    else split_tn_loop<NPROD, 3>(acc, pacc, nm, ks, m_base, n_base, wm, lane, A, lda, B, ldb, tok, smem);
+    if (lane < 32) unsafeAtomicAdd(pad_sum + n_base + wm * 32 + lane, pacc[0]);
+  } else {
+    split_tn_loop<NPROD, -1>(acc, pacc, nm, ks, m_base, n_base, wm, lane, A, lda, B, ldb, tok, smem);
+  }
   const EpiAtomic<4> e{C, ldc};
 #pragma unroll
   for (int mb = 0; mb < 2; ++mb) e(acc[mb], m_base + wm * 64 + mb * 32, n_base, lane, M, N);
 }
 
-template <int NPROD>
-static int launch_gemm_split_tn(int M, int N, int K, const float* A, long lda, const float* B, long ldb, float* C, long ldc, hipStream_t stream) {
+template <int NPROD, bool PAD = false>
+static int launch_gemm_split_tn(int M, int N, int K, const float* A, long lda, const float* B, long ldb, float* C, long ldc, hipStream_t stream,
+                                const int* tok = nullptr, float* pad_sum = nullptr) {
   using Cfg = SplitTnCfg;
   VD_CHECK_ARG(M % Cfg::BM == 0 && N % Cfg::BN == 0 && K % 16 == 0 && lda % 4 == 0 && ldb % 4 == 0 && 16L * lda * 4 < (1L << 31) && 16L * ldb * 4 < (1L << 31),
                "launch_gemm_split_tn: unsupported shape M=%d N=%d K=%d", M, N, K);
@@ -315,13 +362,14 @@
   if (kchunk < 64) kchunk = 64;
   splits = vd_cdiv(K, kchunk);
   if (splits >= 8) splits = (splits + 7) & ~7;
-  auto kern = gemm_split_tn_kernel<NPROD>;
+  VD_CHECK_ARG(PAD == (tok != nullptr) && PAD == (pad_sum != nullptr), "launch_gemm_split_tn: the pad sum takes the tokens and an output");
+  auto kern = gemm_split_tn_kernel<NPROD, PAD>;
   static bool attr_set = false;
   if (!attr_set) {
     VD_HIP(hipFuncSetAttribute(reinterpret_cast<const void*>(kern), hipFuncAttributeMaxDynamicSharedMemorySize, 160 * 1024));
     attr_set = true;
   }
-  hipLaunchKernelGGL(kern, dim3(tiles * splits), dim3(256), Cfg::LDS_BYTES, stream, M, N, kchunk, K, tiles, tiles_n, splits, A, lda, B, ldb, C, ldc);
+  hipLaunchKernelGGL(kern, dim3(tiles * splits), dim3(256), Cfg::LDS_BYTES, stream, M, N, kchunk, K, tiles, tiles_n, splits, A, lda, B, ldb, C, ldc, tok, pad_sum);
   VD_LAUNCH_CHECK();
   return VD_OK;
 }
```

Result: no change. 8152 (-0.4%).
